# ThomasZiegler/RS-aware-differential-SfM

Hardware: AMD Instinct MI355X
Metric: Mpixels/sec RS depth+pose solve, 1280x720 pair (higher is better)
Workload: dtype f64

## Files before the change

include/rsdsfm.h:

```cpp
#ifndef RSDSFM_H
#define RSDSFM_H

#include <stddef.h>
#include <stdint.h>

#ifdef __cplusplus
extern "C" {
#endif

#define RSDSFM_OK 0
#define RSDSFM_ERR_INVALID (-1)
#define RSDSFM_ERR_HIP (-2)
#define RSDSFM_ERR_NO_DEVICE (-3)
#define RSDSFM_ERR_NUMERIC (-4)
#define RSDSFM_ERR_PENDING (-5)
#define RSDSFM_ERR_PEER (-6)

#define RSDSFM_DEPTH_CLOSED_FORM 0
#define RSDSFM_DEPTH_CERES_LM 1

#define RSDSFM_K_COMPAT 0
#define RSDSFM_K_FIXED 1

#define RSDSFM_FLOW_COMPAT_RANK 0
// ... 81 lines not shown
                  const double* alpha_m, const double* alpha_k_m, const int64_t* inlier_idx_or_null,
                  const double v_in[3], const double w_in[3], double k_in, int const_acceleration,
                  int flow_index_mode, double* inliers_out_3m, double v_out[3], double w_out[3], double* k_out,
                  rsdsfm_lm_summary* summary_or_null);
int rsdsfm_last_ransac_tag(rsdsfm_ctx* ctx, uint64_t* tag, int64_t* cache_hits_or_null);
int rsdsfm_refine_from_ransac(rsdsfm_ctx* ctx, uint64_t ransac_tag, const double* flow2n, int64_t n_flow, int64_t m, const double* inliers_3m,
                              const double* alpha_m, const double* alpha_k_m, const int64_t* inlier_idx_or_null, const double v_in[3],
                              const double w_in[3], double k_in, int const_acceleration, int flow_index_mode, double* inliers_out_3m,
                              double v_out[3], double w_out[3], double* k_out, rsdsfm_lm_summary* summary_or_null);
#define RSDSFM_REFINE_TRACE_COLS 8
#define RSDSFM_TRACE_REJECTED 0.0
#define RSDSFM_TRACE_ACCEPTED 1.0
#define RSDSFM_TRACE_INVALID 2.0
#define RSDSFM_TRACE_PARAMETER_TOL 3.0
#define RSDSFM_TRACE_FUNCTION_TOL 4.0
#define RSDSFM_TRACE_ACCEPTED_GRADIENT_TOL 5.0
int rsdsfm_set_refine_trace(rsdsfm_ctx* ctx, int32_t rows);
int rsdsfm_get_refine_trace(rsdsfm_ctx* ctx, double* trace_rows_x_8, int32_t rows);
int rsdsfm_flatten(rsdsfm_ctx* ctx, const double* flow_img_rows_cols_2, int32_t rows, int32_t cols, double fx,
                   double fy, double cx, double cy, double gamma, double flow_threshold, double* q2n,
                   double* u2n, double* alpha_n, double* alpha_k_n, int64_t* n_out);
int rsdsfm_depth_map(rsdsfm_ctx* ctx, double* inliers_3m_inout, int64_t m, double v_inout[3], double fx,
                     double fy, double cx, double cy, int32_t rows, int32_t cols,
                     double* depth_map_colmajor, int32_t* xs_or_null, int32_t* ys_or_null, int* flipped);
int rsdsfm_pose_table(rsdsfm_ctx* ctx, const double v[3], const double w[3], double k, double gamma,
                      int32_t rows, double* R_rows9, double* t_rows3);

int rsdsfm_estimate_inverse_depths_dev(rsdsfm_ctx* ctx, const double* d_q2n, const double* d_u2n, int64_t n,
                                       const double v[3], const double w[3], double k, const double* d_alpha_n,
                                       const double* d_alpha_k_n, int depth_mode, double* d_inv_depth_n);
int rsdsfm_flatten_dev(rsdsfm_ctx* ctx, const double* d_flow_img, int32_t rows, int32_t cols, double fx, double fy,
                       double cx, double cy, double gamma, double flow_threshold, double* d_q2n, double* d_u2n,
                       double* d_alpha_n, double* d_alpha_k_n, int64_t* n_out);
int rsdsfm_depth_map_dev(rsdsfm_ctx* ctx, double* d_inliers_3m_inout, int64_t m, double v_inout[3], double fx, double fy,
                         double cx, double cy, int32_t rows, int32_t cols, double* d_depth_map_colmajor,
                         int32_t* d_xs_or_null, int32_t* d_ys_or_null, int* flipped);
int rsdsfm_pose_table_dev(rsdsfm_ctx* ctx, const double v[3], const double w[3], double k, double gamma, int32_t rows,
                          double* d_R_rows9, double* d_t_rows3);
typedef struct rsdsfm_frame_params {
    int32_t ransac_trials;
    int32_t use_acceleration_mode;
    int32_t use_refinement;
    int32_t depth_mode;
    int32_t k_sign_mode;
    int32_t flow_index_mode;
    int32_t use_global_shutter_mode;
    int32_t struct_bytes;
    double ransac_tol;
    double flow_threshold;
    uint64_t seed;
} rsdsfm_frame_params;

void rsdsfm_frame_params_init(rsdsfm_frame_params* params);

typedef struct rsdsfm_frame_result {
    int64_t n_points, num_inliers;
    int32_t best_trial, flipped;
    double ransac_w[3], ransac_v[3], ransac_k;
    double w[3], v[3], k;
    rsdsfm_lm_summary refine_summary;
    const double* d_inliers;
    const int64_t* d_inlier_idx;
    const int32_t* d_scanline;
} rsdsfm_frame_result;

int rsdsfm_solve_frame_dev(rsdsfm_ctx* ctx, const double* d_flow_img, int32_t rows, int32_t cols, double fx, double fy,
                           double cx, double cy, double gamma, const rsdsfm_frame_params* params,
                           double* d_depth_map_colmajor, double* d_R_rows9_or_null, double* d_t_rows3_or_null,
                           rsdsfm_frame_result* result);
typedef struct rsdsfm_frame_job {
    const double* d_flow_img;
    int32_t rows, cols;
    double fx, fy, cx, cy, gamma;
    double* d_depth_map_colmajor;
    double* d_R_rows9_or_null;
    double* d_t_rows3_or_null;
    uint64_t seed;
} rsdsfm_frame_job;
int rsdsfm_solve_frames_dev(rsdsfm_ctx* ctx, const rsdsfm_frame_job* jobs, int32_t count, const rsdsfm_frame_params* params,
                            rsdsfm_frame_result* results);
int rsdsfm_set_sequence_lanes(rsdsfm_ctx* ctx, int32_t lanes);
int rsdsfm_set_frame_side_flatten(rsdsfm_ctx* ctx, int mode);
int rsdsfm_set_frame_tail(rsdsfm_ctx* ctx, int mode);
int rsdsfm_ransac_dev(rsdsfm_ctx* ctx, const double* d_q2n, const double* d_u2n, const double* d_alpha_n,
                      const double* d_alpha_k_n, int64_t n, int use_alpha_k, int32_t iterations, double tolerance,
                      const int32_t* samples_9xT_or_null, uint64_t seed, int depth_mode, int k_sign_mode,
                      rsdsfm_ransac_out* out);
int rsdsfm_refine_dev(rsdsfm_ctx* ctx, const double* d_flow2n, int64_t n_flow, int64_t m, const double* d_inliers_3m,
                      const double* d_alpha_m, const double* d_alpha_k_m, const int64_t* d_inlier_idx_or_null,
                      const double v_in[3], const double w_in[3], double k_in, int const_acceleration,
                      int flow_index_mode, double* d_inliers_out_3m, double v_out[3], double w_out[3], double* k_out,
                      rsdsfm_lm_summary* summary_or_null);
int rsdsfm_estimate_inverse_depths_batch_dev(rsdsfm_ctx* const* ctxs, int32_t count, const double* const* d_q2n,
                                             const double* const* d_u2n, const int64_t* n, const double* v_count_x3,
                                             const double* w_count_x3, const double* k_count, const double* const* d_alpha_n,
                                             const double* const* d_alpha_k_n, double* const* d_inv_depth_n);
int rsdsfm_depth_lm_batch_launch_dev(rsdsfm_ctx* const* ctxs, int32_t count, const double* const* d_q2n, const double* const* d_u2n,
                                     const int64_t* n, const double* v_count_x3, const double* w_count_x3, const double* k_count,
                                     const double* const* d_alpha_n, const double* const* d_alpha_k_n, double* const* d_inv_depth_n);
int rsdsfm_depth_lm_launch_dev(rsdsfm_ctx* ctx, const double* d_q2n, const double* d_u2n, int64_t n,
                               const double v[3], const double w[3], double k, const double* d_alpha_n,
                               const double* d_alpha_k_n, double* d_inv_depth_n, int launch_id);
int rsdsfm_depth_lm_sums_row_size(void);
int rsdsfm_depth_lm_reduce_dev(rsdsfm_ctx* ctx, int64_t n_shard, double* d_row_out);
int rsdsfm_depth_lm_decide_rows_dev(rsdsfm_ctx* ctx, const double* d_rows, int32_t nrows, int64_t n_total, int launch_id);
int rsdsfm_depth_lm_state(rsdsfm_ctx* ctx, int32_t* status, int32_t* next_launch, rsdsfm_lm_summary* summary_or_null);
int rsdsfm_depth_finish_dev(rsdsfm_ctx* ctx, const double* d_q2n, const double* d_u2n, int64_t n,
                            const double v[3], const double w[3], double k, const double* d_alpha_n,
                            const double* d_alpha_k_n, double* d_inv_depth_n, rsdsfm_lm_summary* summary_or_null,
                            int32_t* extra_launches);

int rsdsfm_flatten_slab_dev(rsdsfm_ctx* ctx, const double* d_img_slab, int32_t rows, int32_t slab_cols, int32_t col0,
                            double fx, double fy, double cx, double cy, double gamma, double thr, double* d_q2n,
                            double* d_u2n, double* d_alpha_n, double* d_alpha_k_n, int64_t* n_out);
int rsdsfm_sample_indices(int64_t n, int32_t iterations, uint64_t seed, int32_t* samples);
int rsdsfm_minimal9_dev(rsdsfm_ctx* ctx, const double* d_q9, const double* d_u9, const double* d_alpha9,
                        const double* d_alpha_k9, int32_t count, int use_alpha_k, int k_sign_mode, double* d_hyp);
int rsdsfm_minimal9_probe_dev(rsdsfm_ctx* ctx, const double* d_q9, const double* d_u9, const double* d_alpha9, const double* d_alpha_k9,
                              int32_t count, int use_alpha_k, int k_sign_mode, int use_cores, double* d_hyp, double* d_probe4);
size_t rsdsfm_tile_lm_state_bytes(void);
size_t rsdsfm_tile_best_bytes(void);
int32_t rsdsfm_tile_ransac_row_size(void);
int32_t rsdsfm_tile_ransac_batch(void);
int rsdsfm_tile_ransac_lm_rows_dev(rsdsfm_ctx* ctx, const double* d_q2n, const double* d_u2n, const double* d_alpha_n,
                                   const double* d_alpha_k_n, int64_t n_shard, const double* d_hyp, int32_t count,
                                   const void* d_states, int32_t round, double tolerance, double* d_rows);
int rsdsfm_tile_ransac_decide_dev(rsdsfm_ctx* ctx, const double* d_rows_all, int32_t nranks, int32_t count, void* d_states,
                                  int64_t n_total, int32_t round, int32_t* d_flags, int32_t* d_scored, double* d_trial_count,
                                  double* d_trial_err);
int rsdsfm_tile_ransac_score_rows_dev(rsdsfm_ctx* ctx, const double* d_q2n, const double* d_u2n, const double* d_alpha_n,
                                      const double* d_alpha_k_n, int64_t n_shard, const double* d_hyp, int32_t count,
                                      const void* d_states, int depth_mode, double tolerance, const int32_t* d_scored_or_null,
                                      double* d_rows);
int rsdsfm_tile_ransac_score_merge_dev(rsdsfm_ctx* ctx, const double* d_rows_all, int32_t nranks, int32_t count,
                                       const int32_t* d_scored_or_null, double* d_trial_count, double* d_trial_err);
int rsdsfm_tile_ransac_pick_dev(rsdsfm_ctx* ctx, const double* d_trial_count, const double* d_trial_err, int32_t iterations,
                                const double* d_hyp, void* d_best);
int rsdsfm_tile_ransac_final_dev(rsdsfm_ctx* ctx, const double* d_q2n, const double* d_u2n, const double* d_alpha_n,
                                 const double* d_alpha_k_n, int64_t n_shard, void* d_best, const void* d_states, int depth_mode,
                                 double tolerance, double* d_inv_depth_n, uint8_t* d_mask_n, int64_t* d_inlier_idx,
                                 double* d_inliers3m, double* d_out_alpha, double* d_out_alpha_k, rsdsfm_ransac_out* out);
int64_t rsdsfm_tile_ransac_global_inliers(rsdsfm_ctx* ctx, const void* d_best);
int rsdsfm_tile_refine_begin_dev(rsdsfm_ctx* ctx, const double* d_flow2n, int64_t n_flow, int64_t m_shard, const double* d_inl3m,
                                 const double* d_alpha_m, const double* d_alpha_k_m, const int64_t* d_inlier_idx,
                                 const double v_in[3], const double w_in[3], double k_in, int const_acceleration,
                                 int flow_index_mode);
int32_t rsdsfm_tile_refine_row_size(int const_acceleration, int32_t stage);
int rsdsfm_tile_refine_rows_dev(rsdsfm_ctx* ctx, int32_t stage, double* d_row);
int rsdsfm_tile_refine_apply_dev(rsdsfm_ctx* ctx, int32_t stage, const double* d_rows_all, int32_t nranks, int64_t m_total);
int rsdsfm_tile_refine_poll(rsdsfm_ctx* ctx, double v_out[3], double w_out[3], double* k_out, rsdsfm_lm_summary* summary);
int rsdsfm_tile_refine_finish_dev(rsdsfm_ctx* ctx, double* d_inl_out3m);
int rsdsfm_tile_zsum_dev(rsdsfm_ctx* ctx, const double* d_inl3m, int64_t m_shard, double* d_zsum1);
int rsdsfm_tile_depth_map_dev(rsdsfm_ctx* ctx, double* d_inl3m, int64_t m_shard, const double* d_zsums_all, int32_t nranks,
                              int64_t m_total, double v_inout[3], double fx, double fy, double cx, double cy, int32_t rows,
                              int32_t col0, int32_t slab_cols, double* d_depth_slab, int32_t* d_xs_or_null,
                              int32_t* d_ys_or_null, int* flipped);

#define RSDSFM_DIST_ID_BYTES 128
int rsdsfm_dist_unique_id(void* id_128_bytes);
int rsdsfm_dist_init(rsdsfm_ctx* ctx, int32_t nranks, int32_t rank, const void* id_128_bytes);
int rsdsfm_dist_adopt(rsdsfm_ctx* ctx, void* nccl_comm, int32_t nranks, int32_t rank);
typedef int (*rsdsfm_all_gather_fn)(void* user, const void* d_send, void* d_recv, size_t bytes_per_rank, void* hip_stream);
typedef int (*rsdsfm_all_reduce_sum_f64_fn)(void* user, double* d_buf, size_t count, void* hip_stream);
int rsdsfm_dist_set_transport(rsdsfm_ctx* ctx, int32_t nranks, int32_t rank, rsdsfm_all_gather_fn all_gather_fn,
                              rsdsfm_all_reduce_sum_f64_fn all_reduce_fn, void* user);
int rsdsfm_dist_finalize(rsdsfm_ctx* ctx);
// ... 75 lines not shown
```

rs-aware-differential-sfm_amd/__init__.py:

```python
import ctypes as C
import os
import sys

import numpy as np

from . import dist, pipeline, synth

_HERE = os.path.dirname(os.path.abspath(__file__))
LIB_PATH = os.environ.get("RSDSFM_LIB") or os.path.join(_HERE, "librsdsfm_hip.so")
LIB_PATH_FUSED = os.path.join(_HERE, "librsdsfm_hip_fused.so")
HEADER_PATH = os.path.join(os.path.dirname(_HERE), "include", "rsdsfm.h")

OK = 0
ERR_PENDING = -5
DEPTH_CLOSED_FORM, DEPTH_CERES_LM = 0, 1
K_COMPAT, K_FIXED = 0, 1
FLOW_COMPAT_RANK, FLOW_GATHERED = 0, 1
REFINE_TRACE_COLS = 8
TRACE_REJECTED, TRACE_ACCEPTED, TRACE_INVALID, TRACE_PARAMETER_TOL, TRACE_FUNCTION_TOL, TRACE_ACCEPTED_GRADIENT_TOL = 0.0, 1.0, 2.0, 3.0, 4.0, 5.0
TERMINATION = {0: "gradient", 1: "parameter", 2: "function", 3: "max_iter", 4: "failure", 5: "min_radius"}

_libs = {}


# ... 411 lines not shown

    def solve_frame_dev(self, d_flow_img, rows, cols, K, gamma, d_depth_map, d_R=None, d_t=None, trials=50, tol=0.05, seed=1,
                        use_acceleration_mode=False, use_refinement=True, depth_mode=DEPTH_CERES_LM, k_sign_mode=K_COMPAT, flow_threshold=1e-10,
                        flow_index_mode=FLOW_COMPAT_RANK, use_global_shutter_mode=False):
        prm = FrameParams(int(trials), int(use_acceleration_mode), int(use_refinement), int(depth_mode), int(k_sign_mode),
                          int(flow_index_mode), int(use_global_shutter_mode), 0, float(tol), float(flow_threshold), int(seed))
        res = FrameResult()
        d = C.c_double
        self._check(self.lib.rsdsfm_solve_frame_dev(self._ctx, _dp(d_flow_img), C.c_int32(rows), C.c_int32(cols), d(K[0]), d(K[1]), d(K[2]), d(K[3]),
                                                    d(gamma), C.byref(prm), _dp(d_depth_map), _dp(d_R) if d_R else None, _dp(d_t) if d_t else None,
                                                    C.byref(res)), "rsdsfm_solve_frame_dev")
        return dict(n=int(res.n_points), num_inliers=int(res.num_inliers), best_trial=int(res.best_trial), flipped=bool(res.flipped),
                    ransac_w=np.array(res.ransac_w[:]), ransac_v=np.array(res.ransac_v[:]), ransac_k=float(res.ransac_k),
                    w=np.array(res.w[:]), v=np.array(res.v[:]), k=float(res.k), refine_summary=res.refine_summary.as_dict(),
                    d_inliers=res.d_inliers, d_inlier_idx=res.d_inlier_idx, d_scanline=res.d_scanline)

    def dist_init(self, nranks, rank, unique_id):
        self._check(self.lib.rsdsfm_dist_init(self._ctx, C.c_int32(nranks), C.c_int32(rank), C.c_char_p(bytes(unique_id))), "rsdsfm_dist_init")

    def dist_set_transport(self, nranks, rank, all_gather, all_reduce):
        self._ag = ALL_GATHER_FN(lambda user, s_, r_, b_, st: int(all_gather(s_, r_, b_, st)))
        self._ar = ALL_REDUCE_FN(lambda user, p_, n_, st: int(all_reduce(p_, n_, st)))
        self._check(self.lib.rsdsfm_dist_set_transport(self._ctx, C.c_int32(nranks), C.c_int32(rank), self._ag, self._ar, None), "rsdsfm_dist_set_transport")

    def dist_finalize(self):
        self._check(self.lib.rsdsfm_dist_finalize(self._ctx), "rsdsfm_dist_finalize")

    def solve_frame_tiled_dev(self, d_img_slab, rows, cols, K, gamma, d_depth_map, d_R=None, d_t=None, trials=50, tol=0.05, seed=1,
                              use_acceleration_mode=False, use_refinement=True, depth_mode=DEPTH_CERES_LM, k_sign_mode=K_COMPAT,
                              flow_threshold=1e-10, use_global_shutter_mode=False, flow_index_mode=FLOW_COMPAT_RANK):
        prm = FrameParams(int(trials), int(use_acceleration_mode), int(use_refinement), int(depth_mode), int(k_sign_mode),
                          int(flow_index_mode), int(use_global_shutter_mode), 0, float(tol), float(flow_threshold), int(seed))
        res, info = FrameResult(), TiledInfo()
        d = C.c_double
        self._check(self.lib.rsdsfm_solve_frame_tiled_dev(self._ctx, _dp(d_img_slab) if d_img_slab else None, C.c_int32(rows), C.c_int32(cols), d(K[0]), d(K[1]),
                                                          d(K[2]), d(K[3]), d(gamma), C.byref(prm), _dp(d_depth_map), _dp(d_R) if d_R else None,
                                                          _dp(d_t) if d_t else None, C.byref(res), C.byref(info)), "rsdsfm_solve_frame_tiled_dev")
        return dict(n=int(res.n_points), num_inliers=int(res.num_inliers), best_trial=int(res.best_trial), flipped=bool(res.flipped),
                    ransac_w=np.array(res.ransac_w[:]), ransac_v=np.array(res.ransac_v[:]), ransac_k=float(res.ransac_k),
                    w=np.array(res.w[:]), v=np.array(res.v[:]), k=float(res.k), refine_summary=res.refine_summary.as_dict(),
                    d_inliers=res.d_inliers, d_inlier_idx=res.d_inlier_idx, d_scanline=res.d_scanline, flow_index_mode=int(flow_index_mode),
                    info={k2: int(getattr(info, k2)) for k2, _ in TiledInfo._fields_ if k2 != "_pad"})

    def estimate_inverse_depths_tiled_dev(self, d_q_shard, d_u_shard, n_total, v, w, k, d_alpha_shard, d_alpha_k_shard, d_inv_depth,
                                          mode=DEPTH_CERES_LM):
        sm, info = LmSummary(), TiledInfo()
        opt = lambda p_: _dp(p_) if p_ else None
        self._check(self.lib.rsdsfm_estimate_inverse_depths_tiled_dev(self._ctx, opt(d_q_shard), opt(d_u_shard), C.c_int64(n_total), _v3(v), _v3(w),
                                                                      C.c_double(k), opt(d_alpha_shard), opt(d_alpha_k_shard), C.c_int(int(mode)),
                                                                      opt(d_inv_depth), C.byref(sm), C.byref(info)),
                    "rsdsfm_estimate_inverse_depths_tiled_dev")
        return (sm.as_dict() if int(mode) == DEPTH_CERES_LM else None,
                {k2: int(getattr(info, k2)) for k2, _ in TiledInfo._fields_ if k2 != "_pad"})

    def prepared_frame_solve(self, d_flow_img, rows, cols, K, gamma, d_depth_map, d_R=None, d_t=None, trials=50, tol=0.05,
                             use_acceleration_mode=False, use_refinement=True, depth_mode=DEPTH_CERES_LM, k_sign_mode=K_COMPAT,
                             flow_threshold=1e-10, flow_index_mode=FLOW_COMPAT_RANK, use_global_shutter_mode=False):
        prm = FrameParams(int(trials), int(use_acceleration_mode), int(use_refinement), int(depth_mode), int(k_sign_mode),
                          int(flow_index_mode), int(use_global_shutter_mode), 0, float(tol), float(flow_threshold), 0)
        res = FrameResult()
        d = C.c_double
        fn = self.lib.rsdsfm_solve_frame_dev
        args = (self._ctx, _dp(d_flow_img), C.c_int32(rows), C.c_int32(cols), d(K[0]), d(K[1]), d(K[2]), d(K[3]), d(gamma), C.byref(prm),
                _dp(d_depth_map), _dp(d_R) if d_R else None, _dp(d_t) if d_t else None, C.byref(res))
        check = self._check

        def call(seed):
            prm.seed = seed
            rc = fn(*args)
            if rc != OK:
                check(rc, "rsdsfm_solve_frame_dev")
            return res

        return call

    def set_sequence_lanes(self, lanes):
        self._check(self.lib.rsdsfm_set_sequence_lanes(self._ctx, C.c_int32(int(lanes))), "rsdsfm_set_sequence_lanes")

    def set_frame_side_flatten(self, on):
        self._check(self.lib.rsdsfm_set_frame_side_flatten(self._ctx, int(on)), "rsdsfm_set_frame_side_flatten")

    def set_frame_tail(self, mode):
        self._check(self.lib.rsdsfm_set_frame_tail(self._ctx, int(mode)), "rsdsfm_set_frame_tail")

    def prepared_frames_solve(self, jobs, trials=50, tol=0.05, use_acceleration_mode=False, use_refinement=True, depth_mode=DEPTH_CERES_LM,
                              k_sign_mode=K_COMPAT, flow_threshold=1e-10, flow_index_mode=FLOW_COMPAT_RANK, use_global_shutter_mode=False):
        n = len(jobs)
        arr = (FrameJob * n)()
        for a, j in zip(arr, jobs):
            K = j["K"]
            a.d_flow_img, a.rows, a.cols = int(j["d_flow_img"]), int(j["rows"]), int(j["cols"])
            a.fx, a.fy, a.cx, a.cy, a.gamma = float(K[0]), float(K[1]), float(K[2]), float(K[3]), float(j["gamma"])
            a.d_depth_map, a.d_R, a.d_t = int(j["d_depth_map"]), int(j.get("d_R") or 0) or None, int(j.get("d_t") or 0) or None
        prm = FrameParams(int(trials), int(use_acceleration_mode), int(use_refinement), int(depth_mode), int(k_sign_mode),
                          int(flow_index_mode), int(use_global_shutter_mode), 0, float(tol), float(flow_threshold), 0)
        res = (FrameResult * n)()
        fn, ctx, check = self.lib.rsdsfm_solve_frames_dev, self._ctx, self._check

        def call(seeds):
            for a, sd in zip(arr, seeds):
                a.seed = int(sd)
            rc = fn(ctx, arr, C.c_int32(n), C.byref(prm), res)
            if rc != OK:
                check(rc, "rsdsfm_solve_frames_dev")
            return res

        return call

    def solve_frames_dev(self, jobs, seeds, **kw):
        res = self.prepared_frames_solve(jobs, **kw)(seeds)
        return [dict(n=int(r.n_points), num_inliers=int(r.num_inliers), best_trial=int(r.best_trial), flipped=bool(r.flipped),
                     ransac_w=np.array(r.ransac_w[:]), ransac_v=np.array(r.ransac_v[:]), ransac_k=float(r.ransac_k),
                     w=np.array(r.w[:]), v=np.array(r.v[:]), k=float(r.k), refine_summary=r.refine_summary.as_dict(),
                     d_inliers=r.d_inliers, d_inlier_idx=r.d_inlier_idx, d_scanline=r.d_scanline) for r in res]

    def depth_lm_reduce_dev(self, n_shard, d_row):
        self._check(self.lib.rsdsfm_depth_lm_reduce_dev(self._ctx, C.c_int64(n_shard), _dp(d_row)), "rsdsfm_depth_lm_reduce_dev")

    def depth_lm_decide_rows_dev(self, d_rows, nrows, n_total, launch_id):
        self._check(self.lib.rsdsfm_depth_lm_decide_rows_dev(self._ctx, _dp(d_rows), C.c_int32(nrows), C.c_int64(n_total), int(launch_id)), "rsdsfm_depth_lm_decide_rows_dev")

    def depth_lm_state(self):
        status, nxt, sm = C.c_int32(), C.c_int32(), LmSummary()
        self._check(self.lib.rsdsfm_depth_lm_state(self._ctx, C.byref(status), C.byref(nxt), C.byref(sm)), "rsdsfm_depth_lm_state")
        return status.value, nxt.value, sm.as_dict()

    def depth_finish_dev(self, d_q, d_u, n, v, w, k, d_alpha, d_alpha_k, d_rho):
        sm = LmSummary()
        extra = C.c_int32()
        self._check(self.lib.rsdsfm_depth_finish_dev(self._ctx, _dp(d_q), _dp(d_u), C.c_int64(n), _v3(v), _v3(w), C.c_double(k), _dp(d_alpha), _dp(d_alpha_k), _dp(d_rho), C.byref(sm), C.byref(extra)), "rsdsfm_depth_finish_dev")
        return sm.as_dict(), extra.value


def _np0(ptr):
    return _dp(ptr) if ptr else None


def tile_sizes():
    lib = load_library()
    lib.rsdsfm_tile_lm_state_bytes.restype = C.c_size_t
    lib.rsdsfm_tile_best_bytes.restype = C.c_size_t
    return (int(lib.rsdsfm_tile_lm_state_bytes()), int(lib.rsdsfm_tile_best_bytes()), int(lib.rsdsfm_tile_ransac_row_size()),
            int(lib.rsdsfm_tile_ransac_batch()))


def sample_indices(n, iterations, seed):
    lib = load_library()
    out = np.zeros((max(int(iterations), 0), 9), dtype=np.int32)
    rc = lib.rsdsfm_sample_indices(C.c_int64(n), C.c_int32(iterations), C.c_uint64(seed), _p(out))
    if rc != OK:
        raise RsdsfmError("rsdsfm_sample_indices failed (%d): needs 9 <= n < 2^31" % rc)
    return out


class _TileMixin:
    def flatten_slab_dev(self, d_img_slab, rows, slab_cols, col0, K, gamma, d_q, d_u, d_alpha, d_alpha_k, thr=1e-10):
        cnt = C.c_int64()
        d = C.c_double
        self._check(self.lib.rsdsfm_flatten_slab_dev(self._ctx, _np0(d_img_slab), C.c_int32(rows), C.c_int32(slab_cols), C.c_int32(col0), d(K[0]), d(K[1]), d(K[2]), d(K[3]), d(gamma), d(thr), _np0(d_q), _np0(d_u), _np0(d_alpha), _np0(d_alpha_k), C.byref(cnt)), "rsdsfm_flatten_slab_dev")
        return cnt.value

    def minimal9_probe_dev(self, d_q9, d_u9, d_a9, d_ak9, count, use_alpha_k, k_sign_mode, use_cores, d_hyp, d_probe4):
        self._check(self.lib.rsdsfm_minimal9_probe_dev(self._ctx, _dp(d_q9), _dp(d_u9), _dp(d_a9), _dp(d_ak9), C.c_int32(count), int(use_alpha_k), int(k_sign_mode),
                                                       int(use_cores), _dp(d_hyp), _dp(d_probe4)), "rsdsfm_minimal9_probe_dev")

    def minimal9_dev(self, d_q9, d_u9, d_a9, d_ak9, count, use_alpha_k, k_sign_mode, d_hyp):
# ... 1441 lines not shown
```

rs-aware-differential-sfm_amd/csrc/frame_host.hip:

```cpp
#include <stdlib.h>
#include <string.h>

#include <atomic>

#include <algorithm>
#include <new>

#include "rsdsfm_internal.hpp"
#include "sequence_host.hpp"

namespace rsdsfm {

static std::atomic<int> g_frames_in_flight[64];
int frames_in_flight(const Ctx* c) { return g_frames_in_flight[c->device & 63].load(std::memory_order_relaxed); }

int alpha_ones_launch(Ctx* c, double* d_alpha, int64_t n);
int flatten_device(Ctx* c, const double* d_img, int32_t rows, int32_t cols, int32_t col0, double fx, double fy, double cx, double cy, double gamma,
                   double thr, double* d_q, double* d_u, double* d_alpha, double* d_alpha_k, int64_t* n_out);

struct FrameRun {
    rsdsfm_frame_job job;
    rsdsfm_frame_params prm;
    size_t N = 0;
    int64_t n = 0;
    double *d_q = nullptr, *d_u = nullptr, *d_a = nullptr, *d_ak = nullptr, *d_in_a = nullptr, *d_in_ak = nullptr, *d_inl = nullptr, *d_inl_ref = nullptr;
    int64_t* d_idx = nullptr;
    uint8_t* d_mask = nullptr;
    int32_t* d_ys = nullptr;
    double *d_zpartials = nullptr, *d_zheader = nullptr;
    char* d_refine_ws = nullptr;
    rsdsfm_ransac_out ro;
    RansacRun ransac;
    RefineRun refine;
    Minimal9Direct direct;
    DenseFlatten dense;
    bool refinement_enqueued = false, ahead = false, side_flatten = false, dense_in_launch = false, open = false;
    bool counted = false;
    int rc_begin = RSDSFM_OK;
    int64_t m_known = -1;
    RefineTail tail;
    FinishClaim claim;
    RansacSpecTail spec_tail;
    std::function<int()> join;
};

namespace {

inline double* header_host(Ctx* c) { return reinterpret_cast<double*>(static_cast<char*>(c->h_pinned) + c->pinned_bytes - 64); }
inline RefineState* state_host(Ctx* c) { return reinterpret_cast<RefineState*>(static_cast<char*>(c->h_pinned) + c->pinned_bytes - kPinnedTail); }
inline int64_t* count_host(Ctx* c) { return reinterpret_cast<int64_t*>(static_cast<char*>(c->h_pinned) + c->pinned_bytes - kPinnedTail / 2); }
static_assert(sizeof(RefineState) + sizeof(int) <= kPinnedTail / 2, "reserved tail: state read-back | point count ... depth-map header");

struct StreamSwap {
    Ctx* c;
    hipStream_t main;
    StreamSwap(Ctx* ctx, hipStream_t other) : c(ctx), main(ctx->stream) { c->stream = other; }
    ~StreamSwap() { c->stream = main; }
};

int ensure_side_stream(Ctx* c) {
    if (c->aux_stream) return RSDSFM_OK;
    RSDSFM_HIP_CHECK(c, hipStreamCreateWithFlags(&c->aux_stream, hipStreamNonBlocking));
    RSDSFM_HIP_CHECK(c, hipEventCreateWithFlags(&c->ev_fork, hipEventDisableTiming));
    RSDSFM_HIP_CHECK(c, hipEventCreateWithFlags(&c->ev_join, hipEventDisableTiming));
    return RSDSFM_OK;
}

static void frame_uncount(const Ctx* c, FrameRun* F) {
    if (F && F->counted) {
        F->counted = false;
        g_frames_in_flight[c->device & 63].fetch_sub(1, std::memory_order_relaxed);
    }
}
struct FrameInFlightEnd {
    const Ctx* c;
    FrameRun* F;
    ~FrameInFlightEnd() { frame_uncount(c, F); }
};

int frame_begin(Ctx* c, FrameRun* F) {
    const rsdsfm_frame_job& J = F->job;
    const rsdsfm_frame_params* prm = &F->prm;
    frame_uncount(c, F);
    F->open = false;
    F->rc_begin = RSDSFM_OK;
    if (J.rows <= 0 || J.cols <= 0 || !J.d_flow_img || !J.d_depth_map_colmajor) return fail(c, RSDSFM_ERR_INVALID, "bad arguments");
    if (prm->flow_index_mode != RSDSFM_FLOW_COMPAT_RANK && prm->flow_index_mode != RSDSFM_FLOW_GATHERED) return fail(c, RSDSFM_ERR_INVALID, "unknown flow_index_mode");
    if (prm->struct_bytes != 0 && prm->struct_bytes != (int32_t)sizeof(rsdsfm_frame_params))
        return fail(c, RSDSFM_ERR_INVALID, "rsdsfm_frame_params: struct_bytes is neither 0 nor sizeof(rsdsfm_frame_params) -- caller built against another header (use rsdsfm_frame_params_init)");
    const int32_t rows = J.rows, cols = J.cols;
    const double fx = J.fx, fy = J.fy, cx = J.cx, cy = J.cy, gamma = J.gamma;
    const size_t N = (size_t)rows * (size_t)cols;
    F->N = N;
    const size_t ncells = (size_t)flatten_cells(rows, cols);
    const size_t need = 2 * Arena::need(16 * N) + 4 * Arena::need(8 * N) + 2 * Arena::need(24 * N) + Arena::need(8 * N) + Arena::need(N) +
                        Arena::need(4 * N) + Arena::need(8 * 1024) + Arena::need(64) + Arena::need(refine_workspace_bytes(c, (int64_t)N, true)) +
                        2 * Arena::need(sizeof(int64_t) * (ncells + 2048)) + Arena::need(64) + 4096;
    if (need > c->frame_bytes) {
        RSDSFM_HIP_CHECK(c, hipStreamSynchronize(c->stream));
        if (c->d_frame) RSDSFM_HIP_CHECK(c, hipFree(c->d_frame));
        c->d_frame = nullptr;
        c->frame_bytes = 0;
        RSDSFM_HIP_CHECK(c, hipMalloc(&c->d_frame, need));
        c->frame_bytes = need;
    }
    Arena fa(c->d_frame);
    F->d_q = fa.take<double>(2 * N);
    F->d_u = fa.take<double>(2 * N);
    F->d_a = fa.take<double>(N);
    F->d_ak = fa.take<double>(N);
    F->d_in_a = fa.take<double>(N);
    F->d_in_ak = fa.take<double>(N);
    F->d_inl = fa.take<double>(3 * N);
    F->d_inl_ref = fa.take<double>(3 * N);
    F->d_idx = fa.take<int64_t>(N);
    F->d_mask = fa.take<uint8_t>(N);
    F->d_ys = fa.take<int32_t>(N);
    F->d_zpartials = fa.take<double>(1024);
    F->d_zheader = fa.take<double>(8);
    F->d_refine_ws = fa.take<char>(refine_workspace_bytes(c, (int64_t)N, true));
    int64_t* d_flat_counts = fa.take<int64_t>(ncells);
    int64_t* d_flat_offsets = fa.take<int64_t>(ncells + 2048);

    int rc = ensure_pinned(c, ransac_pinned_bytes(prm->ransac_trials));
    if (rc != RSDSFM_OK) return rc;
    int64_t n = (int64_t)N;
    F->side_flatten = false;
    if (c->frame_dense_hint) {
        *count_host(c) = -1;
        int side = prm->ransac_trials > 0 ? c->frame_side_flatten : 0;
        if (side == 3 && prm->ransac_trials > c->num_cus * 2) side = 0;
        F->dense_in_launch = false;
        if (side) {
            F->side_flatten = true;
            F->direct = Minimal9Direct();
            F->direct.img = J.d_flow_img, F->direct.rows = rows, F->direct.cols = cols, F->direct.alpha_ones = prm->use_global_shutter_mode ? 1 : 0;
            F->direct.fx = fx, F->direct.fy = fy, F->direct.cx = cx, F->direct.cy = cy, F->direct.gamma = gamma;
        }
        if (side == 3) {
            if (!c->d_flat_counters) {
                RSDSFM_HIP_CHECK(c, hipMalloc(reinterpret_cast<void**>(&c->d_flat_counters), 2 * sizeof(unsigned long long)));
                RSDSFM_HIP_CHECK(c, hipMemsetAsync(c->d_flat_counters, 0, 2 * sizeof(unsigned long long), c->stream));
            }
            F->dense = DenseFlatten();
            F->dense.thr = prm->flow_threshold;
            F->dense.d_q = F->d_q, F->dense.d_u = F->d_u, F->dense.d_alpha = F->d_a, F->dense.d_alpha_k = F->d_ak;
            F->dense.d_counters = c->d_flat_counters;
            F->dense.total_out = count_host(c);
            F->dense_in_launch = true;
        } else if (side == 2) {
            F->join = [c, F, d_flat_counts, d_flat_offsets]() -> int {
                const rsdsfm_frame_job& J2 = F->job;
                int rc2 = flatten_launch(c, J2.d_flow_img, J2.rows, J2.cols, 0, J2.fx, J2.fy, J2.cx, J2.cy, J2.gamma, F->prm.flow_threshold, F->d_q, F->d_u, F->d_a,
                                         F->d_ak, d_flat_counts, d_flat_offsets, count_host(c), nullptr);
                if (rc2 == RSDSFM_OK && F->prm.use_global_shutter_mode) rc2 = alpha_ones_launch(c, F->d_a, (int64_t)F->N);
                return rc2;
            };
        } else if (side == 1) {
            rc = ensure_side_stream(c);
            if (rc != RSDSFM_OK) return rc;
            RSDSFM_HIP_CHECK(c, hipEventRecord(c->ev_fork, c->stream));
            RSDSFM_HIP_CHECK(c, hipStreamWaitEvent(c->aux_stream, c->ev_fork, 0));
            {
                StreamSwap on_side(c, c->aux_stream);
                rc = flatten_launch(c, J.d_flow_img, rows, cols, 0, fx, fy, cx, cy, gamma, prm->flow_threshold, F->d_q, F->d_u, F->d_a, F->d_ak,
                                    d_flat_counts, d_flat_offsets, count_host(c), nullptr);
                if (rc == RSDSFM_OK && prm->use_global_shutter_mode) rc = alpha_ones_launch(c, F->d_a, n);
            }
            if (rc != RSDSFM_OK) return rc;
            RSDSFM_HIP_CHECK(c, hipEventRecord(c->ev_join, c->aux_stream));
            F->join = [c]() -> int {
                RSDSFM_HIP_CHECK(c, hipStreamWaitEvent(c->stream, c->ev_join, 0));
                return RSDSFM_OK;
            };
        } else {
            rc = flatten_enqueue(c, J.d_flow_img, rows, cols, fx, fy, cx, cy, gamma, prm->flow_threshold, F->d_q, F->d_u, F->d_a, F->d_ak, count_host(c));
            if (rc != RSDSFM_OK) return rc;
        }
    } else {
        rc = flatten_device(c, J.d_flow_img, rows, cols, 0, fx, fy, cx, cy, gamma, prm->flow_threshold, F->d_q, F->d_u, F->d_a, F->d_ak, &n);
        if (rc != RSDSFM_OK) return rc;
        *count_host(c) = n;
    }
    if (prm->use_global_shutter_mode && !F->side_flatten) {
        rc = alpha_ones_launch(c, F->d_a, n);
        if (rc != RSDSFM_OK) return rc;
    }
    F->n = n;
    memset(&F->ro, 0, sizeof(F->ro));
    F->ro.inlier_idx = F->d_idx;
    F->ro.inliers = F->d_inl;
    F->ro.alpha = F->d_in_a;
    F->ro.alpha_k = F->d_in_ak;
    F->ro.mask = F->d_mask;
    F->m_known = -1;
    F->tail = [c, F](const RefineBuffers& B) -> int {
        const rsdsfm_frame_job& J2 = F->job;
        const RefineState* st = B.state;
        const int64_t m_arg = F->m_known >= 0 ? F->m_known : F->n;
        const int64_t* m_dev = F->m_known >= 0 ? nullptr : &st->m;
        PoseTableOut pt;
        if (J2.d_R_rows9_or_null && J2.d_t_rows3_or_null)
            pt.R = J2.d_R_rows9_or_null, pt.t = J2.d_t_rows3_or_null, pt.rows = J2.rows, pt.gamma = J2.gamma, pt.wk_dev = st->p + 3;
        if (B.claim.on)
            return depth_map_decided_launch(c, F->d_inl_ref, m_arg, F->d_zpartials, refine_finish_grid(c, B), B, J2.d_depth_map_colmajor, F->d_zheader,
                                            header_host(c), st->p, m_dev, &pt);
        return depth_map_slab_launch(c, F->d_inl_ref, m_arg, F->d_zpartials, refine_finish_grid(c, B), m_arg, nullptr, J2.fx, J2.fy, J2.cx, J2.cy, J2.rows,
                                     0, J2.cols, J2.d_depth_map_colmajor, nullptr, F->d_ys, F->d_zheader, header_host(c), st->p, m_dev, &pt);
    };
    F->claim = FinishClaim();
    if (c->frame_tail == 0) {
        F->claim.on = true;
        F->claim.fx = J.fx, F->claim.fy = J.fy, F->claim.cx = J.cx, F->claim.cy = J.cy;
        F->claim.rows = rows, F->claim.cols = cols;
        F->claim.ys = F->d_ys;
    }
    F->spec_tail = [c, F](const RansacBest* d_best) -> int {
        return refine_begin(c, F->d_u, F->n, F->n, F->d_inl, F->d_in_a, F->d_in_ak, F->d_idx, nullptr, nullptr, 0.0, F->prm.use_acceleration_mode,
                            F->prm.flow_index_mode, F->d_inl_ref, &F->tail, d_best, F->d_refine_ws, &F->refine, state_host(c), F->d_zpartials, false,
                            &F->claim);
    };
    F->refinement_enqueued = false;
    F->ahead = prm->use_refinement && c->ransac_spec_miss < 2;
    F->open = true;
    g_frames_in_flight[c->device & 63].fetch_add(1, std::memory_order_relaxed);
    F->counted = true;
    F->rc_begin = ransac_begin(c, F->d_q, F->d_u, F->d_a, F->d_ak, n, prm->use_acceleration_mode, prm->ransac_trials, prm->ransac_tol, nullptr, J.seed,
                               prm->depth_mode, prm->k_sign_mode, &F->ro, prm->use_refinement ? &F->spec_tail : nullptr, &F->refinement_enqueued, &F->ransac,
                               F->side_flatten ? &F->direct : nullptr, F->side_flatten && !F->dense_in_launch ? &F->join : nullptr,
                               F->dense_in_launch ? &F->dense : nullptr, F->ahead, true,
                               F->claim.on && prm->use_refinement ? refine_flag_words(F->d_refine_ws) : nullptr);
    return RSDSFM_OK;
}

int frame_finish(Ctx* c, FrameRun* F, rsdsfm_frame_result* res) {
    if (!F->open) return fail(c, RSDSFM_ERR_INVALID, "no frame solve in flight");
    F->open = false;
    FrameInFlightEnd in_flight_end_{c, F};
    const rsdsfm_frame_job& J = F->job;
    const rsdsfm_frame_params* prm = &F->prm;
    memset(res, 0, sizeof(*res));
    int rc = F->rc_begin;
    if (rc == RSDSFM_OK) rc = ransac_finish(c, &F->ransac);
    if (rc != RSDSFM_OK) RSDSFM_HIP_CHECK(c, hipStreamSynchronize(c->stream));
    if (F->side_flatten && c->aux_stream) RSDSFM_HIP_CHECK(c, hipStreamSynchronize(c->aux_stream));
    int64_t n = F->n;
    if (*count_host(c) < 0) {
        c->frame_dense_hint = 1;
        return rc != RSDSFM_OK ? rc : fail(c, RSDSFM_ERR_NUMERIC, "frame solve: the point count did not arrive");
    }
    bool counted = true;
    if (*count_host(c) != n) {
        if (F->dense_in_launch) {
            int64_t n_real = 0;
            rc = flatten_device(c, J.d_flow_img, J.rows, J.cols, 0, J.fx, J.fy, J.cx, J.cy, J.gamma, prm->flow_threshold, F->d_q, F->d_u, F->d_a, F->d_ak, &n_real);
            if (rc == RSDSFM_OK && prm->use_global_shutter_mode) rc = alpha_ones_launch(c, F->d_a, n_real);
            if (rc != RSDSFM_OK) return rc;
            *count_host(c) = n_real;
        }
        n = *count_host(c);
        F->n = n;
        F->refinement_enqueued = false;
        counted = false;
        rc = ransac_begin(c, F->d_q, F->d_u, F->d_a, F->d_ak, n, prm->use_acceleration_mode, prm->ransac_trials, prm->ransac_tol, nullptr, J.seed,
                          prm->depth_mode, prm->k_sign_mode, &F->ro, prm->use_refinement ? &F->spec_tail : nullptr, &F->refinement_enqueued, &F->ransac, nullptr, nullptr,
                          nullptr, F->ahead, true,
                               F->claim.on && prm->use_refinement ? refine_flag_words(F->d_refine_ws) : nullptr);
        if (rc == RSDSFM_OK) rc = ransac_finish(c, &F->ransac);
        counted = rc == RSDSFM_OK;
    }
    c->frame_dense_hint = n == (int64_t)F->N ? 1 : 0;
    if (rc != RSDSFM_OK) return rc;
    if (counted) ransac_commit_hints(c, F->ransac);
    const rsdsfm_ransac_out& ro = F->ro;
    res->n_points = n;
    res->num_inliers = ro.num_inliers;
    res->best_trial = ro.best_trial;
    memcpy(res->ransac_w, ro.w, sizeof(ro.w));
    memcpy(res->ransac_v, ro.v, sizeof(ro.v));
    res->ransac_k = ro.k;
    double v[3], w[3], k = ro.k;
    for (int i = 0; i < 3; ++i) v[i] = ro.v[i], w[i] = ro.w[i];
    double* d_final = F->d_inl;
    int flipped = 0;
    F->m_known = ro.num_inliers;
    if (prm->use_refinement) {
        bool exact = false;
        if (F->refinement_enqueued) {
            rc = refine_poll(c, &F->refine, v, w, &k, &res->refine_summary);
            exact = rc == kRcRefineRestartExact;
        }
        if (!F->refinement_enqueued || exact)
            rc = refine_device(c, F->d_u, n, ro.num_inliers, F->d_inl, F->d_in_a, F->d_in_ak, F->d_idx, v, w, k, prm->use_acceleration_mode,
                               prm->flow_index_mode, F->d_inl_ref, v, w, &k, &res->refine_summary, &F->tail, F->d_zpartials, exact, &F->claim);
        if (rc != RSDSFM_OK) return rc;
        d_final = F->d_inl_ref;
        const double* h_header = header_host(c);
        flipped = h_header[0] != 0.0;
        v[0] = h_header[1], v[1] = h_header[2], v[2] = h_header[3];
    } else {
        rc = depth_map_device(c, d_final, ro.num_inliers, v, J.fx, J.fy, J.cx, J.cy, J.rows, J.cols, J.d_depth_map_colmajor, nullptr, F->d_ys, &flipped, w,
                              k, J.gamma, J.d_R_rows9_or_null, J.d_t_rows3_or_null);
        if (rc != RSDSFM_OK) return rc;
    }
    res->flipped = flipped;
    memcpy(res->v, v, sizeof(v));
    memcpy(res->w, w, sizeof(w));
    res->k = k;
    res->d_inliers = d_final;
    res->d_inlier_idx = F->d_idx;
    res->d_scanline = F->d_ys;
    return RSDSFM_OK;
}

FrameRun* frame_run_of(Ctx* c) {
    if (!c->frame_run) c->frame_run = new (std::nothrow) FrameRun();
    return static_cast<FrameRun*>(c->frame_run);
}

}

void frame_release(Ctx* c) {
    frame_uncount(c, static_cast<FrameRun*>(c->frame_run));
    delete static_cast<FrameRun*>(c->frame_run);
    c->frame_run = nullptr;
    for (rsdsfm_ctx* lane : c->lanes) rsdsfm_destroy(lane);
    c->lanes.clear();
    if (c->ev_fork) (void)hipEventDestroy(c->ev_fork);
    if (c->ev_join) (void)hipEventDestroy(c->ev_join);
    if (c->ev_seq) (void)hipEventDestroy(c->ev_seq);
    if (c->aux_stream) (void)hipStreamDestroy(c->aux_stream);
    if (c->d_flat_counters) (void)hipFree(c->d_flat_counters);
    c->d_flat_counters = nullptr;
    c->ev_fork = c->ev_join = c->ev_seq = nullptr;
    c->aux_stream = nullptr;
}

}

using namespace rsdsfm;

extern "C" {

void rsdsfm_frame_params_init(rsdsfm_frame_params* p) {
    if (!p) return;
    memset(p, 0, sizeof(*p));
    p->ransac_trials = 5;
    p->use_acceleration_mode = 0;
    p->use_refinement = 1;
    p->depth_mode = RSDSFM_DEPTH_CERES_LM;
    p->k_sign_mode = RSDSFM_K_COMPAT;
    p->flow_index_mode = RSDSFM_FLOW_COMPAT_RANK;
    p->use_global_shutter_mode = 0;
    p->struct_bytes = (int32_t)sizeof(rsdsfm_frame_params);
    p->ransac_tol = 0.05;
    p->flow_threshold = 1e-10;
    p->seed = 1;
}

int rsdsfm_solve_frame_dev(rsdsfm_ctx* ctx, const double* d_flow_img, int32_t rows, int32_t cols, double fx, double fy, double cx,
                           double cy, double gamma, const rsdsfm_frame_params* prm, double* d_depth_map, double* d_R_rows9,
                           double* d_t_rows3, rsdsfm_frame_result* res) {
    if (!ctx) return RSDSFM_ERR_INVALID;
    Ctx* c = &ctx->c;
    DeviceGuard device_guard_(c);
    if (!prm || !res) return fail(c, RSDSFM_ERR_INVALID, "bad arguments");
    FrameRun* F = frame_run_of(c);
    if (!F) return fail(c, RSDSFM_ERR_INVALID, "out of host memory");
    F->prm = *prm;
    F->job = rsdsfm_frame_job{d_flow_img, rows, cols, fx, fy, cx, cy, gamma, d_depth_map, d_R_rows9, d_t_rows3, prm->seed};
    int rc = frame_begin(c, F);
    if (rc != RSDSFM_OK) return rc;
    return frame_finish(c, F, res);
}

int rsdsfm_set_sequence_lanes(rsdsfm_ctx* ctx, int32_t lanes) {
    if (!ctx) return RSDSFM_ERR_INVALID;
    Ctx* c = &ctx->c;
    DeviceGuard device_guard_(c);
    if (lanes < 0 || lanes > 16) return fail(c, RSDSFM_ERR_INVALID, "lanes must be 0 (default) .. 16");
    c->seq_lanes = lanes;
    return RSDSFM_OK;
}

int rsdsfm_set_frame_tail(rsdsfm_ctx* ctx, int mode) {
    if (!ctx) return RSDSFM_ERR_INVALID;
    if (mode < 0 || mode > 1) return fail(&ctx->c, RSDSFM_ERR_INVALID, "mode must be 0 (short launch tail) or 1 (stage-by-stage launches)");
    ctx->c.frame_tail = mode;
    return RSDSFM_OK;
}

int rsdsfm_set_frame_side_flatten(rsdsfm_ctx* ctx, int mode) {
    if (!ctx) return RSDSFM_ERR_INVALID;
    if (mode < 0 || mode > 3) return fail(&ctx->c, RSDSFM_ERR_INVALID, "mode must be 0 (flatten first), 1 (flatten on a second stream), 2 (flatten behind the minimal solver) or 3 (flatten inside the solver's launch)");
    ctx->c.frame_side_flatten = mode;
    return RSDSFM_OK;
}

}

namespace rsdsfm {

int sequence_lane_count(const Ctx* c, int count) { return std::max(1, std::min<int>(count, c->seq_lanes > 0 ? c->seq_lanes : kSequenceLanesDefault)); }

int solve_frames_run(Ctx* c, const rsdsfm_frame_job* jobs, int32_t count, const rsdsfm_frame_params* prm, rsdsfm_frame_result* results, const PairHook* hook) {
    const int L = sequence_lane_count(c, count);
    while ((int)c->lanes.size() < L - 1) {
        rsdsfm_ctx* lane = nullptr;
        int rc = rsdsfm_create(&lane, c->device, nullptr);
        if (rc != RSDSFM_OK) return fail(c, rc, "could not create a sequence lane");
        c->lanes.push_back(lane);
    }
    auto lane_ctx = [&](int l) -> Ctx* { return l == 0 ? c : &c->lanes[(size_t)l - 1]->c; };
    if (L > 1) {
        if (!c->ev_seq) RSDSFM_HIP_CHECK(c, hipEventCreateWithFlags(&c->ev_seq, hipEventDisableTiming));
        RSDSFM_HIP_CHECK(c, hipEventRecord(c->ev_seq, c->stream));
    }
    for (int l = 1; l < L; ++l) {
        Ctx* lc = lane_ctx(l);
        RSDSFM_HIP_CHECK(c, hipStreamWaitEvent(lc->stream, c->ev_seq, 0));
        lc->ransac_k0 = c->ransac_k0;
        lc->ransac_math_mode = c->ransac_math_mode;
        lc->lm_arithmetic = c->lm_arithmetic;
        lc->refine_arithmetic = c->refine_arithmetic;
        lc->lma_count_only_force = c->lma_count_only_force;
        lc->frame_side_flatten = c->frame_side_flatten;
        lc->frame_tail = c->frame_tail;
        lc->refine_stage_mode = c->refine_stage_mode;
    }
    for (int l = 0; l < L; ++l) lane_ctx(l)->refine_stage_separate = L > 1;
    int first_error = RSDSFM_OK;
    int in_flight[16];
    for (int l = 0; l < 16; ++l) in_flight[l] = -1;
    auto finish_lane = [&](int l) {
        const int i = in_flight[l];
        if (i < 0) return;
        in_flight[l] = -1;
        Ctx* lc = lane_ctx(l);
        int rc = frame_finish(lc, static_cast<FrameRun*>(lc->frame_run), &results[i]);
        if (rc != RSDSFM_OK && first_error == RSDSFM_OK) {
            first_error = rc;
            if (lc != c) c->err = "pair " + std::to_string(i) + ": " + lc->err;
        }
        if (rc == RSDSFM_OK && hook && first_error == RSDSFM_OK) {
            rc = (*hook)(lc, i, static_cast<FrameRun*>(lc->frame_run)->job, results[i]);
            if (rc != RSDSFM_OK) {
                first_error = rc;
                c->err = "pair " + std::to_string(i) + ": " + std::string(lc->err);
            }
        }
    };
    for (int i = 0; i < count && first_error == RSDSFM_OK; ++i) {
        const int l = i % L;
        finish_lane(l);
        if (first_error != RSDSFM_OK) break;
        Ctx* lc = lane_ctx(l);
        FrameRun* F = frame_run_of(lc);
        if (!F) {
            first_error = fail(c, RSDSFM_ERR_INVALID, "out of host memory");
            break;
        }
        F->prm = *prm;
        F->job = jobs[i];
        int rc = frame_begin(lc, F);
        if (rc != RSDSFM_OK) {
            first_error = rc;
            if (lc != c) c->err = "pair " + std::to_string(i) + ": " + lc->err;
            break;
        }
        in_flight[l] = i;
    }
    for (;;) {
        int best = -1;
        for (int l = 0; l < L; ++l)
            if (in_flight[l] >= 0 && (best < 0 || in_flight[l] < in_flight[best])) best = l;
        if (best < 0) break;
        finish_lane(best);
    }
    for (int l = 0; l < L; ++l) lane_ctx(l)->refine_stage_separate = false;
    return first_error;
}

}

extern "C" {

int rsdsfm_solve_frames_dev(rsdsfm_ctx* ctx, const rsdsfm_frame_job* jobs, int32_t count, const rsdsfm_frame_params* prm, rsdsfm_frame_result* results) {
    if (!ctx) return RSDSFM_ERR_INVALID;
    Ctx* c = &ctx->c;
    DeviceGuard device_guard_(c);
    if (count < 0 || !prm || (count > 0 && (!jobs || !results))) return fail(c, RSDSFM_ERR_INVALID, "bad arguments");
    if (count == 0) return RSDSFM_OK;
    return solve_frames_run(c, jobs, count, prm, results, nullptr);
}

int rsdsfm_set_refine_stage(rsdsfm_ctx* ctx, int mode) {
    if (!ctx) return RSDSFM_ERR_INVALID;
    Ctx* c = &ctx->c;
    if (mode < 0 || mode > 2) return fail(c, RSDSFM_ERR_INVALID, "refine stage: 0 (automatic), 1 (in the next pass's prologue) or 2 (a launch of its own)");
    c->refine_stage_mode = mode;
    return RSDSFM_OK;
}

}
```

rs-aware-differential-sfm_amd/csrc/ransac_host.hip:

```cpp
#include <stdio.h>
#include <stdlib.h>
#include <string.h>

#include <algorithm>
#include <vector>

#include "rsdsfm_internal.hpp"

namespace rsdsfm {

namespace {


inline uint64_t splitmix64(uint64_t& state) {
    uint64_t z = (state += 0x9E3779B97F4A7C15ULL);
    z = (z ^ (z >> 30)) * 0xBF58476D1CE4E5B9ULL;
    z = (z ^ (z >> 27)) * 0x94D049BB133111EBULL;
    return z ^ (z >> 31);
}

void sample_indices(int64_t n, int T, uint64_t seed, std::vector<int32_t>& out) {
    struct Slot {
        int64_t key;
        int32_t val;
// ... 75 lines not shown
    rsdsfm_ransac_out* out = R.out;
    const int T = R.T, Tn = R.Tn, batch = R.batch, depth_mode = R.depth_mode;
    const int64_t n = R.n;
    const double tol = R.tol;
    int rc = RSDSFM_OK;
    for (;;) {
        switch (R.pc) {
            case kPcStart: {
                const bool zero_in_minimal9 = T > 0 && R.zero_bytes % 8 == 0 && (reinterpret_cast<uintptr_t>(R.zero_begin) & 7) == 0;
                if (!zero_in_minimal9) RSDSFM_HIP_CHECK(c, hipMemsetAsync(R.zero_begin, 0, R.zero_bytes, c->stream));
                if (T > 0) {
                    memcpy(R.h_samples_pinned, R.samples.data(), sizeof(int32_t) * (size_t)T * 9);
                    Minimal9Direct dir = R.direct ? *R.direct : Minimal9Direct();
                    R.core_epoch = 0;
                    if (R.core_math && depth_mode == RSDSFM_DEPTH_CERES_LM && T <= c->num_cus * 2 && c->d_core_flag) {
                        c->core_epoch = c->core_epoch >= 0x3fffffff ? 1 : c->core_epoch + 1;
                        dir.core_flag = c->d_core_flag;
                        dir.core_epoch = R.core_epoch = c->core_epoch;
                    }
                    if (R.direct && R.dense && T <= c->num_cus * 2)
                        rc = minimal9_flatten_launch(c, R.h_samples_pinned, T, R.use_alpha_k, R.k_sign_mode, R.d_hyp, zero_in_minimal9 ? R.zero_begin : nullptr,
                                                     zero_in_minimal9 ? R.zero_bytes : 0, dir, R.dense->thr, R.dense->d_q, R.dense->d_u, R.dense->d_alpha,
                                                     R.dense->d_alpha_k, R.dense->d_counters, R.dense->total_out);
                    else
                        rc = minimal9_launch(c, R.d_q, R.d_u, R.d_a, R.d_ak, R.h_samples_pinned, T, R.use_alpha_k, R.k_sign_mode, R.d_hyp,
                                             zero_in_minimal9 ? R.zero_begin : nullptr, zero_in_minimal9 ? R.zero_bytes : 0, &dir);
                    if (rc != RSDSFM_OK) return rc;
                    if (R.after_minimal9) {
                        rc = (*R.after_minimal9)();
                        if (rc != RSDSFM_OK) return rc;
                    }
                }
                R.b0 = 0;
                R.pc = kPcBatchBegin;
                break;
            }
            case kPcBatchBegin: {
                if (R.b0 >= T) {
                    R.pc = kPcFinal;
                    break;
                }
                R.B = std::min(batch, T - R.b0);
                R.need_score = true;
                if (depth_mode == RSDSFM_DEPTH_CERES_LM) {
                    if (R.b0 > 0)
                        RSDSFM_HIP_CHECK(c, hipMemsetAsync(R.d_flags, 0, (size_t)(reinterpret_cast<char*>(R.d_irr_count + R.batch) - reinterpret_cast<char*>(R.d_flags)), c->stream));
                    R.round = 0;
                    R.pc = kPcRoundEnqueue;
                } else {
                    R.pc = kPcScore;
                }
                break;
            }
            case kPcRoundEnqueue: {
                const int b0 = R.b0, B = R.B, round = R.round;
                bool flags_via_pick = false;
                if (round > 4 * kMaxIter) return fail(c, RSDSFM_ERR_NUMERIC, "LM state machines did not terminate");
                if (R.analytic && round == 0) {
                    rc = ransac_lma_launch(c, R.d_q, R.d_u, R.d_a, R.d_ak, n, R.d_hyp + (size_t)b0 * 8, B, R.d_states + b0, R.d_partials, R.d_flags,
                                           R.d_scored + b0, R.d_tcount + b0, R.d_terr + b0, tol, R.lma_cand, 2, R.d_irr_count, R.d_irr_list, R.d_unscored,
                                           nullptr, R.core_epoch ? c->d_core_flag : nullptr, R.core_epoch, R.count_only);
                } else {
                    rc = ransac_lm_round_launch(c, R.d_q, R.d_u, R.d_a, R.d_ak, n, R.d_hyp + (size_t)b0 * 8, B, R.d_states + b0, R.d_partials, R.d_flags,
                                                R.d_scored + b0, R.d_tcount + b0, R.d_terr + b0, round, tol, R.k0, R.fused_base, R.core_math,
                                                R.core_epoch ? c->d_core_flag : nullptr, R.core_epoch, R.d_unscored);
                }
                if (rc != RSDSFM_OK) return rc;
                if (round == 0 && B == T) {
                    const PickLazy lazy = R.count_only ? PickLazy{R.d_scored, R.d_unscored, R.d_flags + 1} : PickLazy();
                    if (c->ransac_score_idle < kScoreIdleLimit) {
                        if (R.count_only) {
                            rc = ransac_pick_launch(c, R.d_tcount, R.d_terr, T, R.d_hyp, R.d_best, nullptr, R.d_flags, nullptr, 0, nullptr, 0, 0, nullptr, 0.0, lazy);
                            if (rc != RSDSFM_OK) return rc;
                        }
                        rc = ransac_score_launch(c, R.d_q, R.d_u, R.d_a, R.d_ak, n, R.d_hyp, T, R.d_states, depth_mode, tol, R.d_scored, R.d_partials,
                                                 R.d_tcount, R.d_terr, R.d_unscored, R.d_flags + 1);
                        if (rc != RSDSFM_OK) return rc;
                        R.spec_scored = true;
                    }
                    rc = ransac_pick_launch(c, R.d_tcount, R.d_terr, T, R.d_hyp, R.d_best, R.h_best, R.d_flags, R.h_running, R.spec_scored ? 1 : 0,
                                            nullptr, 0, 0, nullptr, R.tie_margin, lazy);
                    if (rc != RSDSFM_OK) return rc;
                    flags_via_pick = true;
                    rc = ransac_final_launch(c, R.d_q, R.d_u, R.d_a, R.d_ak, n, R.d_best, R.d_states, depth_mode, tol, R.d_rho, R.d_mask, R.d_bcounts,
                                             R.d_boffs, out->inlier_idx, out->inliers, out->alpha, out->alpha_k, R.h_best, R.refine_flag_words);
                    if (rc != RSDSFM_OK) return rc;
                    R.final_done = true;
                    R.spec_final = true;
                    if (R.spec_tail && R.tail_ahead) {
                        rc = (*R.spec_tail)(R.d_best);
                        if (rc != RSDSFM_OK) return rc;
                        R.tail_enqueued = true;
                    }
                }
                if (!flags_via_pick) RSDSFM_HIP_CHECK(c, hipMemcpyAsync(R.h_running, R.d_flags, sizeof(int) * 8, hipMemcpyDeviceToHost, c->stream));
                R.pc = kPcRoundWait;
                if (yield_at_wait) return RSDSFM_OK;
                break;
            }
            case kPcRoundWait: {
                yield_at_wait = false;
                if (int rcs = sync_stream(c, "ransac_finish line 244")) return rcs;
                const int* h_running = R.h_running;
                if (R.round == 0 && R.analytic && (h_running[3] & 16) != 0) R.lma_guard |= h_running[3] >> 8;
                if (R.round == 0 && R.analytic && (h_running[3] & 6) != 0 && !((h_running[3] & 1) && R.core_math)) {
                    rc = lma_start_over(c, R, (h_running[3] >> 8) | ((h_running[3] & 4) ? (1 << 7) : 0));
                    if (rc != RSDSFM_OK) return rc;
                    break;
                }
                if (R.round == 0 && R.core_math && (h_running[3] & 1) != 0) {
                    R.core_math = false;
                    R.restarted = true;
                    R.not_one_step = 0;
                    R.final_done = R.spec_scored = R.tail_enqueued = R.spec_final = false;
                    R.dense = nullptr;
                    R.after_minimal9 = nullptr;
                    R.pc = kPcStart;
                    break;
                }
                if (R.round == 0) {
                    R.not_one_step += h_running[2];
                    if (R.b0 == 0) {
                        int best = 0;
                        for (int a2 = 1; a2 <= 3; ++a2)
                            if (h_running[4 + a2] > (best ? h_running[4 + best] : 0)) best = a2;
                        if (best) R.fused_base_next = best;
                        int second = 0;
                        for (int a2 = 1; a2 <= 3; ++a2)
                            if (a2 != best && h_running[4 + a2] > (second ? h_running[4 + second] : 0)) second = a2;
                        if (best) {
                            R.lma_cand_next[0] = best;
                            R.lma_cand_next[1] = second ? second : (best > 1 ? best - 1 : 2);
                        }
                    }
                }
                if (h_running[0] == 0) {
                    R.pc = kPcAfterRounds;
                } else {
                    R.final_done = false;
                    R.round += 1;
                    R.pc = kPcRoundEnqueue;
                }
                break;
            }
            case kPcAfterRounds: {
                R.need_score = R.h_running[1] > 0;
                if (R.B == T) R.score_hint_next = R.need_score ? 1 : 0;
                if (R.need_score && R.final_done && R.spec_scored && !R.h_best->lazy_pending) R.need_score = false;
                if (R.need_score) R.final_done = false;
                R.pc = kPcScore;
                break;
            }
            case kPcScore: {
                if (R.need_score) {
                    rc = ransac_score_launch(c, R.d_q, R.d_u, R.d_a, R.d_ak, n, R.d_hyp + (size_t)R.b0 * 8, R.B, R.d_states + R.b0, depth_mode, tol,
                                             depth_mode == RSDSFM_DEPTH_CERES_LM ? R.d_scored + R.b0 : nullptr, R.d_partials, R.d_tcount + R.b0,
                                             R.d_terr + R.b0, depth_mode == RSDSFM_DEPTH_CERES_LM ? R.d_unscored : nullptr, R.d_flags + 1);
                    if (rc != RSDSFM_OK) return rc;
                }
                R.b0 += batch;
                R.pc = kPcBatchBegin;
                break;
            }
            case kPcFinal: {
                if (!R.final_done) {
                    R.tail_enqueued = false;
                    R.spec_final = false;
                    rc = ransac_pick_launch(c, R.d_tcount, R.d_terr, T, R.d_hyp, R.d_best, R.h_best, nullptr, nullptr, 0, nullptr, 0, 0, nullptr, R.tie_margin,
                                            R.count_only ? PickLazy{R.d_scored, R.d_unscored, R.d_flags + 1} : PickLazy());
                    if (rc != RSDSFM_OK) return rc;
                    rc = ransac_final_launch(c, R.d_q, R.d_u, R.d_a, R.d_ak, n, R.d_best, R.d_states, depth_mode, tol, R.d_rho, R.d_mask, R.d_bcounts,
                                             R.d_boffs, out->inlier_idx, out->inliers, out->alpha, out->alpha_k, R.h_best, R.refine_flag_words);
                    if (rc != RSDSFM_OK) return rc;
                }
                if (R.spec_tail && !R.tail_enqueued) {
                    rc = (*R.spec_tail)(R.d_best);
                    if (rc != RSDSFM_OK) return rc;
                    R.tail_enqueued = true;
                }
                if (T > 0 && out->trial_count) RSDSFM_HIP_CHECK(c, hipMemcpyAsync(R.h_tcount, R.d_tcount, sizeof(double) * T, hipMemcpyDeviceToHost, c->stream));
                if (T > 0 && out->trial_err) RSDSFM_HIP_CHECK(c, hipMemcpyAsync(R.h_terr, R.d_terr, sizeof(double) * T, hipMemcpyDeviceToHost, c->stream));
                if (T > 0 && out->trial_vel) RSDSFM_HIP_CHECK(c, hipMemcpyAsync(R.h_hyp, R.d_hyp, sizeof(double) * 8 * T, hipMemcpyDeviceToHost, c->stream));
                if (T > 0 && out->trial_steps && depth_mode == RSDSFM_DEPTH_CERES_LM)
                    RSDSFM_HIP_CHECK(c, hipMemcpyAsync(R.h_states, R.d_states, sizeof(LmState) * T, hipMemcpyDeviceToHost, c->stream));
                R.pc = kPcFinalWait;
                if (yield_at_wait) return RSDSFM_OK;
                break;
            }
            case kPcFinalWait: {
                if (int rcs = sync_stream(c, "ransac_finish line 345")) return rcs;
                const RansacBest* h_best = R.h_best;
#ifdef RSDSFM_DEBUG_HOOKS
                if (getenv("RSDSFM_RANSAC_DEBUG")) fprintf(stderr, "[ransac] final wait: lazy_pending %d undecided %d flags %d %d %d %d hist %d %d %d %d spec_scored %d spec_final %d tail %d idle %d\n", h_best->lazy_pending, h_best->undecided, R.h_running[0], R.h_running[1], R.h_running[2], R.h_running[3], R.h_running[4], R.h_running[5], R.h_running[6], R.h_running[7], (int)R.spec_scored, (int)R.spec_final, (int)R.tail_enqueued, c->ransac_score_idle);
#endif
                if (R.count_only && h_best->lazy_pending) {
                    if (++R.lazy_rounds > T + 2) return fail(c, RSDSFM_ERR_NUMERIC, "lazy error sums did not settle");
                    R.final_done = R.tail_enqueued = R.spec_final = false;
                    R.need_score = true;
                    R.score_hint_next = 1;
                    R.b0 = 0;
                    R.B = T;
                    R.pc = kPcScore;
                    break;
                }
                if (R.analytic && h_best->lma_tie) {
                    rc = lma_start_over(c, R, 1 << 7);
                    if (rc != RSDSFM_OK) return rc;
                    break;
                }
                R.lma_tie_seen = h_best->lma_tie != 0;
                R.shared_best = h_best->shared_best;
                if (h_best->num_inliers != h_best->num_inliers_scan) {
                    if (R.analytic) {
                        rc = lma_start_over(c, R, 1 << 10);
                        if (rc != RSDSFM_OK) return rc;
                        break;
                    }
                    return fail(c, RSDSFM_ERR_NUMERIC, "inlier count mismatch between scoring and compaction");
                }
                out->num_inliers = h_best->num_inliers;
                out->best_trial = h_best->best_trial;
                memcpy(out->w, &h_best->hyp[0], 3 * sizeof(double));
                memcpy(out->v, &h_best->hyp[3], 3 * sizeof(double));
                out->k = h_best->hyp[6];
                out->inlier_error = h_best->inlier_error;
                for (int t = 0; t < T; ++t) {
                    if (out->trial_count) out->trial_count[t] = (int64_t)R.h_tcount[t];
                    if (out->trial_err) out->trial_err[t] = R.h_terr[t];
                    if (out->trial_vel) memcpy(out->trial_vel + (size_t)7 * t, R.h_hyp + (size_t)8 * t, 7 * sizeof(double));
                    if (out->trial_steps) out->trial_steps[t] = depth_mode == RSDSFM_DEPTH_CERES_LM ? R.h_states[t].num_successful : 1;
                }
                if (R.spec_tail_held) *R.spec_tail_held = R.tail_enqueued;
                R.hints_ready = true;
                R.pc = kPcDone;
                (void)Tn;
                return RSDSFM_OK;
            }
            default:
                return RSDSFM_OK;
        }
    }
}

}

void ransac_commit_hints(Ctx* c, const RansacRun& R) {
    if (!R.hints_ready || R.depth_mode != RSDSFM_DEPTH_CERES_LM || R.T <= 0) return;
    if (R.fused_base_next) c->ransac_fused_base = R.fused_base_next;
    if (R.score_hint_next >= 0) c->ransac_score_idle = R.score_hint_next ? 0 : std::min(c->ransac_score_idle + 1, kScoreIdleLimit);
    c->ransac_not_one_step = R.not_one_step;
    c->ransac_spec_miss = R.spec_final ? 0 : std::min(c->ransac_spec_miss + 1, 2);
    if (R.count_only) c->lma_count_only_runs += 1, c->lma_lazy_runs += (R.lazy_rounds > 0 || R.shared_best > 1) ? 1 : 0;
    if (R.lazy_rounds > 0 || R.shared_best > 1) c->lma_unique_run = 0;
    else if (R.shared_best == 1) c->lma_unique_run = std::min(c->lma_unique_run + 1, 2);
    if (R.lma_guard) c->lma_last_guard = R.lma_guard, c->lma_handed_over += 1;
    if (R.lma_restarted) {
        c->lma_hold = 16;
        c->lma_restarts += 1;
        c->lma_last_guard = R.lma_guard;
    } else if (c->lma_hold > 0 && !R.analytic) {
        c->lma_hold = R.lma_tie_seen ? 16 : c->lma_hold - 1;
    }
    if (R.restarted) {
        c->ransac_standard_math = 16;
        c->ransac_restarts += 1;
    } else if (c->ransac_standard_math > 0) {
        c->ransac_standard_math -= 1;
    }
}

int ransac_begin(Ctx* c, const double* d_q, const double* d_u, const double* d_a, const double* d_ak, int64_t n, int use_alpha_k, int T,
                 double tol, const int32_t* h_samples, uint64_t seed, int depth_mode, int k_sign_mode, rsdsfm_ransac_out* out,
                 const RansacSpecTail* spec_tail, bool* spec_tail_held, RansacRun* run, const Minimal9Direct* direct,
                 const std::function<int()>* after_minimal9, const DenseFlatten* dense, bool tail_ahead, bool count_only, int* refine_flag_words) {
    RansacRun& R = *run;
    R = RansacRun();
    R.tail_ahead = tail_ahead;
    R.core_math = c->ransac_math_mode == 0 && c->ransac_standard_math == 0;
    R.analytic = depth_mode == RSDSFM_DEPTH_CERES_LM && T > 0 && c->lm_arithmetic == 0 && c->lma_hold == 0;
    R.tie_margin = depth_mode != RSDSFM_DEPTH_CERES_LM || c->lm_arithmetic != 0 ? 0.0 : (R.analytic ? kLmaTie : -kLmaTie);
    R.lma_cand[0] = c->lma_cand[0], R.lma_cand[1] = c->lma_cand[1];
    R.count_only = count_only && R.analytic && T <= kRansacBatch && (c->lma_unique_run >= 2 || c->lma_count_only_force);
    if (R.count_only) R.tie_margin = 0.0;
    R.refine_flag_words = refine_flag_words;
    if (spec_tail_held) *spec_tail_held = false;
    if (!out) return fail(c, RSDSFM_ERR_INVALID, "null out");
    if (n < 9) return fail(c, RSDSFM_ERR_INVALID, "ransac needs at least 9 points (the reference would compute rand() % 0)");
    if (T < 0) return fail(c, RSDSFM_ERR_INVALID, "negative iterations");
    if (depth_mode != RSDSFM_DEPTH_CLOSED_FORM && depth_mode != RSDSFM_DEPTH_CERES_LM) return fail(c, RSDSFM_ERR_INVALID, "unknown depth_mode");
    if (n > (int64_t)INT32_MAX) return fail(c, RSDSFM_ERR_INVALID, "n exceeds the int32 sample index range");
    if (T > 0) {
        if (h_samples) {
            R.samples.assign(h_samples, h_samples + (size_t)T * 9);
            for (int32_t s : R.samples)
                if (s < 0 || s >= n) return fail(c, RSDSFM_ERR_INVALID, "sample index out of range");
        } else {
            sample_indices(n, T, seed, R.samples);
        }
    }
    const int Tn = std::max(T, 1);
    const int batch = std::min(Tn, kRansacBatch);
    const size_t partials_doubles = std::max<size_t>((size_t)ransac_lm_partials_doubles(c, n, batch), (size_t)ransac_lma_partials_doubles(c, n, batch));
    size_t need = Arena::need(sizeof(double) * Tn * 8) + Arena::need(sizeof(int) * batch) + Arena::need(sizeof(int) * ransac_lma_list_ints(batch)) +
                  Arena::need(sizeof(LmState) * Tn) + Arena::need(sizeof(double) * partials_doubles) +
                  Arena::need(sizeof(int) * 8) + 2 * Arena::need(sizeof(int) * Tn) + 2 * Arena::need(sizeof(double) * Tn) + Arena::need(sizeof(RansacBest)) +
                  2 * Arena::need(sizeof(int64_t) * 2048) + Arena::need(sizeof(double) * (size_t)n) + Arena::need((size_t)n) + 4096;
    int rc = ensure_ws(c, need);
    if (rc != RSDSFM_OK) return rc;
    Arena ws(c->d_ws);
    R.d_hyp = ws.take<double>((size_t)Tn * 8);
    R.zero_begin = ws.base + ws.off;
    R.d_states = ws.take<LmState>(Tn);
    R.d_scored = ws.take<int>(Tn);
    R.d_flags = ws.take<int>(8);
    R.d_irr_count = ws.take<int>(batch);
    R.zero_bytes = (size_t)((ws.base + ws.off) - R.zero_begin);
    R.d_irr_list = ws.take<int>(ransac_lma_list_ints(batch));
    R.d_unscored = ws.take<int>(batch);
    R.d_partials = ws.take<double>(partials_doubles);
    R.d_tcount = ws.take<double>(Tn);
    R.d_terr = ws.take<double>(Tn);
    R.d_best = ws.take<RansacBest>(1);
    R.d_bcounts = ws.take<int64_t>(2048);
    R.d_boffs = ws.take<int64_t>(2048);
    R.d_rho = out->inv_depth ? out->inv_depth : ws.take<double>((size_t)n);
    R.d_mask = out->mask ? out->mask : ws.take<uint8_t>((size_t)n);

    rc = ensure_pinned(c, ransac_pinned_bytes(T));
    if (rc != RSDSFM_OK) return rc;
    if (!c->d_core_flag) {
        RSDSFM_HIP_CHECK(c, hipMalloc(reinterpret_cast<void**>(&c->d_core_flag), 64));
        RSDSFM_HIP_CHECK(c, hipMemsetAsync(c->d_core_flag, 0, 64, c->stream));
    }
    char* hp = static_cast<char*>(c->h_pinned);
    R.h_best = reinterpret_cast<RansacBest*>(hp);
    R.h_running = reinterpret_cast<int*>(hp + sizeof(RansacBest));
    R.h_tcount = reinterpret_cast<double*>(hp + sizeof(RansacBest) + 32);
    R.h_terr = R.h_tcount + Tn;
    R.h_hyp = R.h_terr + Tn;
    R.h_states = reinterpret_cast<LmState*>(R.h_hyp + (size_t)8 * Tn);
    R.h_samples_pinned = reinterpret_cast<int32_t*>(R.h_states + Tn);

    R.d_q = d_q, R.d_u = d_u, R.d_a = d_a, R.d_ak = d_ak;
    R.n = n, R.T = T, R.Tn = Tn, R.batch = batch, R.tol = tol, R.depth_mode = depth_mode, R.use_alpha_k = use_alpha_k, R.k_sign_mode = k_sign_mode;
    R.out = out, R.spec_tail = spec_tail, R.spec_tail_held = spec_tail_held;
    R.direct = direct, R.after_minimal9 = after_minimal9, R.dense = dense;
    R.k0 = c->ransac_k0 != 0 ? c->ransac_k0 : (c->ransac_not_one_step == 0 ? 2 : (int)KMAX);
    R.fused_base = R.k0 == 2 ? 1 : std::min(std::max(c->ransac_fused_base, 1), (int)KMAX);
    R.pc = kPcStart;
    return ransac_advance(c, R, true);
}

int ransac_finish(Ctx* c, RansacRun* run) { return ransac_advance(c, *run, false); }

int ransac_device(Ctx* c, const double* d_q, const double* d_u, const double* d_a, const double* d_ak, int64_t n,
                  int use_alpha_k, int T, double tol, const int32_t* h_samples, uint64_t seed, int depth_mode,
                  int k_sign_mode, rsdsfm_ransac_out* out, const RansacSpecTail* spec_tail, bool* spec_tail_held) {
    RansacRun run;
    int rc = ransac_begin(c, d_q, d_u, d_a, d_ak, n, use_alpha_k, T, tol, h_samples, seed, depth_mode, k_sign_mode, out, spec_tail, spec_tail_held,
// ... 126 lines not shown
```

rs-aware-differential-sfm_amd/csrc/ransac_kernels.hip:

```cpp
#include <algorithm>

#include "device_math.hpp"
#include "lm_common.hpp"
#include "rsdsfm_internal.hpp"

namespace rsdsfm {

namespace {

constexpr int kRB = 256;
constexpr int kRP = RSDSFM_FUSED ? 5 : 6;
constexpr int kFused = 1;
constexpr int kTiledFusedBase = 2;
constexpr int NSR = NS + 2 * kFused;
constexpr int kNSum = NSR - (KMAX + 1);
constexpr int kTStride = 65;

template <int K0>
struct R0Shape {
    static constexpr int NSk = 3 + 5 * K0;
    static constexpr int F = kFused;
    static constexpr int nsum = NSk - (K0 + 1) + 2 * F;
};
static_assert(R0Shape<KMAX>::nsum == kNSum, "full shape uses every sum slot");
// ... 599 lines not shown
    }
}

__global__ __launch_bounds__(64) void ransac_pick_kernel(const double* __restrict__ trial_count, const double* __restrict__ trial_err, int T,
                                                        const double* __restrict__ hyp, RansacBest* best, RansacBest* best_host,
                                                        const int* __restrict__ flags, int* __restrict__ flags_host, int scored_ahead,
                                                        const double* __restrict__ cnt_rt = nullptr, int cnt_stride = 0, int nranks = 0,
                                                        int64_t* __restrict__ m_all = nullptr, double tie_margin = 0.0, PickLazy lazy = PickLazy()) {
    if (blockIdx.x != 0) return;
    const int lane = threadIdx.x;
    int undecided = (flags && (flags[0] != 0 || (flags[1] > 0 && !scored_ahead) || flags[3] != 0)) ? 1 : 0;
    double best_count, best_err;
    int bi;
    pick_best_trial(trial_count, trial_err, T, lane, bi, best_count, best_err);
    int tie = 0;
    if (tie_margin != 0.0 && bi >= 0 && best_count > 0.0 && !(flags && (flags[0] != 0 || (flags[1] > 0 && !scored_ahead)))) {
        const double tm = fabs(tie_margin);
        for (int t0 = 0; t0 < T; t0 += 64) {
            const int t = t0 + lane;
            const bool hit = t < T && t != bi && trial_count[t] == best_count && fabs(trial_err[t] - best_err) <= tm * best_count;
            if (__builtin_amdgcn_ballot_w64(hit) != 0) tie = 1;
        }
    }
    if (tie_margin > 0.0) undecided |= tie;
    int pending = 0, list_n = 0, ns = 0;
    if (bi >= 0 && best_count > 0.0 && !(flags && (flags[0] != 0 || (flags[1] > 0 && !scored_ahead) || flags[3] != 0))) {
        int nco = 0;
        for (int t0 = 0; t0 < T; t0 += 64) {
            const int t = t0 + lane;
            const bool hit = t < T && trial_count[t] == best_count;
            ns += __builtin_popcountll(__builtin_amdgcn_ballot_w64(hit));
            nco += __builtin_popcountll(__builtin_amdgcn_ballot_w64(hit && lazy.scored && lazy.scored[t] == 2));
        }
        if (ns > 1 && nco > 0) {
            int base = 0;
            for (int t0 = 0; t0 < T; t0 += 64) {
                const int t = t0 + lane;
                const bool co = t < T && trial_count[t] == best_count && lazy.scored[t] == 2;
                const unsigned long long mk = __builtin_amdgcn_ballot_w64(co);
                if (co) {
                    lazy.list[base + __builtin_popcountll(mk & ((1ull << lane) - 1ull))] = t;
                    lazy.scored[t] = 0;
                }
                base += __builtin_popcountll(mk);
            }
            if (lane == 0) *lazy.list_count = nco;
            pending = 1;
            list_n = nco;
            undecided = 1;
        }
    }
    if (flags_host && lane < 8) flags_host[lane] = (lane == 1 && pending) ? list_n : (flags[lane] | ((lane == 3 && tie && tie_margin > 0.0) ? 4 : 0));
    if (m_all)
        for (int r = lane; r < nranks; r += 64) m_all[r] = bi >= 0 ? (int64_t)cnt_rt[(int64_t)r * cnt_stride + bi] : 0;
    const double h = (lane < 8 && bi >= 0) ? hyp[(int64_t)bi * 8 + lane] : 0.0;
    if (lane < 8) best->hyp[lane] = h;
    if (lane < 8 && best_host) best_host->hyp[lane] = h;
    if (lane == 0) {
        best->best_trial = bi;
        best->undecided = undecided;
        best->lma_tie = tie;
        best->lazy_pending = pending;
        best->shared_best = ns;
        best->num_inliers = bi >= 0 ? (int64_t)best_count : 0;
        best->inlier_error = best_err;
        if (best_host) {
            best_host->best_trial = bi;
            best_host->undecided = undecided;
            best_host->lma_tie = tie;
            best_host->lazy_pending = pending;
            best_host->shared_best = ns;
            best_host->num_inliers = bi >= 0 ? (int64_t)best_count : 0;
            best_host->inlier_error = best_err;
        }
    }
}

__global__ __launch_bounds__(kRB) void ransac_final_kernel(const double2* __restrict__ q, const double2* __restrict__ u,
                                                          const double* __restrict__ alpha,
                                                          const double* __restrict__ alpha_k, int64_t n, int64_t chunk,
                                                          const RansacBest* __restrict__ best,
                                                          const LmState* __restrict__ states, int depth_mode, double tol,
                                                          double* __restrict__ rho_out, uint8_t* __restrict__ mask_out,
                                                          int64_t* __restrict__ block_counts) {
    __shared__ LmPlanLds plan;
    __shared__ int s_cnt[kRB / 64];
    const int tid = threadIdx.x, lane = tid & 63, wv = tid >> 6;
    if (best->undecided) return;
    const int bt = best->best_trial;
    Pose pose;
    pose.w[0] = best->hyp[0], pose.w[1] = best->hyp[1], pose.w[2] = best->hyp[2];
    pose.v[0] = best->hyp[3], pose.v[1] = best->hyp[4], pose.v[2] = best->hyp[5];
    pose.k = best->hyp[6];
    if (depth_mode == RSDSFM_DEPTH_CERES_LM && bt >= 0) {
        if (tid == 0) {
            plan.n_hist = states[bt].n_hist;
            plan.K = 0;
            plan.write_which = 0;
        }
        if (tid < kMaxIter) plan.inv_hist[tid] = 1.0 / states[bt].hist[tid];
    }
    __syncthreads();
    const double two_over = 2.0 / (2.0 + pose.k);
    const int64_t i0 = (int64_t)blockIdx.x * chunk;
    const int64_t i1 = (i0 + chunk < n) ? i0 + chunk : n;
    int count = 0;
    for (int64_t i = i0 + tid; i < i1; i += kRB) {
        double2 qq = q[i], uu = u[i];
        const double al = alpha[i], ak = alpha_k[i];
        bool in = false;
        double rho = 0.0;
        if (bt >= 0) {
            rho = hyp_rho(qq.x, qq.y, uu.x, uu.y, al, ak, pose, two_over, depth_mode, plan);
            in = point_error(qq.x, qq.y, uu.x, uu.y, al, ak, pose, two_over, rho) < tol;
        }
        rho_out[i] = rho;
        mask_out[i] = in ? 1 : 0;
        count += in ? 1 : 0;
    }
    for (int off = 32; off >= 1; off >>= 1) count += __shfl_xor(count, off, 64);
    if (lane == 0) s_cnt[wv] = count;
    __syncthreads();
    if (tid == 0) {
        int c = 0;
        for (int w2 = 0; w2 < kRB / 64; ++w2) c += s_cnt[w2];
        block_counts[blockIdx.x] = c;
    }
}

__global__ __launch_bounds__(256) void ransac_scan_kernel(const int64_t* __restrict__ block_counts, int nblocks,
                                                         int64_t* __restrict__ block_offsets, RansacBest* best, RansacBest* best_host) {
    __shared__ int64_t s_part[256];
    const int tid = threadIdx.x;
    const int per = (nblocks + 255) / 256;
    int64_t sum = 0;
    for (int j = 0; j < per; ++j) {
        const int b = tid * per + j;
        if (b < nblocks) sum += block_counts[b];
    }
    s_part[tid] = sum;
    __syncthreads();
    if (tid == 0) {
        int64_t run = 0;
        for (int i = 0; i < 256; ++i) {
            int64_t v = s_part[i];
            s_part[i] = run;
            run += v;
        }
        best->num_inliers_scan = run;
        if (best_host) best_host->num_inliers_scan = run;
    }
    __syncthreads();
    int64_t run = s_part[tid];
    for (int j = 0; j < per; ++j) {
        const int b = tid * per + j;
        if (b < nblocks) {
            block_offsets[b] = run;
            run += block_counts[b];
        }
    }
}

__global__ __launch_bounds__(kRB) void ransac_scatter_kernel(const double2* __restrict__ q, const double* __restrict__ alpha,
                                                            const double* __restrict__ alpha_k, int64_t n, int64_t chunk,
                                                            const double* __restrict__ rho, const uint8_t* __restrict__ mask,
                                                            const int64_t* __restrict__ block_counts, RansacBest* best,
                                                            RansacBest* best_host, int64_t* __restrict__ inlier_idx, double* __restrict__ inliers,
                                                            double* __restrict__ out_alpha, double* __restrict__ out_alpha_k,
                                                            int* __restrict__ zero_words = nullptr) {
    __shared__ int s_wave[kRB / 64];
    __shared__ int64_t s_base;
    if (zero_words && blockIdx.x == 0 && threadIdx.x < (int)(kRefineStateBlockTail / sizeof(int))) zero_words[threadIdx.x] = 0;
    __shared__ int64_t s_pre[kRB / 64], s_all[kRB / 64];
    const int tid = threadIdx.x, lane = tid & 63, wv = tid >> 6;
    const int undecided = best->undecided;
    const int64_t i0 = (int64_t)blockIdx.x * chunk;
    const int64_t i1 = (i0 + chunk < n) ? i0 + chunk : n;
    {
        int64_t pre = 0, all = 0;
        for (int b = tid; b < (int)gridDim.x; b += kRB) {
            const int64_t cnt = block_counts[b];
            all += cnt;
            if (b < (int)blockIdx.x) pre += cnt;
        }
#pragma unroll
        for (int off = 32; off > 0; off >>= 1) {
            pre += __shfl_down(pre, off);
            all += __shfl_down(all, off);
        }
        if (lane == 0) s_pre[wv] = pre, s_all[wv] = all;
        __syncthreads();
        if (tid == 0) {
            int64_t p2 = 0, a2 = 0;
            for (int w2 = 0; w2 < kRB / 64; ++w2) p2 += s_pre[w2], a2 += s_all[w2];
            s_base = p2;
            if (blockIdx.x == 0 && !undecided) {
                best->num_inliers_scan = a2;
                if (best_host) best_host->num_inliers_scan = a2;
            }
        }
    }
// ... 113 lines not shown
    return RSDSFM_OK;
}

int ransac_score_launch(Ctx* c, const double* q, const double* u, const double* a, const double* ak, int64_t n,
                        const double* hyp, int T, const LmState* states, int depth_mode, double tol, const int* scored,
                        double* partials, double* trial_count, double* trial_err, const int* unscored_list, const int* unscored_count) {
    const int grid = ransac_pixel_grid(c, n);
    const int groups = ransac_lm_groups(c, grid, T);
    hipLaunchKernelGGL(ransac_score_kernel, dim3(((grid + 7) / 8) * 8 * groups), dim3(kRB), sizeof(double) * T * 2, c->stream,
                       reinterpret_cast<const double2*>(q), reinterpret_cast<const double2*>(u), a, ak, n, hyp, T, states,
                       depth_mode, tol, scored, partials, grid, groups, unscored_list, unscored_list ? unscored_count : nullptr);
    RSDSFM_HIP_CHECK(c, hipGetLastError());
    hipLaunchKernelGGL(ransac_reduce_scores_kernel, dim3(T), dim3(256), 0, c->stream, partials, grid, T, scored, trial_count,
                       trial_err);
    RSDSFM_HIP_CHECK(c, hipGetLastError());
    return RSDSFM_OK;
}

int ransac_lm_rows_launch(Ctx* c, const double* q, const double* u, const double* a, const double* ak, int64_t n,
                          const double* hyp, int T, const LmState* states, double* partials, int round, double tol, double* rows,
                          int* core_flags, const int* m9_flag, int m9_epoch) {
    const int grid = ransac_pixel_grid(c, n);
    const dim3 g2(grid, ransac_lm_groups(c, grid, T));
    const bool core = core_flags != nullptr && round == 0;
    int rc = lm_launch(c, g2, KMAX, q, u, a, ak, n, hyp, T, states, partials, round, tol, core ? core_flags : nullptr, kTiledFusedBase, core,
                       core ? m9_flag : nullptr, m9_epoch);
    if (rc != RSDSFM_OK) return rc;
    hipLaunchKernelGGL(ransac_lm_rows_kernel, dim3(T), dim3(256), 0, c->stream, partials, grid, T, states, round, rows,
                       static_cast<const int*>(core ? core_flags : nullptr));
    RSDSFM_HIP_CHECK(c, hipGetLastError());
    return RSDSFM_OK;
}

int ransac_rows_payload_doubles(int T, bool core_trailer) { return T * NSR + (core_trailer ? 2 : 0); }

int ransac_decide_rows_launch(Ctx* c, const double* rows_all, int nranks, int T, LmState* states, int64_t n_total, int round,
                              int* flags, int* scored, double* trial_count, double* trial_err, bool core_trailer, double* cnt_rt, int cnt_stride) {
    if (cnt_rt && nranks > 256) return fail(c, RSDSFM_ERR_INVALID, "more than 256 ranks");
    RSDSFM_HIP_CHECK(c, hipMemsetAsync(flags, 0, sizeof(int), c->stream));
    hipLaunchKernelGGL(ransac_decide_kernel, dim3(T), dim3(256), 0, c->stream, rows_all, nranks, T, 0, states, n_total, round, (int)KMAX, flags,
                       static_cast<int*>(nullptr), scored, trial_count, trial_err, kTiledFusedBase, static_cast<int*>(nullptr),
                       static_cast<int*>(nullptr), core_trailer ? T * NSR / 2 + 1 : 0, cnt_rt, cnt_stride);
    RSDSFM_HIP_CHECK(c, hipGetLastError());
    return RSDSFM_OK;
}

int ransac_score_rows_launch(Ctx* c, const double* q, const double* u, const double* a, const double* ak, int64_t n,
                             const double* hyp, int T, const LmState* states, int depth_mode, double tol, const int* scored,
                             double* partials, double* rows) {
    const int grid = ransac_pixel_grid(c, n);
    const int groups = ransac_lm_groups(c, grid, T);
    hipLaunchKernelGGL(ransac_score_kernel, dim3(((grid + 7) / 8) * 8 * groups), dim3(kRB), sizeof(double) * T * 2, c->stream,
                       reinterpret_cast<const double2*>(q), reinterpret_cast<const double2*>(u), a, ak, n, hyp, T, states,
                       depth_mode, tol, scored, partials, grid, groups, static_cast<const int*>(nullptr), static_cast<const int*>(nullptr));
    RSDSFM_HIP_CHECK(c, hipGetLastError());
    hipLaunchKernelGGL(ransac_score_rows_kernel, dim3(T), dim3(256), 0, c->stream, partials, grid, T, scored, rows);
    RSDSFM_HIP_CHECK(c, hipGetLastError());
    return RSDSFM_OK;
}

int ransac_score_merge_launch(Ctx* c, const double* rows_all, int nranks, int T, const int* scored, double* trial_count,
                              double* trial_err, double* cnt_rt, int cnt_stride) {
    if (cnt_rt && nranks > 256) return fail(c, RSDSFM_ERR_INVALID, "more than 256 ranks");
    hipLaunchKernelGGL(ransac_reduce_scores_kernel, dim3(T), dim3(256), 0, c->stream, rows_all, nranks, T, scored, trial_count,
                       trial_err, cnt_rt, cnt_stride);
    RSDSFM_HIP_CHECK(c, hipGetLastError());
    return RSDSFM_OK;
}

int ransac_rows_doubles() { return NSR; }

int ransac_pick_launch(Ctx* c, const double* trial_count, const double* trial_err, int T, const double* hyp, RansacBest* best,
                       RansacBest* best_host, const int* d_flags, int* h_flags, int scored_ahead, const double* cnt_rt, int cnt_stride,
                       int nranks, int64_t* m_all, double tie_margin, PickLazy lazy) {
    hipLaunchKernelGGL(ransac_pick_kernel, dim3(1), dim3(64), 0, c->stream, trial_count, trial_err, T, hyp, best, best_host, d_flags, h_flags, scored_ahead,
                       cnt_rt, cnt_stride, nranks, m_all, tie_margin, lazy);
    RSDSFM_HIP_CHECK(c, hipGetLastError());
    return RSDSFM_OK;
}

int ransac_final_launch(Ctx* c, const double* q, const double* u, const double* a, const double* ak, int64_t n,
                        RansacBest* best, const LmState* states, int depth_mode, double tol, double* rho, uint8_t* mask,
                        int64_t* block_counts, int64_t* block_offsets, int64_t* inlier_idx, double* inliers,
                        double* out_alpha, double* out_alpha_k, RansacBest* best_host, int* zero_words) {
    int64_t blocks = (n + kRB - 1) / kRB;
    if (blocks < 1) blocks = 1;
    const int64_t cap = 2048;
    int64_t chunk = kRB;
    if (blocks > cap) {
        chunk = ((blocks + cap - 1) / cap) * kRB;
        blocks = (n + chunk - 1) / chunk;
    }
    hipLaunchKernelGGL(ransac_final_kernel, dim3((int)blocks), dim3(kRB), 0, c->stream, reinterpret_cast<const double2*>(q),
                       reinterpret_cast<const double2*>(u), a, ak, n, chunk, best, states, depth_mode, tol, rho, mask,
                       block_counts);
    RSDSFM_HIP_CHECK(c, hipGetLastError());
    if (inlier_idx || inliers || out_alpha || out_alpha_k) {
        hipLaunchKernelGGL(ransac_scatter_kernel, dim3((int)blocks), dim3(kRB), 0, c->stream, reinterpret_cast<const double2*>(q),
                           a, ak, n, chunk, rho, mask, block_counts, best, best_host, inlier_idx, inliers, out_alpha, out_alpha_k, zero_words);
    } else {
        if (zero_words) RSDSFM_HIP_CHECK(c, hipMemsetAsync(zero_words, 0, kRefineStateBlockTail, c->stream));
        hipLaunchKernelGGL(ransac_scan_kernel, dim3(1), dim3(256), 0, c->stream, block_counts, (int)blocks, block_offsets, best, best_host);
    }
    RSDSFM_HIP_CHECK(c, hipGetLastError());
    return RSDSFM_OK;
}

}
```

rs-aware-differential-sfm_amd/csrc/refine_host.hip:

```cpp
#include <string.h>

#include <algorithm>

#include "rsdsfm_internal.hpp"

namespace rsdsfm {

int refine_begin(Ctx* c, const double* d_flow, int64_t n_flow, int64_t m, const double* d_inl, const double* d_alpha,
                 const double* d_alpha_k, const int64_t* d_inlier_idx, const double v_in[3], const double w_in[3], double k_in,
                 int const_acceleration, int flow_index_mode, double* d_inl_out, const RefineTail* tail, const RansacBest* d_best,
                 void* ws_base, RefineRun* run, RefineState* hs_prefetch, double* d_zpartials, bool exact, const FinishClaim* claim) {
    if (m < 0 || n_flow < 0 || (!d_best && (!v_in || !w_in))) return fail(c, RSDSFM_ERR_INVALID, "bad arguments");
    if (flow_index_mode != RSDSFM_FLOW_COMPAT_RANK && flow_index_mode != RSDSFM_FLOW_GATHERED) return fail(c, RSDSFM_ERR_INVALID, "unknown flow_index_mode");
    if (flow_index_mode == RSDSFM_FLOW_GATHERED && m > 0 && !d_inlier_idx) return fail(c, RSDSFM_ERR_INVALID, "gathered mode needs inlier_idx");
    if (m > 0 && (!d_flow || !d_inl || !d_alpha || !d_alpha_k || !d_inl_out)) return fail(c, RSDSFM_ERR_INVALID, "null device pointer");
    const int np = const_acceleration ? 7 : 6;
    const size_t M = (size_t)std::max<int64_t>(m, 1);
    const size_t npart = (size_t)(d_best ? refine_partials_doubles_cap(c) : refine_partials_doubles(c, m));
    int rc = RSDSFM_OK;
    if (!ws_base) {
        rc = ensure_ws(c, refine_workspace_bytes(c, m, d_best != nullptr));
        if (rc != RSDSFM_OK) return rc;
        ws_base = c->d_ws;
    }
    rc = ensure_pinned(c, sizeof(RefineState) + 64);
    if (rc != RSDSFM_OK) return rc;
    Arena ws(ws_base);
    RefineBuffers& B = run->B;
    B = RefineBuffers();
    B.flow = d_flow;
    B.n_flow = n_flow;
    B.m = m;
    B.m_on_device = d_best != nullptr;
    B.inl = d_inl;
    B.alpha = d_alpha;
    B.alpha_k = d_alpha_k;
    B.inlier_idx = d_inlier_idx;
    B.flow_index_mode = flow_index_mode;
    static_assert(sizeof(RefineState) % sizeof(int) == 0, "flag follows the state");
    char* state_block = ws.take<char>(sizeof(RefineState) + 64);
    B.state = reinterpret_cast<RefineState*>(state_block);
    B.uu = ws.take<double>(4 * M);
    B.beta = ws.take<double>(M);
    B.rho_a = ws.take<double>(M);
    B.rho_b = ws.take<double>(M);
    B.srho = ws.take<double>(M);
    B.partials = ws.take<double>(npart);
    B.bad_index = reinterpret_cast<int*>(state_block + sizeof(RefineState));
    B.zpartials = d_zpartials;
    if (claim && claim->on && d_zpartials) B.claim = *claim;
    run->np = np;
    run->rf = !exact && c->lm_arithmetic == 0 && c->refine_arithmetic == 0;
    if (run->rf) c->refine_rf_runs += 1;
    run->d_inl_out = d_inl_out;
    run->tail = tail;
    run->launched = 0;
    run->hint_prev = c->refine_iters_hint;
    run->hs = hs_prefetch ? hs_prefetch : static_cast<RefineState*>(c->h_pinned);
    run->prefetch = hs_prefetch != nullptr;
    run->prefetched = false;
    B.state_host = hs_prefetch;
    if (d_best && claim && claim->on && run->rf && !c->refine_stage_separate) {
        B.best_dev = d_best;
    } else if (d_best) {
        rc = refine_state_from_best_launch(c, d_best, B, np);
        if (rc != RSDSFM_OK) return rc;
    } else {
        RefineState* hs = static_cast<RefineState*>(c->h_pinned);
        int* h_bad = reinterpret_cast<int*>(static_cast<char*>(c->h_pinned) + sizeof(RefineState));
        memset(hs, 0, sizeof(RefineState));
        hs->np = np;
        for (int i = 0; i < 3; ++i) {
            hs->p[i] = v_in[i];
            hs->p[3 + i] = w_in[i];
        }
        hs->p[6] = k_in;
        hs->termination = -1;
        hs->radius = kInitialRadius;
        hs->need_schur = 1;
        memset(h_bad, 0, kRefineStateBlockTail);
        RSDSFM_HIP_CHECK(c, hipMemcpyAsync(B.state, hs, sizeof(RefineState) + kRefineStateBlockTail, hipMemcpyHostToDevice, c->stream));
    }
    rc = refine_trace_reset(c);
    if (rc != RSDSFM_OK) return rc;
    if (!run->rf) {
        rc = refine_init_launch(c, B, np);
        if (rc != RSDSFM_OK) return rc;
    }
    const int hp = run->hint_prev;
    run->chunk = (hp >= 0 && hp <= 3) ? hp + 1 : (hp > 8 ? std::min(hp + 1, 28) : 7);
    return refine_enqueue_chunk(c, run);
}

int refine_enqueue_chunk(Ctx* c, RefineRun* run) {
    static const bool watch = getenv("RSDSFM_SYNC_WATCHDOG_S") != nullptr;
    if (watch) {
        const RefineBuffers B = run->B;
        const int launched = run->launched, chunk = run->chunk, rf = run->rf ? 1 : 0;
        set_sync_dumper([B, launched, chunk, rf](Ctx* cc) {
            fprintf(stderr, "[rsdsfm] last refinement chunk enqueued: slots [%d, %d), radius-factorised %d\n", launched, launched + chunk, rf);
            refine_rf_debug_dump(cc, B);
        });
    }
    if (run->rf) {
        for (int i = 0; i <= run->chunk; ++i) {
            const int g = run->launched + i;
            int rc = refine_rf_pass_launch(c, run->B, run->np, g, run->launched, nullptr, 0, -1, nullptr, i == run->chunk);
            if (rc != RSDSFM_OK) return rc;
        }
        run->launched += 1;
    } else {
        for (int i = 0; i < run->chunk; ++i) {
            int rc = refine_iter_launch(c, run->B, run->np, i, run->chunk);
            if (rc != RSDSFM_OK) return rc;
        }
    }
    run->launched += run->chunk;
    int rc = RSDSFM_OK;
    if (run->B.claim.on) {
        FinishClaim& C = run->B.claim;
        const int64_t npix = (int64_t)C.rows * C.cols;
        if (run->B.m >= ((int64_t)1 << 31)) return fail(c, RSDSFM_ERR_INVALID, "depth map: more than 2^31 inliers");
        rc = claim_map_acquire(c, 2, (size_t)std::max<int64_t>(std::max<int64_t>(npix, run->B.m), 1), &C.owner, &C.tag, &C.mask);
        if (rc != RSDSFM_OK) return rc;
    }
    rc = refine_finish_launch(c, run->B, run->d_inl_out);
    if (rc != RSDSFM_OK) return rc;
    run->tail_done = false;
    if (run->tail && !(run->hint_prev > run->launched + 1)) {
        rc = (*run->tail)(run->B);
        run->tail_done = true;
    }
    if (rc != RSDSFM_OK) return rc;
    if (run->prefetch) run->prefetched = true;
    return rc;
}

int refine_poll(Ctx* c, RefineRun* run, double v_out[3], double w_out[3], double* k_out, rsdsfm_lm_summary* summary) {
    if (!v_out || !w_out || !k_out) return fail(c, RSDSFM_ERR_INVALID, "bad arguments");
    RefineState* hs = run->hs;
    int* h_bad = reinterpret_cast<int*>(reinterpret_cast<char*>(hs) + sizeof(RefineState));
    for (bool first = true;; first = false) {
        if (!(first && run->prefetch && run->prefetched)) {
            if (!run->prefetch) RSDSFM_HIP_CHECK(c, hipMemcpyAsync(hs, run->B.state, sizeof(RefineState) + sizeof(int), hipMemcpyDeviceToHost, c->stream));
            if (int rcs = sync_stream(c, "refine_poll line 168")) return rcs;
        }
// ... 164 lines not shown
```

rs-aware-differential-sfm_amd/csrc/refine_kernels.hip:

```cpp
#include "refine_common.hpp"

namespace rsdsfm {


template <int NP>
__global__ __launch_bounds__(kFB) void refine_init_kernel(const double2* __restrict__ flow, int64_t n_flow, int64_t m,
                                                         const double* __restrict__ inl, const double* __restrict__ alpha,
                                                         const double* __restrict__ alpha_k,
                                                         const int64_t* __restrict__ inlier_idx, int flow_index_mode,
                                                         const RefineState* __restrict__ st, double4* __restrict__ xyuv,
                                                         double* __restrict__ beta_out, double* __restrict__ rho0,
                                                         double* __restrict__ srho, double* __restrict__ partials,
                                                         int* __restrict__ bad_index, int want_zsum) {
    using CT = Counts<NP>;
    __shared__ double s_red[kFB / 64][CT::NINIT];
    const PassShape ps = pass_shape(st, m);
    if (!ps.live) return;
    m = ps.m;
    double p[7];
#pragma unroll
    for (int c = 0; c < 7; ++c) p[c] = st->p[c];
    double acc[CT::NINIT];
#pragma unroll
    for (int s = 0; s < CT::NINIT; ++s) acc[s] = 0.0;
// ... 356 lines not shown
        return 0;
    }
    const double rel = cost_change / model_change;
    if (tr) tr[4] = rel;
    if (rel > kMinRelDecrease) {
        double gmax = s[CT::BACK_MAX], xsq = s[CT::BACK_MAX + 1];
        for (int c = 0; c < 7; ++c) st->p[c] = st->pc[c];
        for (int c = 0; c < NP; ++c) {
            xsq += st->p[c] * st->p[c];
            if (fabs(s[4 + c]) > gmax) gmax = fabs(s[4 + c]);
        }
        st->cur ^= 1;
        st->zsum = s[CT::BACK_MAX + 2];
        st->cost = 0.5 * s[3];
        st->gmax = gmax;
        st->x_norm = sqrt(xsq);
        st->radius = radius_accept(st->radius, rel);
        st->decrease_factor = 2.0;
        st->num_successful += 1;
        if (gmax <= kGradientTol) st->termination = RSDSFM_TERM_GRADIENT;
        if (tr) tr[7] = gmax <= kGradientTol ? RSDSFM_TRACE_ACCEPTED_GRADIENT_TOL : RSDSFM_TRACE_ACCEPTED;
    } else {
        if (tr) tr[7] = RSDSFM_TRACE_REJECTED;
        st->num_unsuccessful += 1;
        st->radius = st->radius / st->decrease_factor;
        st->decrease_factor *= 2.0;
    }
    return st->termination < 0 && st->num_successful > successful_before ? 1 : 0;
}

template <int NP>
__global__ __launch_bounds__(kFB) void refine_decide_kernel(const double* __restrict__ partials, int nblocks,
                                                           RefineState* st, double* __restrict__ trace, int trace_rows) {
    using CT = Counts<NP>;
    __shared__ double s_red[kFB / 64][CT::NBACK];
    __shared__ double s[CT::NBACK];
    if (st->termination >= 0) return;
    const int solve_ok = st->solve_ok;
    if (solve_ok) reduce_partials<CT::NBACK>(partials, nblocks >= 0 ? nblocks : st->grid, CT::BACK_MAX, s_red, s);
    if (threadIdx.x != 0) return;
    (void)decide_serial<NP>(st, s, solve_ok, trace, trace_rows);
}

__global__ __launch_bounds__(kFB) void refine_finish_kernel(int64_t m, const double* __restrict__ inl,
                                                           const double* __restrict__ rho_a, const double* __restrict__ rho_b,
                                                           const RefineState* __restrict__ st, double* __restrict__ inl_out,
                                                           double* __restrict__ zpartials, RefineState* __restrict__ state_host,
                                                           const int* __restrict__ bad_index) {
    __shared__ double s_red[kFB / 64];
    if (state_host && blockIdx.x == 0) {
        static_assert(sizeof(RefineState) % 8 == 0, "copied as 8-byte words");
        for (int i = threadIdx.x; i < (int)(sizeof(RefineState) / 8); i += kFB)
            reinterpret_cast<double*>(state_host)[i] = reinterpret_cast<const double*>(st)[i];
        if (threadIdx.x == 0) *reinterpret_cast<int*>(reinterpret_cast<char*>(state_host) + sizeof(RefineState)) = *bad_index;
    }
    const double* __restrict__ rho = st->cur ? rho_b : rho_a;
    if (m < 0) m = st->m;
    const int64_t stride = (int64_t)gridDim.x * kFB;
    double acc = 0.0;
    for (int64_t i = (int64_t)blockIdx.x * kFB + threadIdx.x; i < m; i += stride) {
        inl_out[3 * i] = inl[3 * i];
        inl_out[3 * i + 1] = inl[3 * i + 1];
        const double z = 1.0 / rho[i];
        inl_out[3 * i + 2] = z;
        acc += z;
    }
    if (zpartials) {
        const double r = wave_sum(acc);
        if ((threadIdx.x & 63) == 0) s_red[threadIdx.x >> 6] = r;
        __syncthreads();
        if (threadIdx.x == 0) {
            double t = s_red[0];
            for (int w2 = 1; w2 < kFB / 64; ++w2) t += s_red[w2];
            zpartials[blockIdx.x] = t;
        }
    }
}

__global__ __launch_bounds__(kFB) void refine_finish_claim_kernel(int64_t m, const double* __restrict__ inl, const double* __restrict__ rho_a,
                                                                 const double* __restrict__ rho_b, const RefineState* __restrict__ st,
                                                                 double* __restrict__ inl_out, double* __restrict__ zpartials,
                                                                 RefineState* __restrict__ state_host, const int* __restrict__ bad_index,
                                                                 double fx, double fy, double cx, double cy, int rows, int ncols,
                                                                 unsigned* __restrict__ owner, unsigned tag, int32_t* __restrict__ ys) {
    __shared__ double s_red[kFB / 64];
    if (state_host && blockIdx.x == 0) {
        for (int i = threadIdx.x; i < (int)(sizeof(RefineState) / 8); i += kFB)
            reinterpret_cast<double*>(state_host)[i] = reinterpret_cast<const double*>(st)[i];
        if (threadIdx.x == 0) *reinterpret_cast<int*>(reinterpret_cast<char*>(state_host) + sizeof(RefineState)) = *bad_index;
    }
    const double* __restrict__ rho = st->cur ? rho_b : rho_a;
    if (m < 0) m = st->m;
    const int64_t stride = (int64_t)gridDim.x * kFB;
    double acc = 0.0;
    for (int64_t i = (int64_t)blockIdx.x * kFB + threadIdx.x; i < m; i += stride) {
        const double xn = inl[3 * i], yn = inl[3 * i + 1];
        inl_out[3 * i] = xn;
        inl_out[3 * i + 1] = yn;
        const double z = 1.0 / rho[i];
        inl_out[3 * i + 2] = z;
        acc += z;
        const int x = (int)(fx * xn + cx + 0.5);
        const int y = (int)(fy * yn + cy + 0.5);
        ys[i] = y;
        if (x >= 0 && x < ncols && y >= 0 && y < rows) atomicMax(&owner[(int64_t)x * rows + y], tag | (unsigned)i);
    }
    const double r = wave_sum(acc);
    if ((threadIdx.x & 63) == 0) s_red[threadIdx.x >> 6] = r;
    __syncthreads();
    if (threadIdx.x == 0) {
        double t = s_red[0];
        for (int w2 = 1; w2 < kFB / 64; ++w2) t += s_red[w2];
        zpartials[blockIdx.x] = t;
    }
}

__global__ void refine_state_from_best_kernel(const RansacBest* __restrict__ best, RefineState* __restrict__ st, int np, int cap,
                                              int* __restrict__ bad_index) {
    if (threadIdx.x != 0 || blockIdx.x != 0) return;
    RefineState z;
    memset(&z, 0, sizeof(z));
    z.np = np;
    for (int i = 0; i < 3; ++i) {
        z.p[i] = best->hyp[3 + i];
        z.p[3 + i] = best->hyp[i];
    }
    z.p[6] = best->hyp[6];
    z.termination = -1;
    z.radius = kInitialRadius;
    z.need_schur = 1;
    const int64_t m = best->undecided ? 0 : best->num_inliers_scan;
    z.m = m;
    int64_t b = (m + kFB - 1) / kFB;
    if (b < 1) b = 1;
    if (b > cap) {
        const int64_t iters = (b + cap - 1) / cap;
        b = (b + iters - 1) / iters;
    }
    z.grid = (int)b;
    *st = z;
    bad_index[0] = 0;
    bad_index[4] = bad_index[5] = bad_index[6] = 0;
}

static inline int refine_grid_cap(const Ctx* c) { return c->num_cus * kWorkgroupsPerCu; }
static inline int refine_grid(const Ctx* c, int64_t m) {
    int64_t b = (m + kFB - 1) / kFB;
    const int64_t cap = (int64_t)c->num_cus * kWorkgroupsPerCu;
    if (b < 1) b = 1;
    if (b > cap) {
        const int64_t iters = (b + cap - 1) / cap;
        b = (b + iters - 1) / iters;
    }
    return (int)b;
}

static inline int refine_partials_half(const Ctx* c) { return refine_grid_cap(c) * SlotRow<7>::NW; }
constexpr int kStateDoubles = (int)((sizeof(RefineState) + 63) / 64 * 8);
int refine_partials_doubles_cap(const Ctx* c) { return 2 * refine_partials_half(c) + 2 * kStateDoubles + 8 + refine_rf_extra_doubles(); }
int refine_partials_half_doubles(const Ctx* c) { return refine_partials_half(c); }
int refine_state_doubles() { return kStateDoubles; }
int refine_partials_doubles(const Ctx* c, int64_t m) { (void)m; return refine_partials_doubles_cap(c); }
static inline double* rows_buffer(const Ctx* c, const RefineBuffers& B, int which) { return B.partials + (size_t)(which & 1) * refine_partials_half(c); }
static inline RefineState* chunk_state(const Ctx* c, const RefineBuffers& B, int which) {
    return reinterpret_cast<RefineState*>(B.partials + 2 * (size_t)refine_partials_half(c) + (size_t)(which & 1) * kStateDoubles);
}
static inline const RefineState* slot_state_in(const Ctx* c, const RefineBuffers& B, int j) { return j == 0 ? B.state : chunk_state(c, B, j - 1); }

int refine_state_from_best_launch(Ctx* c, const RansacBest* d_best, const RefineBuffers& B, int np) {
    hipLaunchKernelGGL(refine_state_from_best_kernel, dim3(1), dim3(64), 0, c->stream, d_best, B.state, np, refine_grid_cap(c), B.bad_index);
    RSDSFM_HIP_CHECK(c, hipGetLastError());
    return RSDSFM_OK;
}

template <int NP>
static int refine_init_t(Ctx* c, const RefineBuffers& B) {
    const int grid = B.m_on_device ? refine_grid_cap(c) : refine_grid(c, B.m);
    const int64_t m_arg = B.m_on_device ? -1 : B.m;
    hipLaunchKernelGGL(refine_init_kernel<NP>, dim3(grid), dim3(kFB), 0, c->stream, reinterpret_cast<const double2*>(B.flow), B.n_flow,
// ... 255 lines not shown
        st->need_schur = 0;
    }
}

template <int NP>
__global__ __launch_bounds__(kFB) void refine_slot_apply_kernel(const double* __restrict__ rows_all, int nranks, const RefineState* __restrict__ st_in,
                                                               RefineState* __restrict__ st_out, double* __restrict__ trace, int trace_rows) {
    __shared__ RefineState s_state;
    state_to_lds(&s_state, st_in);
    RefineState* st = &s_state;
    if (st->termination < 0 && st->pending_apply) slot_apply_body<NP>(st, rows_all, nranks >= 0 ? nranks : st->grid, trace, trace_rows);
    __syncthreads();
    if (threadIdx.x == 0) st->pending_apply = 0;
    __syncthreads();
    state_from_lds(st_out, st);
}

template <int NP>
static int refine_iter_t(Ctx* c, const RefineBuffers& B, int j, int chunk) {
    const int grid = B.m_on_device ? refine_grid_cap(c) : refine_grid(c, B.m);
    const int64_t m_arg = B.m_on_device ? -1 : B.m;
    const int nb_arg = B.m_on_device ? -1 : grid;
    hipLaunchKernelGGL(refine_slot_pass_kernel<NP>, dim3(grid), dim3(kFB), 0, c->stream, m_arg, reinterpret_cast<const double4*>(B.uu), B.beta,
                       B.alpha, B.alpha_k, B.rho_a, B.rho_b, B.srho, slot_state_in(c, B, j), chunk_state(c, B, j), rows_buffer(c, B, j - 1), nb_arg,
                       rows_buffer(c, B, j), B.want_zsum ? 1 : 0, c->d_refine_trace, c->refine_trace_rows);
    RSDSFM_HIP_CHECK(c, hipGetLastError());
    const bool separate = c->refine_stage_mode == 2 || (c->refine_stage_mode == 0 && (c->refine_stage_separate || frames_in_flight(c) > 1));
    if (j == chunk - 1 || separate) {
        hipLaunchKernelGGL(refine_slot_apply_kernel<NP>, dim3(1), dim3(kFB), 0, c->stream, rows_buffer(c, B, j), nb_arg, chunk_state(c, B, j),
                           j == chunk - 1 ? B.state : chunk_state(c, B, j), c->d_refine_trace, c->refine_trace_rows);
        RSDSFM_HIP_CHECK(c, hipGetLastError());
    }
    return RSDSFM_OK;
}

template <int NP>
static int refine_slot_rows_t(Ctx* c, const RefineBuffers& B, double* row, int j, const double* rows_all_prev, int nranks) {
    const int grid = B.m_on_device ? refine_grid_cap(c) : refine_grid(c, B.m);
    hipLaunchKernelGGL(refine_slot_pass_kernel<NP>, dim3(grid), dim3(kFB), 0, c->stream, B.m_on_device ? (int64_t)-1 : B.m, reinterpret_cast<const double4*>(B.uu), B.beta, B.alpha,
                       B.alpha_k, B.rho_a, B.rho_b, B.srho, slot_state_in(c, B, j), chunk_state(c, B, j), rows_all_prev, nranks, rows_buffer(c, B, 0),
                       B.want_zsum ? 1 : 0, c->d_refine_trace, c->refine_trace_rows);
    RSDSFM_HIP_CHECK(c, hipGetLastError());
    hipLaunchKernelGGL(refine_slot_row_kernel<NP>, dim3(1), dim3(kFB), 0, c->stream, rows_buffer(c, B, 0), B.m_on_device ? -1 : grid, row,
                       static_cast<const RefineState*>(B.state));
    RSDSFM_HIP_CHECK(c, hipGetLastError());
    return RSDSFM_OK;
}
int refine_slot_row_doubles(int np) { return np == 7 ? SlotRow<7>::NW : SlotRow<6>::NW; }
int refine_slot_partials_doubles(const Ctx* c, int64_t m) { return refine_partials_doubles(c, m); }
int refine_slot_rows_launch(Ctx* c, const RefineBuffers& B, int np, double* row, int j, const double* rows_all_prev, int nranks) {
    return np == 7 ? refine_slot_rows_t<7>(c, B, row, j, rows_all_prev, nranks) : refine_slot_rows_t<6>(c, B, row, j, rows_all_prev, nranks);
}
int refine_slot_apply_launch(Ctx* c, const RefineBuffers& B, int np, const double* rows_all, int nranks, int chunk) {
    if (np == 7)
        hipLaunchKernelGGL(refine_slot_apply_kernel<7>, dim3(1), dim3(kFB), 0, c->stream, rows_all, nranks, chunk_state(c, B, chunk - 1), B.state,
                           c->d_refine_trace, c->refine_trace_rows);
    else
        hipLaunchKernelGGL(refine_slot_apply_kernel<6>, dim3(1), dim3(kFB), 0, c->stream, rows_all, nranks, chunk_state(c, B, chunk - 1), B.state,
                           c->d_refine_trace, c->refine_trace_rows);
    RSDSFM_HIP_CHECK(c, hipGetLastError());
    return RSDSFM_OK;
}

int refine_stage_row_doubles(int np, int stage) {
    if (np == 7) return stage == 0 ? Counts<7>::NINIT : stage == 1 ? Counts<7>::NSCHUR : Counts<7>::NBACK;
    return stage == 0 ? Counts<6>::NINIT : stage == 1 ? Counts<6>::NSCHUR : Counts<6>::NBACK;
}
int refine_stage_rows_launch(Ctx* c, const RefineBuffers& B, int np, int stage, double* row) {
    return np == 7 ? refine_stage_rows_t<7>(c, B, stage, row) : refine_stage_rows_t<6>(c, B, stage, row);
}
int refine_stage_apply_launch(Ctx* c, const RefineBuffers& B, int np, int stage, const double* rows_all, int nranks, int64_t m_total, const int64_t* m_total_dev) {
    return np == 7 ? refine_stage_apply_t<7>(c, B, stage, rows_all, nranks, m_total, m_total_dev)
                   : refine_stage_apply_t<6>(c, B, stage, rows_all, nranks, m_total, m_total_dev);
}

int refine_init_launch(Ctx* c, const RefineBuffers& B, int np) { return np == 7 ? refine_init_t<7>(c, B) : refine_init_t<6>(c, B); }
int refine_iter_launch(Ctx* c, const RefineBuffers& B, int np, int j, int chunk) { return np == 7 ? refine_iter_t<7>(c, B, j, chunk) : refine_iter_t<6>(c, B, j, chunk); }

int refine_finish_grid(const Ctx* c, const RefineBuffers& B) { return B.m_on_device ? refine_grid_cap(c) : refine_grid(c, B.m); }

int refine_finish_launch(Ctx* c, const RefineBuffers& B, double* inl_out) {
    if (!B.m_on_device && B.m == 0 && !B.zpartials && !B.state_host) return RSDSFM_OK;
    if (B.claim.on) {
        hipLaunchKernelGGL(refine_finish_claim_kernel, dim3(refine_finish_grid(c, B)), dim3(kFB), 0, c->stream, B.m_on_device ? (int64_t)-1 : B.m, B.inl,
                           B.rho_a, B.rho_b, B.state, inl_out, B.zpartials, B.state_host, B.bad_index, B.claim.fx, B.claim.fy, B.claim.cx, B.claim.cy,
                           B.claim.rows, B.claim.cols, B.claim.owner, B.claim.tag, B.claim.ys);
        RSDSFM_HIP_CHECK(c, hipGetLastError());
        return RSDSFM_OK;
    }
    hipLaunchKernelGGL(refine_finish_kernel, dim3(refine_finish_grid(c, B)), dim3(kFB), 0, c->stream,
                       B.m_on_device ? (int64_t)-1 : B.m, B.inl, B.rho_a, B.rho_b, B.state, inl_out, B.zpartials, B.state_host, B.bad_index);
    RSDSFM_HIP_CHECK(c, hipGetLastError());
    return RSDSFM_OK;
}

}
```

rs-aware-differential-sfm_amd/csrc/refine_rf_kernels.hip:

```cpp
#include "refine_common.hpp"

#ifndef RF_LOADS_ONLY
#define RF_LOADS_ONLY 0
#endif
#ifndef RF_NP7_PREFETCH
#define RF_NP7_PREFETCH 0
#endif

namespace rsdsfm {

namespace {

constexpr int kRfListCap = 64;
constexpr int kRfEntry = 8;

template <int NP>
struct RfRow {
    static constexpr int TRI = NP * (NP + 1) / 2;
    static constexpr int OFF_JTJ = 0, OFF_B = TRI, OFF_JTB = 2 * TRI, OFF_C = 2 * TRI + NP;
    static constexpr int NSCHUR = 2 * TRI + 2 * NP;
    static constexpr int MODEL = NSCHUR, STEPSQ = NSCHUR + 1, COST2 = NSCHUR + 2, XSQ = NSCHUR + 3, ZSUM = NSCHUR + 4, GMAX = NSCHUR + 5;
    static constexpr int NW = NSCHUR + 6;
    static constexpr int NF = TRI + NP;
    static_assert(NW % 2 == 0, "rows are read as double2");
// ... 512 lines not shown
            if (tid < RR::NF) {
                double f = L.fe[0][tid];
                for (int e = 1; e < n; ++e) f += L.fe[e][tid];
                L.F[tid] = f;
            }
            __syncthreads();
        }
        if (tid == 0) {
            const int rc = rf_solve<NP>(st, L.cur, L.F, n > 0, radius);
            int again = 0;
            if (rc < 0) {
                rf_restart(st, kRfGuardPivot);
            } else if (rc == 0) {
                double* tr = (trace && st->iteration >= 1 && st->iteration <= trace_rows) ? trace + (int64_t)(st->iteration - 1) * kRefineTraceCols : nullptr;
                if (tr) {
                    tr[0] = (double)st->iteration, tr[1] = st->cost, tr[3] = 0.0, tr[5] = st->radius, tr[7] = RSDSFM_TRACE_INVALID;
                    tr[2] = tr[4] = tr[6] = __builtin_nan("");
                }
                st->num_unsuccessful += 1;
                st->invalid_run += 1;
                if (st->invalid_run >= kMaxInvalid)
                    st->termination = RSDSFM_TERM_FAILURE;
                else
                    st->radius *= 0.5, again = 1;
            } else if (resolve) {
                st->rf_resolves += 1;
            }
            st->solve_ok = rc == 1 ? 1 : 0;
            L.loop = again;
        }
        __syncthreads();
        RF_BEAT(21);
        const int again = L.loop;
        __syncthreads();
        if (!again) break;
        resolve = true;
    }
    RF_BEAT(30);
    if (ext_out) {
        if (tid < RR::NSCHUR) ext_out->sums[tid] = L.cur[tid];
        const int n = L.nlist;
        for (int q = tid; q < n * kRfEntry; q += kFB) ext_out->list[q] = L.list[q];
        if (tid == 0) ext_out->nlist = (double)n;
    }
    RF_BEAT(31);
#undef RF_BEAT
}

struct RfPassArgs {
    int64_t m;
    const double4* xyuv_in;
    double4* xyuv_out;
    double* beta;
    const double* alpha;
    const double* alpha_k;
    double* rho_a;
    double* rho_b;
    const RefineState* st_in;
    RefineState* st_out;
    const double* rows_prev;
    int nrows_prev, row_stride;
    RfLists lists_prev;
    int* list_count;
    double* list_entries;
    int* list_count_zero;
    const RfExt* ext_in;
    RfExt* ext_out;
    double* partials;
    double* trace;
    int trace_rows;
    int64_t m_total;
    const int64_t* m_total_dev;
    const double2* flow;
    int64_t n_flow;
    const double* inl;
    const int64_t* inlier_idx;
    int flow_index_mode;
    int* bad_index;
    unsigned long long* beat;
    int slot;
    const RansacBest* best;
    int grid_cap;
    unsigned long long* stamps;
};

struct RfLoad {
    double4 c4;
    double rho, ab, ak;
};
template <int NP>
__device__ __forceinline__ RfLoad rf_load(const RfPassArgs& A, const double* __restrict__ rho, int64_t i, bool live) {
    RfLoad l;
    l.c4 = make_double4(0.0, 0.0, 0.0, 0.0), l.rho = 0.0, l.ab = 0.0, l.ak = 0.0;
    if (live) {
        l.c4 = A.xyuv_in[i];
        l.rho = rho[i];
        if (NP == 6) {
            l.ab = A.beta[i];
        } else {
            l.ab = A.alpha[i], l.ak = A.alpha_k[i];
        }
    }
    return l;
}

}

template <int NP, bool FIRST, bool ZSUM>
__global__ __launch_bounds__(kFB) void refine_rf_pass_kernel(const RfPassArgs A) {
    using RR = RfRow<NP>;
    __shared__ RfStageLds<NP> s_stage;
    __shared__ double s_red[kFB / 64][RR::NW];
    __shared__ RefineState s_state;
    const bool stamp = A.stamps && blockIdx.x == 0 && threadIdx.x == 0;
    if (A.beat && threadIdx.x == 0) {
        if (A.beat[7]) atomicAdd(&A.beat[2], 1ull);
        if (blockIdx.x == 0) A.beat[0] = ((unsigned long long)A.slot << 8) | 1;
        if (blockIdx.x < 512) A.beat[8 + blockIdx.x] = ((unsigned long long)A.slot << 8) | 1;
    }
    __shared__ unsigned long long tk[8];
    if (stamp) {
#pragma unroll
        for (int i = 0; i < 8; ++i) tk[i] = 0;
    }
    if (stamp) tk[0] = wall_clock64();
    if (FIRST && A.best) {
        if (threadIdx.x < sizeof(RefineState) / 8) reinterpret_cast<unsigned long long*>(&s_state)[threadIdx.x] = 0ull;
        __syncthreads();
        if (threadIdx.x == 0) {
            RefineState& z = s_state;
            z.np = NP;
            for (int i = 0; i < 3; ++i) {
                z.p[i] = A.best->hyp[3 + i];
                z.p[3 + i] = A.best->hyp[i];
            }
            z.p[6] = A.best->hyp[6];
            z.termination = -1;
            z.radius = kInitialRadius;
            z.need_schur = 1;
            const int64_t mb = A.best->undecided ? 0 : A.best->num_inliers_scan;
            z.m = mb;
            int64_t b = (mb + kFB - 1) / kFB;
            if (b < 1) b = 1;
            if (b > A.grid_cap) {
                const int64_t iters = (b + A.grid_cap - 1) / A.grid_cap;
                b = (b + iters - 1) / iters;
            }
            z.grid = (int)b;
        }
        __syncthreads();
    } else {
        state_to_lds(&s_state, A.st_in);
    }
    RefineState* st = &s_state;
    if (stamp) tk[1] = wall_clock64();
    if (FIRST) {
        if (threadIdx.x < 7) st->p0[threadIdx.x] = st->p[threadIdx.x];
        if (threadIdx.x == 0) st->rf = 1, st->rf_guard = 0, st->rf_resolves = 0, st->pending_apply = 0;
        __syncthreads();
    } else if (st->termination < 0 && st->pending_apply) {
        int64_t mt = A.m_total_dev ? *A.m_total_dev : (A.m_total >= 0 ? A.m_total : (A.m >= 0 ? A.m : st->m));
        rf_apply_body<NP>(st, s_stage, A.rows_prev, A.nrows_prev >= 0 ? A.nrows_prev : st->grid, A.row_stride, A.lists_prev, A.ext_in,
                          blockIdx.x == 0 ? A.ext_out : nullptr, mt, blockIdx.x == 0 ? A.trace : nullptr, A.trace_rows, stamp ? tk + 4 : nullptr);
        __syncthreads();
    }
    if (threadIdx.x == 0) st->pending_apply = st->termination < 0 ? 1 : 0;
    __syncthreads();
    if (stamp) tk[2] = wall_clock64();
    if (A.beat && threadIdx.x == 0) {
        if (blockIdx.x == 0) A.beat[0] = ((unsigned long long)A.slot << 8) | 2;
        if (blockIdx.x < 512) A.beat[8 + blockIdx.x] = ((unsigned long long)A.slot << 8) | ((st->termination >= 0 || (A.m < 0 && (int)blockIdx.x >= st->grid)) ? 9 : 2);
        if (A.beat[7] && (st->termination >= 0 || (A.m < 0 && (int)blockIdx.x >= st->grid))) atomicAdd(&A.beat[3], 1ull);
    }
    if (blockIdx.x == 0) {
        state_from_lds(A.st_out, st);
        if (threadIdx.x == 0) *A.list_count_zero = 0;
    }
    if (st->termination >= 0) return;
    const PassShape ps = pass_shape(st, A.m);
    if (!ps.live) return;
    const int64_t m = ps.m;
    double acc[RR::NW];
#pragma unroll
    for (int s = 0; s < RR::NW; ++s) acc[s] = 0.0;
    constexpr bool kLdsC = NP == 7 && !FIRST;
    __shared__ double s_cacc[kLdsC ? 3 * NP : 1][kLdsC ? kFB : 1];
    double* const lds_c = kLdsC ? &s_cacc[0][threadIdx.x] : nullptr;
    if (kLdsC) {
#pragma unroll
        for (int a = 0; a < 3 * NP; ++a) lds_c[a * kFB] = 0.0;
    }
    const int64_t stride = (int64_t)ps.grid * kFB;
    const int64_t i0 = (int64_t)blockIdx.x * kFB + threadIdx.x;
    RfPoint P0q = rf_point(st->p0);
    const RfPoint P0 = rf_point_uniform(P0q);
    if (FIRST) {
        RfPoint Pq = rf_point(st->p);
        const RfPoint P = rf_point_uniform(Pq);
        for (int64_t i = i0; i < m; i += stride) {
            int64_t fi = (A.flow_index_mode == RSDSFM_FLOW_GATHERED) ? A.inlier_idx[i] : i;
            if (fi < 0 || fi >= A.n_flow) {
                *A.bad_index = 1;
                fi = 0;
            }
            const double2 f = A.flow[fi];
            const double x = A.inl[3 * i], y = A.inl[3 * i + 1];
            const double rho = 1.0 / A.inl[3 * i + 2];
            const double al = A.alpha[i], ak = A.alpha_k[i];
            A.xyuv_out[i] = make_double4(x, y, f.x, f.y);
            const double ab = NP == 6 ? P.c1 * __builtin_fma(P.k, ak, al) : al;
            if (NP == 6) A.beta[i] = ab;
            A.rho_a[i] = rho;
            const RfGeom g = rf_geom(x, y);
            double be, dbe;
            rf_beta<NP>(ab, ak, P, be, dbe);
            RfEval<NP> o;
            rf_resid<NP>(g, f.x, f.y, be, P, rho, o);
            rf_jac<NP>(g, be, dbe, rho, o);
            acc[RR::COST2] = __builtin_fma(o.r0, o.r0, __builtin_fma(o.r1, o.r1, acc[RR::COST2]));
            acc[RR::GMAX] = fmax(acc[RR::GMAX], fabs(__builtin_fma(o.J0, o.r0, o.J1 * o.r1)));
            acc[RR::XSQ] = __builtin_fma(rho, rho, acc[RR::XSQ]);
            if (ZSUM) acc[RR::ZSUM] += 1.0 / rho;
            const bool flagged = rf_flagged(o.h, o.h);
            const double ihm = flagged ? 0.0 : rcp_core(flagged ? 1.0 : o.h);
            rf_schur_accumulate<NP>(o, ihm, acc);
            if (flagged) rf_list_append(A.list_count, A.list_entries, x, y, f.x, f.y, ab, ak, rho, i);
        }
    } else {
        RfPoint Pq = rf_point(st->p), Pcq = rf_point(st->pc);
        const RfPoint P = rf_point_uniform(Pq), Pc = rf_point_uniform(Pcq);
        double dp[7];
#pragma unroll
        for (int c = 0; c < 7; ++c) dp[c] = uniform_d(st->dp[c]);
        const double inv_radius = uniform_d(1.0 / st->radius);
        const double psi = uniform_d(1.0 / (1.0 + 1.0 / st->radius));
        const double* __restrict__ rho = st->cur ? A.rho_b : A.rho_a;
        double* __restrict__ cand = st->cur ? A.rho_a : A.rho_b;
        auto body = [&](const RfLoad& l0, int64_t i) {
            const double x = l0.c4.x, y = l0.c4.y, ux = l0.c4.z, uy = l0.c4.w, rh = l0.rho;
            const RfGeom g = rf_geom(x, y);
            double be, dbe, bec, dbec, be0, dbe0;
            rf_beta<NP>(l0.ab, l0.ak, P, be, dbe);
            rf_beta<NP>(l0.ab, l0.ak, Pc, bec, dbec);
            rf_beta<NP>(l0.ab, l0.ak, P0, be0, dbe0);
            RfEval<NP> o;
            rf_resid<NP>(g, ux, uy, be, P, rh, o);
            double da0, da1, db0, db1;
            rf_av(g, dp[0], dp[1], dp[2], da0, da1);
            rf_bw(g, dp[3], dp[4], dp[5], db0, db1);
            double t0 = be * __builtin_fma(rh, da0, db0), t1 = be * __builtin_fma(rh, da1, db1);
            if (NP == 7) {
                const double dk = dbe * dp[6];
                t0 = __builtin_fma(dk, o.in0, t0);
                t1 = __builtin_fma(dk, o.in1, t1);
            }
            double a00, a10;
            rf_av(g, P0.v0, P0.v1, P0.v2, a00, a10);
            const double h0 = (be0 * be0) * __builtin_fma(a00, a00, a10 * a10);
            const double gJ = __builtin_fma(o.J0, o.r0, o.J1 * o.r1), tJ = __builtin_fma(o.J0, t0, o.J1 * t1);
            const bool flagged = rf_flagged(o.h, h0);
            double drho = -((psi * (gJ + tJ)) * rcp_core(flagged ? 1.0 : o.h));
            if (__builtin_amdgcn_ballot_w64(flagged) != 0) {
                if (flagged) {
                    asm volatile("; listed inlier: exact e-block inverse" ::: "memory");
                    double sr, E0, E1;
                    const double ete_inv = rf_ete_inv_exact(o.J0, o.J1, h0, inv_radius, sr, E0, E1);
                    drho = -((ete_inv * (sr * (gJ + tJ))) * sr);
                }
            }
            const double m0 = __builtin_fma(o.J0, drho, t0), m1 = __builtin_fma(o.J1, drho, t1);
            acc[RR::MODEL] -= __builtin_fma(m0, __builtin_fma(0.5, m0, o.r0), m1 * __builtin_fma(0.5, m1, o.r1));
            const double cd = rh + drho;
            cand[i] = cd;
            acc[RR::STEPSQ] = __builtin_fma(drho, drho, acc[RR::STEPSQ]);
            RfEval<NP> oc;
            rf_resid<NP>(g, ux, uy, bec, Pc, cd, oc);
            rf_jac<NP>(g, bec, dbec, cd, oc);
            acc[RR::COST2] = __builtin_fma(oc.r0, oc.r0, __builtin_fma(oc.r1, oc.r1, acc[RR::COST2]));
            acc[RR::GMAX] = fmax(acc[RR::GMAX], fabs(__builtin_fma(oc.J0, oc.r0, oc.J1 * oc.r1)));
            acc[RR::XSQ] = __builtin_fma(cd, cd, acc[RR::XSQ]);
            if (ZSUM) acc[RR::ZSUM] += 1.0 / cd;
            const bool flagged_c = rf_flagged(oc.h, h0);
            const double ihm = flagged_c ? 0.0 : rcp_core(flagged_c ? 1.0 : oc.h);
            rf_schur_accumulate<NP>(oc, ihm, acc, lds_c);
            if (flagged_c) rf_list_append(A.list_count, A.list_entries, x, y, ux, uy, l0.ab, l0.ak, cd, i);
        };
        const int64_t last = m - 1;
        if (NP == 6) {
            RfLoad l0 = rf_load<NP>(A, rho, i0, i0 <= last);
            RfLoad l1 = rf_load<NP>(A, rho, i0 + stride, i0 + stride <= last);
            for (int64_t i = i0; i < m; i += stride) {
                const int64_t i2 = i + 2 * stride;
                const RfLoad l2 = rf_load<NP>(A, rho, i2, i2 <= last);
#if RF_LOADS_ONLY
                acc[0] += l0.c4.x + l0.c4.y + l0.c4.z + l0.c4.w + l0.rho + l0.ab;
                cand[i] = l0.rho;
#else
                body(l0, i);
#endif
                l0 = l1;
                l1 = l2;
            }
        } else {
#if RF_NP7_PREFETCH == 1
            RfLoad l0 = rf_load<NP>(A, rho, i0, i0 <= last);
            for (int64_t i = i0; i < m; i += stride) {
                const RfLoad l1 = rf_load<NP>(A, rho, i + stride, i + stride <= last);
                body(l0, i);
                l0 = l1;
// ... 89 lines not shown
int refine_rf_row_doubles(int np) { return (np == 7 ? RfRow<7>::NW : RfRow<6>::NW) + kRfListDoubles; }

namespace {
static_assert(kWorkgroupsPerCu == 1, "rf_grid_cap and the cap of RefineState::grid (refine_state_from_best_kernel) agree only at one workgroup per CU");
inline int rf_grid_cap(const Ctx* c) { return c->num_cus; }
inline int rf_grid(const Ctx* c, int64_t m) {
    int64_t b = (m + kFB - 1) / kFB;
    const int64_t cap = rf_grid_cap(c);
    if (b < 1) b = 1;
    if (b > cap) {
        const int64_t iters = (b + cap - 1) / cap;
        b = (b + iters - 1) / iters;
    }
    return (int)b;
}
struct RfLayout {
    double* rows[2];
    RefineState* cs[2];
    double* list[3];
    RfExt* ext[2];
};
static_assert(RfRow<7>::NW <= SlotRow<7>::NW && RfRow<6>::NW <= SlotRow<7>::NW, "the rows buffer is sized by SlotRow<7>::NW doubles per workgroup");
inline RfLayout rf_layout(const Ctx* c, const RefineBuffers& B) {
    RfLayout Lo;
    double* base = B.partials;
    const size_t half = (size_t)refine_partials_half_doubles(c);
    Lo.rows[0] = base, Lo.rows[1] = base + half;
    double* p = base + 2 * half;
    const size_t sd = (size_t)refine_state_doubles();
    Lo.cs[0] = reinterpret_cast<RefineState*>(p), Lo.cs[1] = reinterpret_cast<RefineState*>(p + sd);
    p += 2 * sd + 8;
    for (int i = 0; i < 3; ++i) Lo.list[i] = p + (size_t)i * kRfListCap * kRfEntry;
    p += 3 * kRfListCap * kRfEntry;
    Lo.ext[0] = reinterpret_cast<RfExt*>(p), Lo.ext[1] = reinterpret_cast<RfExt*>(p + kRfExtDoubles);
    return Lo;
}
inline int rf_mod3(int g) { return ((g % 3) + 3) % 3; }
inline int* rf_list_count(const RefineBuffers& B, int g) { return refine_rf_counters(B) + rf_mod3(g); }
inline double* rf_list_entries(const RfLayout& Lo, int g) { return Lo.list[rf_mod3(g)]; }
inline RfLists rf_lists_of(const RfLayout& Lo, const RefineBuffers& B, int g, const double* rows_all, int nranks, int nw) {
    RfLists l;
    if (rows_all) {
        l.counts = reinterpret_cast<const int*>(rows_all + nw), l.count_stride = 2 * (nw + kRfListDoubles);
        l.entries = rows_all + nw + 2, l.entry_stride = nw + kRfListDoubles, l.nlists = nranks;
    } else {
        l.counts = rf_list_count(B, g), l.count_stride = 0, l.entries = rf_list_entries(Lo, g), l.entry_stride = 0, l.nlists = 1;
    }
    return l;
}

struct RfBeat {
    const Ctx* c;
    unsigned long long* words;
};
RfBeat g_beats[32];
int g_nbeats = 0;
unsigned long long* rf_beat(Ctx* c) {
    static const bool on = getenv("RSDSFM_SYNC_WATCHDOG_S") != nullptr && getenv("RSDSFM_NO_BEAT") == nullptr;
    if (!on) return nullptr;
    for (int i = 0; i < g_nbeats; ++i)
        if (g_beats[i].c == c) return g_beats[i].words;
    if (g_nbeats >= 32) return nullptr;
    unsigned long long* w = nullptr;
    if (hipHostMalloc((void**)&w, 64 + 8 * 512, hipHostMallocDefault) != hipSuccess) return nullptr;
    for (int i = 0; i < 8 + 512; ++i) w[i] = 0;
    w[7] = getenv("RSDSFM_BEAT_COUNT_WORKGROUPS") ? 1 : 0;
    g_beats[g_nbeats].c = c, g_beats[g_nbeats].words = w;
    ++g_nbeats;
    return w;
}
unsigned long long* rf_stamps(Ctx* c) {
    static int on = -1;
    static unsigned long long* buf = nullptr;
    if (on < 0) {
        const char* e = getenv("RSDSFM_RF_STAMPS");
        on = (e && e[0] == '1') ? 1 : 0;
        if (on && (hipMalloc(&buf, 128) != hipSuccess || hipMemset(buf, 0, 128) != hipSuccess)) buf = nullptr;
    }
    (void)c;
    return buf;
}
template <int NP, bool ZSUM>
void rf_pass_launch_t(Ctx* c, const RfPassArgs& A, bool first, int grid) {
    if (first)
        hipLaunchKernelGGL((refine_rf_pass_kernel<NP, true, ZSUM>), dim3(grid), dim3(kFB), 0, c->stream, A);
    else
        hipLaunchKernelGGL((refine_rf_pass_kernel<NP, false, ZSUM>), dim3(grid), dim3(kFB), 0, c->stream, A);
}
}

int refine_rf_pass_launch(Ctx* c, const RefineBuffers& B, int np, int g, int g_first, const double* rows_all_prev, int nranks, int64_t m_total,
                          const int64_t* m_total_dev, bool publish) {
    const RfLayout Lo = rf_layout(c, B);
    const int grid = B.m_on_device ? rf_grid_cap(c) : rf_grid(c, B.m);
    const int nw = np == 7 ? RfRow<7>::NW : RfRow<6>::NW;
    RfPassArgs A = {};
    A.m = B.m_on_device ? -1 : B.m;
    A.xyuv_in = reinterpret_cast<const double4*>(B.uu);
    A.xyuv_out = reinterpret_cast<double4*>(B.uu);
    A.beta = B.beta;
    A.alpha = B.alpha;
    A.alpha_k = B.alpha_k;
    A.rho_a = B.rho_a;
    A.rho_b = B.rho_b;
    A.st_in = g == g_first ? B.state : Lo.cs[(g - 1) & 1];
    A.st_out = publish ? B.state : Lo.cs[g & 1];
    if (rows_all_prev)
        A.rows_prev = rows_all_prev, A.nrows_prev = nranks, A.row_stride = nw + kRfListDoubles;
    else
        A.rows_prev = Lo.rows[(g - 1) & 1], A.nrows_prev = B.m_on_device ? -1 : grid, A.row_stride = nw;
    A.lists_prev = rf_lists_of(Lo, B, g - 1, rows_all_prev, nranks, nw);
    A.list_count = rf_list_count(B, g);
    A.list_entries = rf_list_entries(Lo, g);
    A.list_count_zero = rf_list_count(B, g + 1);
    A.ext_in = Lo.ext[(g - 1) & 1];
    A.ext_out = Lo.ext[g & 1];
    A.partials = Lo.rows[g & 1];
    A.trace = c->d_refine_trace;
    A.trace_rows = c->refine_trace_rows;
    A.m_total = m_total;
    A.m_total_dev = m_total_dev;
    A.flow = reinterpret_cast<const double2*>(B.flow);
    A.n_flow = B.n_flow;
    A.inl = B.inl;
    A.inlier_idx = B.inlier_idx;
    A.flow_index_mode = B.flow_index_mode;
    A.bad_index = B.bad_index;
    A.best = g == 0 ? B.best_dev : nullptr;
    A.grid_cap = rf_grid_cap(c);
    A.stamps = rf_stamps(c);
    A.beat = rf_beat(c);
    A.slot = g;
    const bool first = g == 0;
    if (np == 7) {
        if (B.want_zsum) rf_pass_launch_t<7, true>(c, A, first, grid); else rf_pass_launch_t<7, false>(c, A, first, grid);
    } else {
        if (B.want_zsum) rf_pass_launch_t<6, true>(c, A, first, grid); else rf_pass_launch_t<6, false>(c, A, first, grid);
    }
    RSDSFM_HIP_CHECK(c, hipGetLastError());
    return RSDSFM_OK;
}

int refine_rf_apply_launch(Ctx* c, const RefineBuffers& B, int np, int g, bool to_published, const double* rows_all, int nranks, int64_t m_total,
                           const int64_t* m_total_dev) {
    const RfLayout Lo = rf_layout(c, B);
    const int grid = B.m_on_device ? rf_grid_cap(c) : rf_grid(c, B.m);
    const int nw = np == 7 ? RfRow<7>::NW : RfRow<6>::NW;
    const double* rows = rows_all ? rows_all : Lo.rows[g & 1];
    const int nrows = rows_all ? nranks : (B.m_on_device ? -1 : grid);
    const int stride = rows_all ? nw + kRfListDoubles : nw;
    const RfLists lists = rf_lists_of(Lo, B, g, rows_all, nranks, nw);
    RefineState* st_io = Lo.cs[g & 1];
    if (np == 7)
        hipLaunchKernelGGL(refine_rf_apply_kernel<7>, dim3(1), dim3(kFB), 0, c->stream, rows, nrows, stride, lists, st_io, to_published ? B.state : st_io,
                           Lo.ext[g & 1], Lo.ext[(g + 1) & 1], m_total, m_total_dev, c->d_refine_trace, c->refine_trace_rows, rf_beat(c), g);
    else
        hipLaunchKernelGGL(refine_rf_apply_kernel<6>, dim3(1), dim3(kFB), 0, c->stream, rows, nrows, stride, lists, st_io, to_published ? B.state : st_io,
                           Lo.ext[g & 1], Lo.ext[(g + 1) & 1], m_total, m_total_dev, c->d_refine_trace, c->refine_trace_rows, rf_beat(c), g);
    RSDSFM_HIP_CHECK(c, hipGetLastError());
    return RSDSFM_OK;
}

int refine_rf_row_launch(Ctx* c, const RefineBuffers& B, int np, int g, double* row) {
    const RfLayout Lo = rf_layout(c, B);
    const int grid = B.m_on_device ? rf_grid_cap(c) : rf_grid(c, B.m);
    if (np == 7)
        hipLaunchKernelGGL(refine_rf_row_kernel<7>, dim3(1), dim3(kFB), 0, c->stream, Lo.rows[g & 1], B.m_on_device ? -1 : grid, static_cast<const RefineState*>(Lo.cs[g & 1]),
                           rf_list_count(B, g), rf_list_entries(Lo, g), row);
    else
        hipLaunchKernelGGL(refine_rf_row_kernel<6>, dim3(1), dim3(kFB), 0, c->stream, Lo.rows[g & 1], B.m_on_device ? -1 : grid, static_cast<const RefineState*>(Lo.cs[g & 1]),
                           rf_list_count(B, g), rf_list_entries(Lo, g), row);
    RSDSFM_HIP_CHECK(c, hipGetLastError());
    return RSDSFM_OK;
}

void refine_rf_debug_dump(Ctx* c, const RefineBuffers& B) {
    const RfLayout Lo = rf_layout(c, B);
    hipStream_t s2 = nullptr;
    if (hipStreamCreateWithFlags(&s2, hipStreamNonBlocking) != hipSuccess) return;
    RefineState h[3];
    int cnt[8] = {0, 0, 0, 0, 0, 0, 0, 0};
    const RefineState* src[3] = {B.state, Lo.cs[0], Lo.cs[1]};
    for (int i = 0; i < 3; ++i) (void)hipMemcpyAsync(&h[i], src[i], sizeof(RefineState), hipMemcpyDeviceToHost, s2);
    (void)hipMemcpyAsync(cnt, B.bad_index, sizeof(int) * 8, hipMemcpyDeviceToHost, s2);
    if (hipStreamSynchronize(s2) != hipSuccess) {
        fprintf(stderr, "[rsdsfm] refinement dump: the copies did not complete either\n");
        return;
    }
    const char* names[3] = {"published", "chunk state 0", "chunk state 1"};
    for (int i = 0; i < 3; ++i)
        fprintf(stderr, "[rsdsfm] %s: np %d termination %d iteration %d slots %d pending_apply %d rf %d guard %d cur %d solve_ok %d m %lld grid %d radius %g cost %g successful %d unsuccessful %d invalid_run %d\n",
                names[i], h[i].np, h[i].termination, h[i].iteration, h[i].slots, h[i].pending_apply, h[i].rf, h[i].rf_guard, h[i].cur, h[i].solve_ok, (long long)h[i].m, h[i].grid, h[i].radius,
                h[i].cost, h[i].num_successful, h[i].num_unsuccessful, h[i].invalid_run);
    fprintf(stderr, "[rsdsfm] bad_index %d, list counters %d %d %d (m_on_device %d, m %lld)\n", cnt[0], cnt[4], cnt[5], cnt[6], (int)B.m_on_device, (long long)B.m);
    for (int i = 0; i < g_nbeats; ++i)
        fprintf(stderr, "[rsdsfm] context %p%s: last pass slot %llu phase %llu; pass workgroups started %llu, left %llu; last stage kernel slot %llu phase %llu\n", (const void*)g_beats[i].c, g_beats[i].c == c ? " (the waiting one)" : "",
                g_beats[i].words[0] >> 8, g_beats[i].words[0] & 255, g_beats[i].words[2], g_beats[i].words[3], g_beats[i].words[1] >> 8, g_beats[i].words[1] & 255);
    for (int i = 0; i < g_nbeats; ++i) {
        if (g_beats[i].c != c) continue;
        int hist[16] = {0};
        const unsigned long long last = g_beats[i].words[0] >> 8;
        fprintf(stderr, "[rsdsfm] workgroups of the waiting context's pass (slot %llu) not at phase 4 / 9:", last);
        for (int b = 0; b < 256; ++b) {
            const unsigned long long w = g_beats[i].words[8 + b];
            hist[w & 15] += 1;
            if ((w & 255) != 4 && (w & 255) != 9) fprintf(stderr, " [%d: slot %llu phase %llu]", b, w >> 8, w & 255);
        }
        fprintf(stderr, "\n[rsdsfm] phase histogram:");
        for (int p = 0; p < 10; ++p) fprintf(stderr, " %d:%d", p, hist[p]);
        fprintf(stderr, "\n");
    }
}

int refine_rf_read_stamps(Ctx* c, unsigned long long out[16]) {
    unsigned long long* b = rf_stamps(c);
    if (!b) return RSDSFM_ERR_INVALID;
// ... 8 lines not shown
```

rs-aware-differential-sfm_amd/csrc/rsdsfm_internal.hpp:

```cpp
#pragma once

#include <hip/hip_runtime.h>
#include <stdint.h>

#include <functional>
#include <string>
#include <vector>

#include "../../include/rsdsfm.h"

namespace rsdsfm {

constexpr int kMaxIter = 50;
constexpr int kRefineTraceCols = RSDSFM_REFINE_TRACE_COLS;
constexpr double kInitialRadius = 1e4;
constexpr double kMaxRadius = 1e16;
constexpr double kMinRadius = 1e-32;
constexpr double kMinRelDecrease = 1e-3;
constexpr double kMinLmDiag = 1e-6;
constexpr double kMaxLmDiag = 1e32;
constexpr double kFunctionTol = 1e-6;
constexpr double kGradientTol = 1e-10;
static_assert(kGradientTol < 1.0, "the indicator encoding of the gradient-maximum slots needs kGradientTol < 1");
constexpr double kParameterTol = 1e-8;
constexpr int kMaxInvalid = 5;
constexpr double kLmaTie = 1e-11;

constexpr int KMAX = 3;
constexpr int NS = 3 + 5 * KMAX;

struct Pose {
    double v[3];
    double w[3];
    double k;
};

struct LmScal {
    int32_t status;
    int32_t n_hist;
    int32_t K;
    int32_t write_which;
    int32_t iteration;
    int32_t num_successful;
    int32_t num_unsuccessful;
    int32_t invalid_run;
    int32_t termination;
    int32_t rho_holds;
    int32_t launches;
    int32_t next_launch;
    int32_t predict;
    int32_t restart;
    double radius;
    double decrease_factor;
    double cost;
    double initial_cost;
    double cand[KMAX];
};
struct LmState : LmScal {
    double hist[kMaxIter];
};

constexpr size_t kRefineStateBlockTail = 32;
struct RansacBest {
    int32_t best_trial;
    int32_t undecided;
    int64_t num_inliers;
    int64_t num_inliers_scan;
    double inlier_error;
    double hyp[8];
    int32_t lma_tie;
    int32_t shared_best;
    int32_t _pad_shared;
    int32_t lazy_pending;
};
struct PickLazy {
    int* scored = nullptr;
    int* list = nullptr;
    int* list_count = nullptr;
};

constexpr int kScoreIdleLimit = 4;
constexpr int kRansacBatch = 128;

struct Ctx {
    int device = 0;
    hipStream_t stream = nullptr;
    bool own_stream = false;
    std::string err;
    double* d_partials = nullptr;
    unsigned* d_tickets = nullptr;
    LmState* d_lm = nullptr;
    LmState* h_lm = nullptr;
    int lm_issued_k = 0;
    int true_flow_exhaustive = 0;
    int ransac_fused_base = 2;
    int ransac_score_idle = kScoreIdleLimit;
    int refine_iters_hint = -1;
    int ransac_standard_math = 0;
    int* d_core_flag = nullptr;
    int core_epoch = 0;
    int ransac_math_mode = 0;
    int64_t ransac_restarts = 0;
    int lm_arithmetic = 0;
    int lma_hold = 0;
    bool lma_count_only_force = false;
    int64_t lma_count_only_runs = 0, lma_lazy_runs = 0;
    int lma_unique_run = 0;
    int64_t lma_restarts = 0;
    int64_t lma_handed_over = 0;
    int lma_last_guard = 0;
    int* d_lma_list = nullptr;
    int depth_lma_parity = 0;
    int lma_cand[2] = {2, 1};
    int ransac_spec_miss = 0;
    int frame_dense_hint = 1;
    int lm_issued_d = 0;
    int depth_epoch = 0;
    int depth_standard_math = 0;
    int64_t depth_restarts = 0;
    int depth_core_launch = 0;
    int prof_what = 0;
    void* d_stage = nullptr;
    size_t stage_bytes = 0;
    void* d_ws = nullptr;
    size_t ws_bytes = 0;
    void* d_frame = nullptr;
    size_t frame_bytes = 0;
    void* h_pinned = nullptr;
    hipEvent_t ev_ready = nullptr;
    size_t pinned_bytes = 0;
    int num_cus = 256;
    int ransac_k0 = 0;
    int ransac_not_one_step = -1;
    bool profile = false;
    hipEvent_t ev_prof[2] = {nullptr, nullptr};
    unsigned long long* d_clk_probe = nullptr;
    bool prof_pending = false;
    double* d_refine_trace = nullptr;
    int refine_trace_rows = 0;
    int depth_variant = 0;
    void* d_tile = nullptr;
    size_t tile_bytes = 0;
    void* tile_session = nullptr;
    int tile_np = 0;
    void* flow_pair = nullptr;
    void* flow_clip = nullptr;
    int flow_batch = 0;
    void* flow_check = nullptr;
    void* link = nullptr;
    void* fuse = nullptr;
    void* rectify_dense = nullptr;
    unsigned* d_claim[3] = {nullptr, nullptr, nullptr};
    size_t claim_words[3] = {0, 0, 0};
    unsigned claim_epoch[3] = {0, 0, 0};
    void* dist = nullptr;
    void* frame_run = nullptr;
    hipStream_t aux_stream = nullptr;
    hipEvent_t ev_fork = nullptr, ev_join = nullptr, ev_seq = nullptr;
    int frame_side_flatten = 3;
    int frame_tail = 0;
    unsigned long long* d_flat_counters = nullptr;
    int seq_lanes = 0;
    int refine_stage_mode = 0;
    bool refine_stage_separate = false;
    int refine_arithmetic = 0;
    int64_t refine_rf_runs = 0, refine_rf_restarts = 0, refine_rf_resolves = 0;
    int refine_rf_last_guard = 0;
    struct RansacCache {
        uint64_t tag = 0, stage_gen = 0;
        const double *d_u = nullptr, *d_inl = nullptr, *d_alpha = nullptr, *d_alpha_k = nullptr;
        const int64_t* d_idx = nullptr;
        int64_t n = 0, m = 0;
        const void* h_u = nullptr;
        double u_probe[16] = {0};
        double inl_probe[16] = {0};
    } ransac_cache;
    uint64_t stage_gen = 0, ransac_tag_counter = 0;
    int64_t refine_cache_hits = 0;
    std::vector<rsdsfm_ctx*> lanes;
};
constexpr int kSequenceLanesDefault = 3;
void dist_release(Ctx* c);
void dist_reset_hold(Ctx* c);
void frame_release(Ctx* c);
void flow_release(Ctx* c);
void flow_check_release(Ctx* c);
void rectify_dense_release(Ctx* c);
void link_release(Ctx* c);
void fuse_release(Ctx* c);

constexpr int kDepthBlock = 256;
constexpr int kDepthMaxBlocks = 512;
constexpr int kDecideBlock = 256;
constexpr int kDepthBatchMax = 8;

#define RSDSFM_HIP_CHECK(ctx, expr)                                                            \
    do {                                                                                       \
        hipError_t _e = (expr);                                                                \
        if (_e != hipSuccess) {                                                                \
            (ctx)->err = std::string(#expr) + ": " + hipGetErrorString(_e);                    \
            return RSDSFM_ERR_HIP;                                                             \
        }                                                                                      \
    } while (0)

struct DeviceGuard {
    int prev = -1;
    bool switched = false;
    explicit DeviceGuard(const Ctx* c) {
        if (hipGetDevice(&prev) == hipSuccess && prev != c->device) switched = hipSetDevice(c->device) == hipSuccess;
    }
    ~DeviceGuard() {
        if (switched) (void)hipSetDevice(prev);
    }
    DeviceGuard(const DeviceGuard&) = delete;
    DeviceGuard& operator=(const DeviceGuard&) = delete;
};

int fail(Ctx* c, int code, const char* msg);
int ensure_stage(Ctx* c, size_t bytes);
struct XferItem {
    void* host;
    const void* dev;
    size_t bytes;
};
struct XferUp {
    void* dev;
    const void* host;
    size_t bytes;
};
int xfer_h2d(Ctx* c, void* d_dst, const void* h_src, size_t bytes);
int xfer_h2d_many(Ctx* c, const XferUp* items, int count);
int xfer_d2h(Ctx* c, void* h_dst, const void* d_src, size_t bytes);
int xfer_d2h_many(Ctx* c, const XferItem* items, int count);
bool xfer_trace_on();
void xfer_trace(const char* label);
void xfer_trace_span(const char* label, double us);
void xfer_trace_dump(const char* what);
int ensure_ws(Ctx* c, size_t bytes);
int sync_stream(Ctx* c, const char* where);
void set_sync_dumper(std::function<void(Ctx*)> f);
int ensure_pinned(Ctx* c, size_t bytes);

struct Arena {
// ... 26 lines not shown
int depth_lm_decide_rows_launch(Ctx* c, const double* d_rows, int nrows, int64_t n_total, int launch_id);
bool depth_lma_allowed(const Ctx* c, int64_t n);
int depth_lma_batch_launch(Ctx* const* cs, int count, const double* const* q, const double* const* u, const double* const* a,
                           const double* const* ak, const int64_t* n, const Pose* poses, double* const* rho);
int depth_lma_row_doubles();
int depth_lma_shard_launch(Ctx* c, const double* q, const double* u, const double* a, const double* ak, int64_t n, const Pose& pose, double* rho, double* d_row);
int depth_lma_shard_finish_launch(Ctx* c, const double* q, const double* u, const double* a, const double* ak, int64_t n, const Pose& pose, double* rho,
                                  const double* d_rows_all, int nranks, int64_t n_total);

}

namespace rsdsfm {
int alpha_launch(Ctx* c, const double* flow_px, int64_t n, double h, double gamma, double* alpha);
int alpha_k_launch(Ctx* c, const double* q_px, const double* flow_px, int64_t n, double h, double gamma, double* alpha_k);
int depth_map_device(Ctx* c, double* d_inl, int64_t m, double v_inout[3], double fx, double fy, double cx, double cy, int32_t rows, int32_t cols,
                     double* d_depth_map, int32_t* d_xs, int32_t* d_ys, int* flipped, const double* w_or_null, double k, double gamma,
                     double* d_R_rows9, double* d_t_rows3);
struct PoseTableOut {
    double* R = nullptr;
    double* t = nullptr;
    int rows = 0;
    double gamma = 0.0;
    const double* wk_dev = nullptr;
};
int pose_table_launch(Ctx* c, const Pose& pose, double gamma, int rows, double* R, double* t, const double* v_dev = nullptr,
                      const double* wk_dev = nullptr);
int64_t flatten_cells(int rows, int cols);
int flatten_launch(Ctx* c, const double* d_img, int rows, int cols, int col0, double fx, double fy, double cx, double cy,
                   double gamma, double thr, double* d_q, double* d_u, double* d_alpha, double* d_alpha_k, int64_t* d_counts,
                   int64_t* d_offsets, int64_t* d_total, hipEvent_t total_ready = nullptr);
int depth_map_launch(Ctx* c, double* d_inl, int64_t m, const double v[3], double fx, double fy, double cx, double cy, int rows,
                     int cols, double* d_depth_map, int32_t* d_xs, int32_t* d_ys, double* d_header, double* d_partials,
                     double* h_header = nullptr, const double* v_dev = nullptr, const int64_t* m_dev = nullptr,
                     const PoseTableOut* pt = nullptr);
int depth_map_slab_launch(Ctx* c, double* d_inl, int64_t m, const double* d_zsums, int nz, int64_t m_total, const double v[3],
                          double fx, double fy, double cx, double cy, int rows, int col0, int ncols, double* d_depth_map,
                          int32_t* d_xs, int32_t* d_ys, double* d_header, double* h_header = nullptr, const double* v_dev = nullptr,
                          const int64_t* m_dev = nullptr, const PoseTableOut* pt = nullptr);
int claim_map_acquire(Ctx* c, int which, size_t npix, unsigned** map, unsigned* tag, unsigned* mask);
int claim_map_reserve(Ctx* c, int which, size_t words);
int zsum_row_launch(Ctx* c, const double* d_inl, int64_t m, double* d_partials, double* d_out);
}

namespace rsdsfm {
struct Minimal9Direct {
    const double* img = nullptr;
    int rows = 0, cols = 0, alpha_ones = 0;
    double fx = 0, fy = 0, cx = 0, cy = 0, gamma = 0;
    int* core_flag = nullptr;
    int core_epoch = 0;
    double* probe = nullptr;
};
int minimal9_launch(Ctx* c, const double* q, const double* u, const double* alpha, const double* alpha_k,
                    const int32_t* samples, int T, int use_alpha_k, int k_sign_mode, double* hyp_out, void* zero_begin = nullptr,
                    size_t zero_bytes = 0, const Minimal9Direct* direct = nullptr);
struct DenseFlatten {
    double thr = 0.0;
    double *d_q = nullptr, *d_u = nullptr, *d_alpha = nullptr, *d_alpha_k = nullptr;
    unsigned long long* d_counters = nullptr;
    int64_t* total_out = nullptr;
};
int minimal9_flatten_launch(Ctx* c, const int32_t* samples, int T, int use_alpha_k, int k_sign_mode, double* hyp_out, void* zero_begin, size_t zero_bytes,
                            const Minimal9Direct& direct, double thr, double* d_q, double* d_u, double* d_alpha, double* d_alpha_k,
                            unsigned long long* d_counters, int64_t* total_out);
}

namespace rsdsfm {
int ransac_pixel_grid(const Ctx* c, int64_t n);
int ransac_lm_partials_doubles(const Ctx* c, int64_t n, int batch);
int ransac_lm_round_launch(Ctx* c, const double* q, const double* u, const double* a, const double* ak, int64_t n,
                           const double* hyp, int T, LmState* states, double* partials, int* flags, int* scored,
                           double* trial_count, double* trial_err, int round, double tol, int k0, int fused_base, bool core_math,
                           const int* m9_core_flag = nullptr, int m9_core_epoch = 0, int* unscored_list = nullptr);
int ransac_score_launch(Ctx* c, const double* q, const double* u, const double* a, const double* ak, int64_t n,
                        const double* hyp, int T, const LmState* states, int depth_mode, double tol, const int* scored,
                        double* partials, double* trial_count, double* trial_err, const int* unscored_list = nullptr, const int* unscored_count = nullptr);
int ransac_pick_launch(Ctx* c, const double* trial_count, const double* trial_err, int T, const double* hyp, RansacBest* best,
                       RansacBest* best_host = nullptr, const int* d_flags = nullptr, int* h_flags = nullptr, int scored_ahead = 0,
                       const double* cnt_rt = nullptr, int cnt_stride = 0, int nranks = 0, int64_t* m_all = nullptr, double tie_margin = 0.0,
                       PickLazy lazy = PickLazy());
int ransac_final_launch(Ctx* c, const double* q, const double* u, const double* a, const double* ak, int64_t n,
                        RansacBest* best, const LmState* states, int depth_mode, double tol, double* rho, uint8_t* mask,
                        int64_t* block_counts, int64_t* block_offsets, int64_t* inlier_idx, double* inliers,
                        double* out_alpha, double* out_alpha_k, RansacBest* best_host = nullptr, int* zero_words = nullptr);
int ransac_rows_doubles();
int ransac_lm_rows_launch(Ctx* c, const double* q, const double* u, const double* a, const double* ak, int64_t n,
                          const double* hyp, int T, const LmState* states, double* partials, int round, double tol, double* rows,
                          int* core_flags = nullptr, const int* m9_flag = nullptr, int m9_epoch = 0);
int ransac_rows_payload_doubles(int T, bool core_trailer);
int ransac_decide_rows_launch(Ctx* c, const double* rows_all, int nranks, int T, LmState* states, int64_t n_total, int round,
                              int* flags, int* scored, double* trial_count, double* trial_err, bool core_trailer = false,
                              double* cnt_rt = nullptr, int cnt_stride = 0);
int ransac_score_rows_launch(Ctx* c, const double* q, const double* u, const double* a, const double* ak, int64_t n,
                             const double* hyp, int T, const LmState* states, int depth_mode, double tol, const int* scored,
                             double* partials, double* rows);
int ransac_score_merge_launch(Ctx* c, const double* rows_all, int nranks, int T, const int* scored, double* trial_count,
                              double* trial_err, double* cnt_rt = nullptr, int cnt_stride = 0);
void sample_indices(int64_t n, int T, uint64_t seed, int32_t* out);
int64_t ransac_lma_partials_doubles(const Ctx* c, int64_t n, int batch);
size_t ransac_lma_list_ints(int batch);
int ransac_lma_launch(Ctx* c, const double* q, const double* u, const double* a, const double* ak, int64_t n, const double* hyp, int T,
                      LmState* states, double* partials, int* flags, int* scored, double* trial_count, double* trial_err, double tol,
                      const int* cand_steps, int ncand, int* irr_count, int* irr_list, int* unscored_list, int* guard_word,
                      const int* m9_core_flag = nullptr, int m9_core_epoch = 0, bool count_only = false);
int ransac_lma_rows_doubles();
int ransac_lma_rows_launch(Ctx* c, const double* q, const double* u, const double* a, const double* ak, int64_t n, const double* hyp, int T,
                           double* partials, double tol, const int* cand_steps, int ncand, int* irr_count, int* irr_list, double* rows);
int ransac_lma_decide_rows_launch(Ctx* c, const double* rows_all, int nranks, int64_t rank_stride, int T, int64_t n_total, const double* hyp,
                                  LmState* states, int* flags, int* scored, double* trial_count, double* trial_err, double tol, const int* cand_steps,
                                  int ncand, int* unscored_list, int* guard_word, double* cnt_rt, int cnt_stride, const int* m9_core_flag = nullptr,
                                  int m9_core_epoch = 0);
}

namespace rsdsfm {
struct RefineState {
    int32_t np, cur, iteration, invalid_run, num_successful, num_unsuccessful, termination, solve_ok;
    double p[7], pc[7], sp[7], yp[7];
    double radius, decrease_factor, cost, initial_cost, x_norm, gmax, stepsq_p;
    int64_t m;
    int32_t grid;
    int32_t need_schur;
    double zsum;
    int32_t slots;
    int32_t spec_miss_run;
    int32_t pending_apply;
    int32_t rf;
    double dp[7];
    double p0[7];
    int32_t rf_guard, rf_resolves;
};
constexpr int kTermRestartExact = 64;
struct FinishClaim {
    bool on = false;
    double fx = 0.0, fy = 0.0, cx = 0.0, cy = 0.0;
    int rows = 0, cols = 0;
    int32_t* ys = nullptr;
    unsigned* owner = nullptr;
    unsigned tag = 0, mask = 0;
};
struct RefineBuffers {
    const double* flow;
    int64_t n_flow, m;
    bool m_on_device = false;
    const double* inl;
    const double* alpha;
    const double* alpha_k;
    const int64_t* inlier_idx;
    int flow_index_mode;
    RefineState* state;
    double* uu;
    double* beta;
    double* rho_a;
    double* rho_b;
    double* srho;
    double* partials;
    int* bad_index;
    RefineState* state_host = nullptr;
    double* zpartials = nullptr;
    const RansacBest* best_dev = nullptr;
    FinishClaim claim;
    bool want_zsum = false;
};
size_t ransac_pinned_bytes(int T);
typedef std::function<int(const RansacBest*)> RansacSpecTail;
struct RansacRun {
    int pc = 0;
    const double *d_q = nullptr, *d_u = nullptr, *d_a = nullptr, *d_ak = nullptr;
    int64_t n = 0;
    int T = 0, Tn = 1, batch = 1, depth_mode = 0, use_alpha_k = 0, k_sign_mode = 0, k0 = 0, fused_base = 0;
    double tol = 0.0;
    rsdsfm_ransac_out* out = nullptr;
    const RansacSpecTail* spec_tail = nullptr;
    bool* spec_tail_held = nullptr;
    int core_epoch = 0;
    int* d_unscored = nullptr;
    bool core_math = true;
    bool analytic = false;
    bool lma_restarted = false;
    int* refine_flag_words = nullptr;
    bool count_only = false;
    int lazy_rounds = 0;
    int shared_best = 0;
    double tie_margin = 0.0;
    int lma_guard = 0;
    bool lma_tie_seen = false;
    int lma_cand[2] = {2, 1}, lma_cand_next[2] = {0, 0};
    int *d_irr_count = nullptr, *d_irr_list = nullptr;
    bool restarted = false;
    bool tail_ahead = true;
    const Minimal9Direct* direct = nullptr;
    const DenseFlatten* dense = nullptr;
    const std::function<int()>* after_minimal9 = nullptr;
    std::vector<int32_t> samples;
    double *d_hyp = nullptr, *d_partials = nullptr, *d_tcount = nullptr, *d_terr = nullptr, *d_rho = nullptr;
    char* zero_begin = nullptr;
    size_t zero_bytes = 0;
    LmState* d_states = nullptr;
    int *d_scored = nullptr, *d_flags = nullptr;
    RansacBest* d_best = nullptr;
    int64_t *d_bcounts = nullptr, *d_boffs = nullptr;
    uint8_t* d_mask = nullptr;
    RansacBest* h_best = nullptr;
    int* h_running = nullptr;
    double *h_tcount = nullptr, *h_terr = nullptr, *h_hyp = nullptr;
    LmState* h_states = nullptr;
    int32_t* h_samples_pinned = nullptr;
    int b0 = 0, B = 0, round = 0;
    bool need_score = true, final_done = false, spec_scored = false, tail_enqueued = false, spec_final = false;
    int not_one_step = 0, fused_base_next = 0, score_hint_next = -1;
    bool hints_ready = false;
};
int ransac_begin(Ctx* c, const double* d_q, const double* d_u, const double* d_a, const double* d_ak, int64_t n, int use_alpha_k, int T,
                 double tol, const int32_t* h_samples, uint64_t seed, int depth_mode, int k_sign_mode, rsdsfm_ransac_out* out,
                 const RansacSpecTail* spec_tail, bool* spec_tail_held, RansacRun* run, const Minimal9Direct* direct,
                 const std::function<int()>* after_minimal9, const DenseFlatten* dense = nullptr, bool tail_ahead = true, bool count_only = false,
                 int* refine_flag_words = nullptr);
int ransac_finish(Ctx* c, RansacRun* run);
void ransac_commit_hints(Ctx* c, const RansacRun& run);
int flatten_enqueue(Ctx* c, const double* d_img, int32_t rows, int32_t cols, double fx, double fy, double cx, double cy, double gamma,
                    double thr, double* d_q, double* d_u, double* d_alpha, double* d_alpha_k, int64_t* h_total);
typedef std::function<int(const RefineBuffers&)> RefineTail;
int refine_finish_grid(const Ctx* c, const RefineBuffers& B);
int depth_map_decided_launch(Ctx* c, double* d_inl, int64_t m, const double* d_zsums, int nz, const RefineBuffers& B, double* d_depth_map,
                             double* d_header, double* h_header, const double* v_dev, const int64_t* m_dev, const PoseTableOut* pt);
struct RefineRun {
    RefineBuffers B;
    int np = 6, launched = 0, chunk = 5, hint_prev = -1;
    bool rf = false;
    double* d_inl_out = nullptr;
    const RefineTail* tail = nullptr;
    RefineState* hs = nullptr;
    bool prefetch = false, prefetched = false;
    bool tail_done = false;
};
constexpr size_t kPinnedTail = 1024;
size_t refine_workspace_bytes(const Ctx* c, int64_t m, bool m_on_device);
int refine_begin(Ctx* c, const double* d_flow, int64_t n_flow, int64_t m, const double* d_inl, const double* d_alpha,
                 const double* d_alpha_k, const int64_t* d_inlier_idx, const double v_in[3], const double w_in[3], double k_in,
                 int const_acceleration, int flow_index_mode, double* d_inl_out, const RefineTail* tail, const RansacBest* d_best,
                 void* ws_base, RefineRun* run, RefineState* hs_prefetch, double* d_zpartials, bool exact = false,
                 const FinishClaim* claim = nullptr);
constexpr int kRcRefineRestartExact = 1;
int refine_device(Ctx* c, const double* d_flow, int64_t n_flow, int64_t m, const double* d_inl, const double* d_alpha,
                  const double* d_alpha_k, const int64_t* d_inlier_idx, const double v_in[3], const double w_in[3], double k_in,
                  int const_acceleration, int flow_index_mode, double* d_inl_out, double v_out[3], double w_out[3], double* k_out,
                  rsdsfm_lm_summary* summary, const RefineTail* tail, double* d_zpartials, bool exact = false, const FinishClaim* claim = nullptr);
int refine_enqueue_chunk(Ctx* c, RefineRun* run);
int frames_in_flight(const Ctx* c);
int refine_poll(Ctx* c, RefineRun* run, double v_out[3], double w_out[3], double* k_out, rsdsfm_lm_summary* summary);
int refine_partials_doubles(const Ctx* c, int64_t m);
int refine_partials_doubles_cap(const Ctx* c);
int refine_state_from_best_launch(Ctx* c, const RansacBest* d_best, const RefineBuffers& B, int np);
int* refine_flag_words(void* ws_base);
inline int refine_trace_reset(Ctx* c) {
    if (!c->d_refine_trace) return RSDSFM_OK;
    return hipMemsetAsync(c->d_refine_trace, 0xFF, (size_t)c->refine_trace_rows * kRefineTraceCols * sizeof(double), c->stream) == hipSuccess ? RSDSFM_OK : RSDSFM_ERR_HIP;
}
int refine_init_launch(Ctx* c, const RefineBuffers& B, int np);
int refine_rf_pass_launch(Ctx* c, const RefineBuffers& B, int np, int g, int g_first, const double* rows_all_prev, int nranks, int64_t m_total,
                          const int64_t* m_total_dev, bool publish = false);
int refine_rf_apply_launch(Ctx* c, const RefineBuffers& B, int np, int g, bool to_published, const double* rows_all, int nranks, int64_t m_total,
                           const int64_t* m_total_dev);
int refine_rf_row_launch(Ctx* c, const RefineBuffers& B, int np, int g, double* row);
int refine_rf_row_doubles(int np);
void refine_rf_debug_dump(Ctx* c, const RefineBuffers& B);
int refine_rf_read_stamps(Ctx* c, unsigned long long out[16]);
int refine_rf_extra_doubles();
int refine_partials_half_doubles(const Ctx* c);
int refine_state_doubles();
inline int* refine_rf_counters(const RefineBuffers& B) { return B.bad_index + 4; }
int refine_iter_launch(Ctx* c, const RefineBuffers& B, int np, int j, int chunk);
int refine_finish_launch(Ctx* c, const RefineBuffers& B, double* inl_out);
int refine_stage_row_doubles(int np, int stage);
int refine_slot_row_doubles(int np);
int refine_slot_partials_doubles(const Ctx* c, int64_t m);
int refine_slot_rows_launch(Ctx* c, const RefineBuffers& B, int np, double* row, int j, const double* rows_all_prev, int nranks);
int refine_slot_apply_launch(Ctx* c, const RefineBuffers& B, int np, const double* rows_all, int nranks, int chunk);
int refine_stage_rows_launch(Ctx* c, const RefineBuffers& B, int np, int stage, double* row);
int refine_stage_apply_launch(Ctx* c, const RefineBuffers& B, int np, int stage, const double* rows_all, int nranks, int64_t m_total,
                              const int64_t* m_total_dev = nullptr);
}

namespace rsdsfm {
int back_project_launch(Ctx* c, const unsigned char* d_img, const double* d_depth_cm, const double* d_R, const double* d_t, double fx,
                        double fy, double cx, double cy, int rows, int cols, int mode, int q5_mode, unsigned char* d_gs, float* d_c3d);
int interpolate_cracky_launch(Ctx* c, const unsigned char* d_in, int rows, int cols, int offset, unsigned char* d_out);
int rectify_frame_launch(Ctx* c, const double* d_inl, int64_t m, const unsigned char* d_img, const double* d_depth_cm, const double* d_R,
                         const double* d_t, double fx, double fy, double cx, double cy, int rows, int cols, int mode, int q5_mode, int offset,
                         unsigned char* d_preview, unsigned char* d_gs, float* d_c3d, unsigned char* d_fixed, double* d_partials);
int depth_preview_launch(Ctx* c, const double* d_inl, int64_t m, double fx, double fy, double cx, double cy, int rows, int cols,
                         unsigned char* d_out, double* d_partials);
}

struct rsdsfm_ctx {
    rsdsfm::Ctx c;
};
```

Baseline: 1755.

## Hand RANSAC inliers directly to first refinement pass, skipping scatter launch

The RANSAC final kernel now writes per-block compacted local inlier indices using ballot and prefix counts. The first refinement pass gathers inlier data straight from the pixel arrays through those indices and writes the inlier outputs itself, so the separate scatter kernel launch and its extra pass over memory are skipped. A fallback launches the scatter when refinement is not enqueued or has to restart in exact mode. The cost is an added barrier per block iteration in the final kernel and more complex first-pass loads, and the path only applies when several context conditions hold.

```diff
diff --git a/include/rsdsfm.h b/include/rsdsfm.h
--- a/include/rsdsfm.h
+++ b/include/rsdsfm.h
@@ -187,6 +187,7 @@
 int rsdsfm_set_sequence_lanes(rsdsfm_ctx* ctx, int32_t lanes);
 int rsdsfm_set_frame_side_flatten(rsdsfm_ctx* ctx, int mode);
 int rsdsfm_set_frame_tail(rsdsfm_ctx* ctx, int mode);
+int rsdsfm_set_frame_handoff(rsdsfm_ctx* ctx, int mode);
 int rsdsfm_ransac_dev(rsdsfm_ctx* ctx, const double* d_q2n, const double* d_u2n, const double* d_alpha_n,
                       const double* d_alpha_k_n, int64_t n, int use_alpha_k, int32_t iterations, double tolerance,
                       const int32_t* samples_9xT_or_null, uint64_t seed, int depth_mode, int k_sign_mode,
diff --git a/rs-aware-differential-sfm_amd/__init__.py b/rs-aware-differential-sfm_amd/__init__.py
--- a/rs-aware-differential-sfm_amd/__init__.py
+++ b/rs-aware-differential-sfm_amd/__init__.py
@@ -517,6 +517,9 @@
 
     def set_frame_tail(self, mode):
         self._check(self.lib.rsdsfm_set_frame_tail(self._ctx, int(mode)), "rsdsfm_set_frame_tail")
+
+    def set_frame_handoff(self, mode):
+        self._check(self.lib.rsdsfm_set_frame_handoff(self._ctx, int(mode)), "rsdsfm_set_frame_handoff")
 
     def prepared_frames_solve(self, jobs, trials=50, tol=0.05, use_acceleration_mode=False, use_refinement=True, depth_mode=DEPTH_CERES_LM,
                               k_sign_mode=K_COMPAT, flow_threshold=1e-10, flow_index_mode=FLOW_COMPAT_RANK, use_global_shutter_mode=False):
diff --git a/rs-aware-differential-sfm_amd/csrc/frame_host.hip b/rs-aware-differential-sfm_amd/csrc/frame_host.hip
--- a/rs-aware-differential-sfm_amd/csrc/frame_host.hip
+++ b/rs-aware-differential-sfm_amd/csrc/frame_host.hip
@@ -27,6 +27,7 @@
     int64_t* d_idx = nullptr;
     uint8_t* d_mask = nullptr;
     int32_t* d_ys = nullptr;
+    uint32_t* d_local_idx = nullptr;
     double *d_zpartials = nullptr, *d_zheader = nullptr;
     char* d_refine_ws = nullptr;
     rsdsfm_ransac_out ro;
@@ -94,7 +95,7 @@
     F->N = N;
     const size_t ncells = (size_t)flatten_cells(rows, cols);
     const size_t need = 2 * Arena::need(16 * N) + 4 * Arena::need(8 * N) + 2 * Arena::need(24 * N) + Arena::need(8 * N) + Arena::need(N) +
-                        Arena::need(4 * N) + Arena::need(8 * 1024) + Arena::need(64) + Arena::need(refine_workspace_bytes(c, (int64_t)N, true)) +
+                        2 * Arena::need(4 * N) + Arena::need(8 * 1024) + Arena::need(64) + Arena::need(refine_workspace_bytes(c, (int64_t)N, true)) +
                         2 * Arena::need(sizeof(int64_t) * (ncells + 2048)) + Arena::need(64) + 4096;
     if (need > c->frame_bytes) {
         RSDSFM_HIP_CHECK(c, hipStreamSynchronize(c->stream));
@@ -116,6 +117,7 @@
     F->d_idx = fa.take<int64_t>(N);
     F->d_mask = fa.take<uint8_t>(N);
     F->d_ys = fa.take<int32_t>(N);
+    uint32_t* d_local_idx = fa.take<uint32_t>(N);
     F->d_zpartials = fa.take<double>(1024);
     F->d_zheader = fa.take<double>(8);
     F->d_refine_ws = fa.take<char>(refine_workspace_bytes(c, (int64_t)N, true));
@@ -218,10 +220,12 @@
     F->spec_tail = [c, F](const RansacBest* d_best) -> int {
         return refine_begin(c, F->d_u, F->n, F->n, F->d_inl, F->d_in_a, F->d_in_ak, F->d_idx, nullptr, nullptr, 0.0, F->prm.use_acceleration_mode,
                             F->prm.flow_index_mode, F->d_inl_ref, &F->tail, d_best, F->d_refine_ws, &F->refine, state_host(c), F->d_zpartials, false,
-                            &F->claim);
+                            &F->claim, F->ransac.direct_final ? &F->ransac.handoff : nullptr);
     };
     F->refinement_enqueued = false;
     F->ahead = prm->use_refinement && c->ransac_spec_miss < 2;
+    F->d_local_idx = (c->frame_handoff == 0 && F->ahead && F->claim.on && c->lm_arithmetic == 0 && c->refine_arithmetic == 0 && !c->refine_stage_separate)
+                         ? d_local_idx : nullptr;
     F->open = true;
     g_frames_in_flight[c->device & 63].fetch_add(1, std::memory_order_relaxed);
     F->counted = true;
@@ -229,7 +233,7 @@
                                prm->depth_mode, prm->k_sign_mode, &F->ro, prm->use_refinement ? &F->spec_tail : nullptr, &F->refinement_enqueued, &F->ransac,
                                F->side_flatten ? &F->direct : nullptr, F->side_flatten && !F->dense_in_launch ? &F->join : nullptr,
                                F->dense_in_launch ? &F->dense : nullptr, F->ahead, true,
-                               F->claim.on && prm->use_refinement ? refine_flag_words(F->d_refine_ws) : nullptr);
+                               F->claim.on && prm->use_refinement ? refine_flag_words(F->d_refine_ws) : nullptr, F->d_local_idx);
     return RSDSFM_OK;
 }
 
@@ -265,7 +269,7 @@
         rc = ransac_begin(c, F->d_q, F->d_u, F->d_a, F->d_ak, n, prm->use_acceleration_mode, prm->ransac_trials, prm->ransac_tol, nullptr, J.seed,
                           prm->depth_mode, prm->k_sign_mode, &F->ro, prm->use_refinement ? &F->spec_tail : nullptr, &F->refinement_enqueued, &F->ransac, nullptr, nullptr,
                           nullptr, F->ahead, true,
-                               F->claim.on && prm->use_refinement ? refine_flag_words(F->d_refine_ws) : nullptr);
+                               F->claim.on && prm->use_refinement ? refine_flag_words(F->d_refine_ws) : nullptr, F->d_local_idx);
         if (rc == RSDSFM_OK) rc = ransac_finish(c, &F->ransac);
         counted = rc == RSDSFM_OK;
     }
@@ -290,6 +294,11 @@
             rc = refine_poll(c, &F->refine, v, w, &k, &res->refine_summary);
             exact = rc == kRcRefineRestartExact;
         }
+        if ((!F->refinement_enqueued || exact) && F->ransac.direct_final) {
+            rc = ransac_scatter_launch(c, F->ransac.handoff);
+            if (rc != RSDSFM_OK) return rc;
+            F->ransac.direct_final = false;
+        }
         if (!F->refinement_enqueued || exact)
             rc = refine_device(c, F->d_u, n, ro.num_inliers, F->d_inl, F->d_in_a, F->d_in_ak, F->d_idx, v, w, k, prm->use_acceleration_mode,
                                prm->flow_index_mode, F->d_inl_ref, v, w, &k, &res->refine_summary, &F->tail, F->d_zpartials, exact, &F->claim);
@@ -390,6 +399,13 @@
     return RSDSFM_OK;
 }
 
+int rsdsfm_set_frame_handoff(rsdsfm_ctx* ctx, int mode) {
+    if (!ctx) return RSDSFM_ERR_INVALID;
+    if (mode < 0 || mode > 1) return fail(&ctx->c, RSDSFM_ERR_INVALID, "mode must be 0 (the first refinement pass gathers its inliers) or 1 (the compaction launch)");
+    ctx->c.frame_handoff = mode;
+    return RSDSFM_OK;
+}
+
 int rsdsfm_set_frame_side_flatten(rsdsfm_ctx* ctx, int mode) {
     if (!ctx) return RSDSFM_ERR_INVALID;
     if (mode < 0 || mode > 3) return fail(&ctx->c, RSDSFM_ERR_INVALID, "mode must be 0 (flatten first), 1 (flatten on a second stream), 2 (flatten behind the minimal solver) or 3 (flatten inside the solver's launch)");
@@ -426,6 +442,7 @@
         lc->lma_count_only_force = c->lma_count_only_force;
         lc->frame_side_flatten = c->frame_side_flatten;
         lc->frame_tail = c->frame_tail;
+        lc->frame_handoff = c->frame_handoff;
         lc->refine_stage_mode = c->refine_stage_mode;
     }
     for (int l = 0; l < L; ++l) lane_ctx(l)->refine_stage_separate = L > 1;
diff --git a/rs-aware-differential-sfm_amd/csrc/ransac_host.hip b/rs-aware-differential-sfm_amd/csrc/ransac_host.hip
--- a/rs-aware-differential-sfm_amd/csrc/ransac_host.hip
+++ b/rs-aware-differential-sfm_amd/csrc/ransac_host.hip
@@ -181,9 +181,12 @@
                                             nullptr, 0, 0, nullptr, R.tie_margin, lazy);
                     if (rc != RSDSFM_OK) return rc;
                     flags_via_pick = true;
+                    const bool direct = R.d_local_idx && R.spec_tail && R.tail_ahead;
                     rc = ransac_final_launch(c, R.d_q, R.d_u, R.d_a, R.d_ak, n, R.d_best, R.d_states, depth_mode, tol, R.d_rho, R.d_mask, R.d_bcounts,
-                                             R.d_boffs, out->inlier_idx, out->inliers, out->alpha, out->alpha_k, R.h_best, R.refine_flag_words);
-                    if (rc != RSDSFM_OK) return rc;
+                                             R.d_boffs, out->inlier_idx, out->inliers, out->alpha, out->alpha_k, R.h_best, R.refine_flag_words,
+                                             direct ? R.d_local_idx : nullptr, direct ? &R.handoff : nullptr);
+                    if (rc != RSDSFM_OK) return rc;
+                    R.direct_final = direct && R.handoff.local_idx;
                     R.final_done = true;
                     R.spec_final = true;
                     if (R.spec_tail && R.tail_ahead) {
@@ -271,6 +274,8 @@
                     rc = ransac_final_launch(c, R.d_q, R.d_u, R.d_a, R.d_ak, n, R.d_best, R.d_states, depth_mode, tol, R.d_rho, R.d_mask, R.d_bcounts,
                                              R.d_boffs, out->inlier_idx, out->inliers, out->alpha, out->alpha_k, R.h_best, R.refine_flag_words);
                     if (rc != RSDSFM_OK) return rc;
+                    R.direct_final = false;
+                    R.handoff = FrameHandoff();
                 }
                 if (R.spec_tail && !R.tail_enqueued) {
                     rc = (*R.spec_tail)(R.d_best);
@@ -371,9 +376,11 @@
 int ransac_begin(Ctx* c, const double* d_q, const double* d_u, const double* d_a, const double* d_ak, int64_t n, int use_alpha_k, int T,
                  double tol, const int32_t* h_samples, uint64_t seed, int depth_mode, int k_sign_mode, rsdsfm_ransac_out* out,
                  const RansacSpecTail* spec_tail, bool* spec_tail_held, RansacRun* run, const Minimal9Direct* direct,
-                 const std::function<int()>* after_minimal9, const DenseFlatten* dense, bool tail_ahead, bool count_only, int* refine_flag_words) {
+                 const std::function<int()>* after_minimal9, const DenseFlatten* dense, bool tail_ahead, bool count_only, int* refine_flag_words,
+                 uint32_t* local_idx) {
     RansacRun& R = *run;
     R = RansacRun();
+    R.d_local_idx = local_idx;
     R.tail_ahead = tail_ahead;
     R.core_math = c->ransac_math_mode == 0 && c->ransac_standard_math == 0;
     R.analytic = depth_mode == RSDSFM_DEPTH_CERES_LM && T > 0 && c->lm_arithmetic == 0 && c->lma_hold == 0;
diff --git a/rs-aware-differential-sfm_amd/csrc/ransac_kernels.hip b/rs-aware-differential-sfm_amd/csrc/ransac_kernels.hip
--- a/rs-aware-differential-sfm_amd/csrc/ransac_kernels.hip
+++ b/rs-aware-differential-sfm_amd/csrc/ransac_kernels.hip
@@ -705,10 +705,13 @@
                                                           const RansacBest* __restrict__ best,
                                                           const LmState* __restrict__ states, int depth_mode, double tol,
                                                           double* __restrict__ rho_out, uint8_t* __restrict__ mask_out,
-                                                          int64_t* __restrict__ block_counts) {
+                                                          int64_t* __restrict__ block_counts, uint32_t* __restrict__ local_idx = nullptr,
+                                                          int* __restrict__ zero_words = nullptr) {
     __shared__ LmPlanLds plan;
     __shared__ int s_cnt[kRB / 64];
+    __shared__ int s_win[2][kRB / 64];
     const int tid = threadIdx.x, lane = tid & 63, wv = tid >> 6;
+    if (zero_words && blockIdx.x == 0 && tid < (int)(kRefineStateBlockTail / sizeof(int))) zero_words[tid] = 0;
     if (best->undecided) return;
     const int bt = best->best_trial;
     Pose pose;
@@ -728,18 +731,50 @@
     const int64_t i0 = (int64_t)blockIdx.x * chunk;
     const int64_t i1 = (i0 + chunk < n) ? i0 + chunk : n;
     int count = 0;
-    for (int64_t i = i0 + tid; i < i1; i += kRB) {
-        double2 qq = q[i], uu = u[i];
-        const double al = alpha[i], ak = alpha_k[i];
-        bool in = false;
-        double rho = 0.0;
-        if (bt >= 0) {
-            rho = hyp_rho(qq.x, qq.y, uu.x, uu.y, al, ak, pose, two_over, depth_mode, plan);
-            in = point_error(qq.x, qq.y, uu.x, uu.y, al, ak, pose, two_over, rho) < tol;
-        }
-        rho_out[i] = rho;
-        mask_out[i] = in ? 1 : 0;
-        count += in ? 1 : 0;
+    if (local_idx) {
+        int base = 0, par = 0;
+        for (int64_t start = i0; start < i1; start += kRB, par ^= 1) {
+            const int64_t i = start + tid;
+            bool in = false;
+            if (i < i1) {
+                double2 qq = q[i], uu = u[i];
+                const double al = alpha[i], ak = alpha_k[i];
+                double rho = 0.0;
+                if (bt >= 0) {
+                    rho = hyp_rho(qq.x, qq.y, uu.x, uu.y, al, ak, pose, two_over, depth_mode, plan);
+                    in = point_error(qq.x, qq.y, uu.x, uu.y, al, ak, pose, two_over, rho) < tol;
+                }
+                rho_out[i] = rho;
+                mask_out[i] = in ? 1 : 0;
+                count += in ? 1 : 0;
+            }
+            const unsigned long long bal = __ballot(in);
+            if (lane == 0) s_win[par][wv] = __popcll(bal);
+            __syncthreads();
+            int woff = 0, total = 0;
+#pragma unroll
+            for (int w2 = 0; w2 < kRB / 64; ++w2) {
+                const int c = s_win[par][w2];
+                if (w2 < wv) woff += c;
+                total += c;
+            }
+            if (in) local_idx[i0 + base + woff + __popcll(bal & ((1ull << lane) - 1ull))] = (uint32_t)i;
+            base += total;
+        }
+    } else {
+        for (int64_t i = i0 + tid; i < i1; i += kRB) {
+            double2 qq = q[i], uu = u[i];
+            const double al = alpha[i], ak = alpha_k[i];
+            bool in = false;
+            double rho = 0.0;
+            if (bt >= 0) {
+                rho = hyp_rho(qq.x, qq.y, uu.x, uu.y, al, ak, pose, two_over, depth_mode, plan);
+                in = point_error(qq.x, qq.y, uu.x, uu.y, al, ak, pose, two_over, rho) < tol;
+            }
+            rho_out[i] = rho;
+            mask_out[i] = in ? 1 : 0;
+            count += in ? 1 : 0;
+        }
     }
     for (int off = 32; off >= 1; off >>= 1) count += __shfl_xor(count, off, 64);
     if (lane == 0) s_cnt[wv] = count;
@@ -1019,19 +1054,30 @@
 int ransac_final_launch(Ctx* c, const double* q, const double* u, const double* a, const double* ak, int64_t n,
                         RansacBest* best, const LmState* states, int depth_mode, double tol, double* rho, uint8_t* mask,
                         int64_t* block_counts, int64_t* block_offsets, int64_t* inlier_idx, double* inliers,
-                        double* out_alpha, double* out_alpha_k, RansacBest* best_host, int* zero_words) {
+                        double* out_alpha, double* out_alpha_k, RansacBest* best_host, int* zero_words, uint32_t* local_idx,
+                        FrameHandoff* handoff) {
     int64_t blocks = (n + kRB - 1) / kRB;
     if (blocks < 1) blocks = 1;
-    const int64_t cap = 2048;
+    const int64_t cap = kRfHandoffBlocks;
     int64_t chunk = kRB;
     if (blocks > cap) {
         chunk = ((blocks + cap - 1) / cap) * kRB;
         blocks = (n + chunk - 1) / chunk;
     }
+    const bool direct = local_idx && handoff && n <= (int64_t)INT32_MAX;
+    if (handoff) *handoff = FrameHandoff();
     hipLaunchKernelGGL(ransac_final_kernel, dim3((int)blocks), dim3(kRB), 0, c->stream, reinterpret_cast<const double2*>(q),
                        reinterpret_cast<const double2*>(u), a, ak, n, chunk, best, states, depth_mode, tol, rho, mask,
-                       block_counts);
-    RSDSFM_HIP_CHECK(c, hipGetLastError());
+                       block_counts, direct ? local_idx : nullptr, direct ? zero_words : nullptr);
+    RSDSFM_HIP_CHECK(c, hipGetLastError());
+    if (direct) {
+        FrameHandoff& H = *handoff;
+        H.local_idx = local_idx, H.block_counts = block_counts, H.nblocks = (int)blocks, H.chunk = chunk, H.n = n;
+        H.q = q, H.alpha = a, H.alpha_k = ak, H.rho = rho, H.mask = mask;
+        H.best = best, H.best_host = best_host;
+        H.inlier_idx = inlier_idx, H.inliers = inliers, H.out_alpha = out_alpha, H.out_alpha_k = out_alpha_k;
+        return RSDSFM_OK;
+    }
     if (inlier_idx || inliers || out_alpha || out_alpha_k) {
         hipLaunchKernelGGL(ransac_scatter_kernel, dim3((int)blocks), dim3(kRB), 0, c->stream, reinterpret_cast<const double2*>(q),
                            a, ak, n, chunk, rho, mask, block_counts, best, best_host, inlier_idx, inliers, out_alpha, out_alpha_k, zero_words);
@@ -1043,4 +1089,11 @@
     return RSDSFM_OK;
 }
 
-}
+int ransac_scatter_launch(Ctx* c, const FrameHandoff& H) {
+    hipLaunchKernelGGL(ransac_scatter_kernel, dim3(H.nblocks), dim3(kRB), 0, c->stream, reinterpret_cast<const double2*>(H.q), H.alpha, H.alpha_k, H.n,
+                       H.chunk, H.rho, H.mask, H.block_counts, H.best, H.best_host, H.inlier_idx, H.inliers, H.out_alpha, H.out_alpha_k, nullptr);
+    RSDSFM_HIP_CHECK(c, hipGetLastError());
+    return RSDSFM_OK;
+}
+
+}
diff --git a/rs-aware-differential-sfm_amd/csrc/refine_host.hip b/rs-aware-differential-sfm_amd/csrc/refine_host.hip
--- a/rs-aware-differential-sfm_amd/csrc/refine_host.hip
+++ b/rs-aware-differential-sfm_amd/csrc/refine_host.hip
@@ -9,7 +9,9 @@
 int refine_begin(Ctx* c, const double* d_flow, int64_t n_flow, int64_t m, const double* d_inl, const double* d_alpha,
                  const double* d_alpha_k, const int64_t* d_inlier_idx, const double v_in[3], const double w_in[3], double k_in,
                  int const_acceleration, int flow_index_mode, double* d_inl_out, const RefineTail* tail, const RansacBest* d_best,
-                 void* ws_base, RefineRun* run, RefineState* hs_prefetch, double* d_zpartials, bool exact, const FinishClaim* claim) {
+                 void* ws_base, RefineRun* run, RefineState* hs_prefetch, double* d_zpartials, bool exact, const FinishClaim* claim,
+                 const FrameHandoff* handoff) {
+    const bool direct = handoff && handoff->local_idx;
     if (m < 0 || n_flow < 0 || (!d_best && (!v_in || !w_in))) return fail(c, RSDSFM_ERR_INVALID, "bad arguments");
     if (flow_index_mode != RSDSFM_FLOW_COMPAT_RANK && flow_index_mode != RSDSFM_FLOW_GATHERED) return fail(c, RSDSFM_ERR_INVALID, "unknown flow_index_mode");
     if (flow_index_mode == RSDSFM_FLOW_GATHERED && m > 0 && !d_inlier_idx) return fail(c, RSDSFM_ERR_INVALID, "gathered mode needs inlier_idx");
@@ -62,6 +64,12 @@
     B.state_host = hs_prefetch;
     if (d_best && claim && claim->on && run->rf && !c->refine_stage_separate) {
         B.best_dev = d_best;
+        if (direct) {
+            B.handoff = *handoff;
+            B.fin_xy = B.uu, B.fin_stride = 4;
+        }
+    } else if (direct) {
+        return fail(c, RSDSFM_ERR_INVALID, "refinement: direct hand-off without the start state in the first pass");
     } else if (d_best) {
         rc = refine_state_from_best_launch(c, d_best, B, np);
         if (rc != RSDSFM_OK) return rc;
diff --git a/rs-aware-differential-sfm_amd/csrc/refine_kernels.hip b/rs-aware-differential-sfm_amd/csrc/refine_kernels.hip
--- a/rs-aware-differential-sfm_amd/csrc/refine_kernels.hip
+++ b/rs-aware-differential-sfm_amd/csrc/refine_kernels.hip
@@ -462,7 +462,8 @@
                                                                  double* __restrict__ inl_out, double* __restrict__ zpartials,
                                                                  RefineState* __restrict__ state_host, const int* __restrict__ bad_index,
                                                                  double fx, double fy, double cx, double cy, int rows, int ncols,
-                                                                 unsigned* __restrict__ owner, unsigned tag, int32_t* __restrict__ ys) {
+                                                                 unsigned* __restrict__ owner, unsigned tag, int32_t* __restrict__ ys,
+                                                                 int xy_stride) {
     __shared__ double s_red[kFB / 64];
     if (state_host && blockIdx.x == 0) {
         for (int i = threadIdx.x; i < (int)(sizeof(RefineState) / 8); i += kFB)
@@ -474,7 +475,7 @@
     const int64_t stride = (int64_t)gridDim.x * kFB;
     double acc = 0.0;
     for (int64_t i = (int64_t)blockIdx.x * kFB + threadIdx.x; i < m; i += stride) {
-        const double xn = inl[3 * i], yn = inl[3 * i + 1];
+        const double xn = inl[xy_stride * i], yn = inl[xy_stride * i + 1];
         inl_out[3 * i] = xn;
         inl_out[3 * i + 1] = yn;
         const double z = 1.0 / rho[i];
@@ -896,12 +897,13 @@
 int refine_finish_launch(Ctx* c, const RefineBuffers& B, double* inl_out) {
     if (!B.m_on_device && B.m == 0 && !B.zpartials && !B.state_host) return RSDSFM_OK;
     if (B.claim.on) {
-        hipLaunchKernelGGL(refine_finish_claim_kernel, dim3(refine_finish_grid(c, B)), dim3(kFB), 0, c->stream, B.m_on_device ? (int64_t)-1 : B.m, B.inl,
-                           B.rho_a, B.rho_b, B.state, inl_out, B.zpartials, B.state_host, B.bad_index, B.claim.fx, B.claim.fy, B.claim.cx, B.claim.cy,
-                           B.claim.rows, B.claim.cols, B.claim.owner, B.claim.tag, B.claim.ys);
+        hipLaunchKernelGGL(refine_finish_claim_kernel, dim3(refine_finish_grid(c, B)), dim3(kFB), 0, c->stream, B.m_on_device ? (int64_t)-1 : B.m,
+                           B.fin_xy ? B.fin_xy : B.inl, B.rho_a, B.rho_b, B.state, inl_out, B.zpartials, B.state_host, B.bad_index, B.claim.fx, B.claim.fy,
+                           B.claim.cx, B.claim.cy, B.claim.rows, B.claim.cols, B.claim.owner, B.claim.tag, B.claim.ys, B.fin_xy ? B.fin_stride : 3);
         RSDSFM_HIP_CHECK(c, hipGetLastError());
         return RSDSFM_OK;
     }
+    if (B.fin_xy) return fail(c, RSDSFM_ERR_INVALID, "refinement: the direct hand-off needs the claiming output pass");
     hipLaunchKernelGGL(refine_finish_kernel, dim3(refine_finish_grid(c, B)), dim3(kFB), 0, c->stream,
                        B.m_on_device ? (int64_t)-1 : B.m, B.inl, B.rho_a, B.rho_b, B.state, inl_out, B.zpartials, B.state_host, B.bad_index);
     RSDSFM_HIP_CHECK(c, hipGetLastError());
diff --git a/rs-aware-differential-sfm_amd/csrc/refine_rf_kernels.hip b/rs-aware-differential-sfm_amd/csrc/refine_rf_kernels.hip
--- a/rs-aware-differential-sfm_amd/csrc/refine_rf_kernels.hip
+++ b/rs-aware-differential-sfm_amd/csrc/refine_rf_kernels.hip
@@ -618,6 +618,19 @@
     const RansacBest* best;
     int grid_cap;
     unsigned long long* stamps;
+    const uint32_t* local_idx;
+    const int64_t* block_counts;
+    int nblocks;
+    int64_t chunk;
+    const double2* q_px;
+    const double* alpha_px;
+    const double* alpha_k_px;
+    const double* rho_px;
+    int64_t* inlier_idx_out;
+    double* alpha_out;
+    double* alpha_k_out;
+    RansacBest* best_pub;
+    RansacBest* best_host;
 };
 
 struct RfLoad {
@@ -642,9 +655,14 @@
 
 }
 
-template <int NP, bool FIRST, bool ZSUM>
+template <int NP, bool FIRST, bool ZSUM, bool DIRECT = false>
 __global__ __launch_bounds__(kFB) void refine_rf_pass_kernel(const RfPassArgs A) {
+    static_assert(FIRST || !DIRECT, "only the first pass gathers");
     using RR = RfRow<NP>;
+    __shared__ uint32_t s_off[DIRECT ? kRfHandoffBlocks + 1 : 1];
+    __shared__ uint32_t s_coarse[64];
+    static_assert(kRfHandoffBlocks == 64 * 32, "rounds of the search");
+    __shared__ uint32_t s_wtot[kFB / 64];
     __shared__ RfStageLds<NP> s_stage;
     __shared__ double s_red[kFB / 64][RR::NW];
     __shared__ RefineState s_state;
@@ -660,6 +678,54 @@
         for (int i = 0; i < 8; ++i) tk[i] = 0;
     }
     if (stamp) tk[0] = wall_clock64();
+    int64_t m_direct = 0;
+    if (DIRECT) {
+        const int tid = threadIdx.x, lane = tid & 63, wv = tid >> 6;
+        const int nb = A.nblocks;
+        if (!A.best->undecided) {
+            constexpr int kPer = (kRfHandoffBlocks + kFB - 1) / kFB;
+            const int per = (nb + kFB - 1) / kFB;
+            uint32_t cnt[kPer], sum = 0;
+#pragma unroll
+            for (int j = 0; j < kPer; ++j) {
+                const int b = tid * per + j;
+                cnt[j] = (j < per && b < nb) ? (uint32_t)A.block_counts[b] : 0u;
+                sum += cnt[j];
+            }
+            uint32_t inc = sum;
+#pragma unroll
+            for (int off = 1; off < 64; off <<= 1) {
+                const uint32_t t = __shfl_up(inc, off, 64);
+                if (lane >= off) inc += t;
+            }
+            if (lane == 63) s_wtot[wv] = inc;
+            __syncthreads();
+            uint32_t wbase = 0, total = 0;
+#pragma unroll
+            for (int w2 = 0; w2 < kFB / 64; ++w2) {
+                const uint32_t v = s_wtot[w2];
+                if (w2 < wv) wbase += v;
+                total += v;
+            }
+            uint32_t run = wbase + inc - sum;
+#pragma unroll
+            for (int j = 0; j < kPer; ++j) {
+                const int b = tid * per + j;
+                if (j < per && b < nb) {
+                    s_off[b] = run;
+                    run += cnt[j];
+                }
+            }
+            if (tid == 0) s_off[nb] = total;
+            m_direct = (int64_t)total;
+            __syncthreads();
+            if (tid < 64) s_coarse[tid] = tid * 32 < nb ? s_off[tid * 32] : 0xFFFFFFFFu;
+            if (blockIdx.x == 0 && tid == 0) {
+                A.best_pub->num_inliers_scan = m_direct;
+                if (A.best_host) A.best_host->num_inliers_scan = m_direct;
+            }
+        }
+    }
     if (FIRST && A.best) {
         if (threadIdx.x < sizeof(RefineState) / 8) reinterpret_cast<unsigned long long*>(&s_state)[threadIdx.x] = 0ull;
         __syncthreads();
@@ -674,7 +740,7 @@
             z.termination = -1;
             z.radius = kInitialRadius;
             z.need_schur = 1;
-            const int64_t mb = A.best->undecided ? 0 : A.best->num_inliers_scan;
+            const int64_t mb = A.best->undecided ? 0 : (DIRECT ? m_direct : A.best->num_inliers_scan);
             z.m = mb;
             int64_t b = (mb + kFB - 1) / kFB;
             if (b < 1) b = 1;
@@ -733,16 +799,7 @@
     if (FIRST) {
         RfPoint Pq = rf_point(st->p);
         const RfPoint P = rf_point_uniform(Pq);
-        for (int64_t i = i0; i < m; i += stride) {
-            int64_t fi = (A.flow_index_mode == RSDSFM_FLOW_GATHERED) ? A.inlier_idx[i] : i;
-            if (fi < 0 || fi >= A.n_flow) {
-                *A.bad_index = 1;
-                fi = 0;
-            }
-            const double2 f = A.flow[fi];
-            const double x = A.inl[3 * i], y = A.inl[3 * i + 1];
-            const double rho = 1.0 / A.inl[3 * i + 2];
-            const double al = A.alpha[i], ak = A.alpha_k[i];
+        auto body = [&](int64_t i, double x, double y, double rho, double al, double ak, const double2 f) {
             A.xyuv_out[i] = make_double4(x, y, f.x, f.y);
             const double ab = NP == 6 ? P.c1 * __builtin_fma(P.k, ak, al) : al;
             if (NP == 6) A.beta[i] = ab;
@@ -761,6 +818,84 @@
             const double ihm = flagged ? 0.0 : rcp_core(flagged ? 1.0 : o.h);
             rf_schur_accumulate<NP>(o, ihm, acc);
             if (flagged) rf_list_append(A.list_count, A.list_entries, x, y, f.x, f.y, ab, ak, rho, i);
+        };
+        if (DIRECT) {
+            const int lane = threadIdx.x & 63;
+            auto rank_pixel = [&](int64_t iw) -> int64_t {
+                if (iw >= m) return 0;
+                const uint32_t r0 = (uint32_t)iw, r = r0 + (uint32_t)lane;
+                const int c = __popcll(__ballot(s_coarse[lane] <= r0)) - 1;
+                const int t = c * 32 + lane;
+                const int b_lo = c * 32 + __popcll(__ballot(lane < 32 && t <= A.nblocks && s_off[t] <= r0)) - 1;
+                if (r >= (uint32_t)m) return 0;
+                int b = b_lo;
+                while (s_off[b + 1] <= r) ++b;
+                return (int64_t)A.local_idx[(int64_t)b * A.chunk + (r - s_off[b])];
+            };
+            struct Rec {
+                double2 q, f;
+                double rho, al, ak;
+                int64_t p;
+            };
+            auto load = [&](int64_t i, int64_t p) {
+                Rec r;
+                r.q = r.f = make_double2(0.0, 0.0), r.rho = r.al = r.ak = 0.0, r.p = p;
+                if (i < m) {
+                    int64_t fi = (A.flow_index_mode == RSDSFM_FLOW_GATHERED) ? p : i;
+                    if (fi < 0 || fi >= A.n_flow) {
+                        *A.bad_index = 1;
+                        fi = 0;
+                    }
+                    r.f = A.flow[fi];
+                    r.q = A.q_px[p];
+                    r.rho = A.rho_px[p];
+                    r.al = A.alpha_px[p], r.ak = A.alpha_k_px[p];
+                }
+                return r;
+            };
+            auto turn = [&](const Rec& r, int64_t i) {
+                const double z = 1.0 / r.rho;
+                const double rho = 1.0 / z;
+                A.inlier_idx_out[i] = r.p;
+                if (NP == 7) A.alpha_out[i] = r.al, A.alpha_k_out[i] = r.ak;
+                body(i, r.q.x, r.q.y, rho, r.al, r.ak, r.f);
+            };
+            const int64_t iw0 = i0 - lane;
+            if (NP == 6) {
+                Rec r0 = load(i0, rank_pixel(iw0));
+                Rec r1 = load(i0 + stride, rank_pixel(iw0 + stride));
+                int64_t p2 = rank_pixel(iw0 + 2 * stride);
+                for (int64_t iw = iw0; iw < m; iw += stride) {
+                    const int64_t i = iw + lane;
+                    const Rec r2 = load(i + 2 * stride, p2);
+                    p2 = rank_pixel(iw + 3 * stride);
+                    if (i < m) turn(r0, i);
+                    r0 = r1;
+                    r1 = r2;
+                }
+            } else {
+                int64_t p0 = rank_pixel(iw0), p1 = rank_pixel(iw0 + stride);
+                for (int64_t iw = iw0; iw < m; iw += stride) {
+                    const int64_t i = iw + lane;
+                    const Rec r = load(i, p0);
+                    p0 = p1;
+                    p1 = rank_pixel(iw + 2 * stride);
+                    if (i < m) turn(r, i);
+                }
+            }
+        } else {
+            for (int64_t i = i0; i < m; i += stride) {
+                int64_t fi = (A.flow_index_mode == RSDSFM_FLOW_GATHERED) ? A.inlier_idx[i] : i;
+                if (fi < 0 || fi >= A.n_flow) {
+                    *A.bad_index = 1;
+                    fi = 0;
+                }
+                const double2 f = A.flow[fi];
+                const double x = A.inl[3 * i], y = A.inl[3 * i + 1];
+                const double rho = 1.0 / A.inl[3 * i + 2];
+                const double al = A.alpha[i], ak = A.alpha_k[i];
+                body(i, x, y, rho, al, ak, f);
+            }
         }
     } else {
         RfPoint Pq = rf_point(st->p), Pcq = rf_point(st->pc);
@@ -1016,7 +1151,9 @@
 }
 template <int NP, bool ZSUM>
 void rf_pass_launch_t(Ctx* c, const RfPassArgs& A, bool first, int grid) {
-    if (first)
+    if (first && A.local_idx)
+        hipLaunchKernelGGL((refine_rf_pass_kernel<NP, true, ZSUM, true>), dim3(grid), dim3(kFB), 0, c->stream, A);
+    else if (first)
         hipLaunchKernelGGL((refine_rf_pass_kernel<NP, true, ZSUM>), dim3(grid), dim3(kFB), 0, c->stream, A);
     else
         hipLaunchKernelGGL((refine_rf_pass_kernel<NP, false, ZSUM>), dim3(grid), dim3(kFB), 0, c->stream, A);
@@ -1066,6 +1203,14 @@
     A.beat = rf_beat(c);
     A.slot = g;
     const bool first = g == 0;
+    if (first && B.handoff.local_idx) {
+        const FrameHandoff& H = B.handoff;
+        if (!A.best || H.nblocks > kRfHandoffBlocks || H.n > (int64_t)INT32_MAX) return fail(c, RSDSFM_ERR_INVALID, "refinement: direct hand-off without its preconditions");
+        A.local_idx = H.local_idx, A.block_counts = H.block_counts, A.nblocks = H.nblocks, A.chunk = H.chunk;
+        A.q_px = reinterpret_cast<const double2*>(H.q), A.alpha_px = H.alpha, A.alpha_k_px = H.alpha_k, A.rho_px = H.rho;
+        A.inlier_idx_out = H.inlier_idx, A.alpha_out = H.out_alpha, A.alpha_k_out = H.out_alpha_k;
+        A.best_pub = H.best, A.best_host = H.best_host;
+    }
     if (np == 7) {
         if (B.want_zsum) rf_pass_launch_t<7, true>(c, A, first, grid); else rf_pass_launch_t<7, false>(c, A, first, grid);
     } else {
diff --git a/rs-aware-differential-sfm_amd/csrc/rsdsfm_internal.hpp b/rs-aware-differential-sfm_amd/csrc/rsdsfm_internal.hpp
--- a/rs-aware-differential-sfm_amd/csrc/rsdsfm_internal.hpp
+++ b/rs-aware-differential-sfm_amd/csrc/rsdsfm_internal.hpp
@@ -72,6 +72,18 @@
     int32_t shared_best;
     int32_t _pad_shared;
     int32_t lazy_pending;
+};
+constexpr int kRfHandoffBlocks = 2048;
+struct FrameHandoff {
+    const uint32_t* local_idx = nullptr;
+    const int64_t* block_counts = nullptr;
+    int nblocks = 0;
+    int64_t chunk = 0, n = 0;
+    const double *q = nullptr, *alpha = nullptr, *alpha_k = nullptr, *rho = nullptr;
+    const uint8_t* mask = nullptr;
+    RansacBest *best = nullptr, *best_host = nullptr;
+    int64_t* inlier_idx = nullptr;
+    double *inliers = nullptr, *out_alpha = nullptr, *out_alpha_k = nullptr;
 };
 struct PickLazy {
     int* scored = nullptr;
@@ -159,6 +171,7 @@
     hipEvent_t ev_fork = nullptr, ev_join = nullptr, ev_seq = nullptr;
     int frame_side_flatten = 3;
     int frame_tail = 0;
+    int frame_handoff = 0;
     unsigned long long* d_flat_counters = nullptr;
     int seq_lanes = 0;
     int refine_stage_mode = 0;
@@ -351,7 +364,9 @@
 int ransac_final_launch(Ctx* c, const double* q, const double* u, const double* a, const double* ak, int64_t n,
                         RansacBest* best, const LmState* states, int depth_mode, double tol, double* rho, uint8_t* mask,
                         int64_t* block_counts, int64_t* block_offsets, int64_t* inlier_idx, double* inliers,
-                        double* out_alpha, double* out_alpha_k, RansacBest* best_host = nullptr, int* zero_words = nullptr);
+                        double* out_alpha, double* out_alpha_k, RansacBest* best_host = nullptr, int* zero_words = nullptr,
+                        uint32_t* local_idx = nullptr, FrameHandoff* handoff = nullptr);
+int ransac_scatter_launch(Ctx* c, const FrameHandoff& H);
 int ransac_rows_doubles();
 int ransac_lm_rows_launch(Ctx* c, const double* q, const double* u, const double* a, const double* ak, int64_t n,
                           const double* hyp, int T, const LmState* states, double* partials, int round, double tol, double* rows,
@@ -428,6 +443,9 @@
     double* zpartials = nullptr;
     const RansacBest* best_dev = nullptr;
     FinishClaim claim;
+    FrameHandoff handoff;
+    const double* fin_xy = nullptr;
+    int fin_stride = 3;
     bool want_zsum = false;
 };
 size_t ransac_pinned_bytes(int T);
@@ -447,6 +465,9 @@
     bool analytic = false;
     bool lma_restarted = false;
     int* refine_flag_words = nullptr;
+    uint32_t* d_local_idx = nullptr;
+    FrameHandoff handoff;
+    bool direct_final = false;
     bool count_only = false;
     int lazy_rounds = 0;
     int shared_best = 0;
@@ -483,7 +504,7 @@
                  double tol, const int32_t* h_samples, uint64_t seed, int depth_mode, int k_sign_mode, rsdsfm_ransac_out* out,
                  const RansacSpecTail* spec_tail, bool* spec_tail_held, RansacRun* run, const Minimal9Direct* direct,
                  const std::function<int()>* after_minimal9, const DenseFlatten* dense = nullptr, bool tail_ahead = true, bool count_only = false,
-                 int* refine_flag_words = nullptr);
+                 int* refine_flag_words = nullptr, uint32_t* local_idx = nullptr);
 int ransac_finish(Ctx* c, RansacRun* run);
 void ransac_commit_hints(Ctx* c, const RansacRun& run);
 int flatten_enqueue(Ctx* c, const double* d_img, int32_t rows, int32_t cols, double fx, double fy, double cx, double cy, double gamma,
@@ -508,7 +529,7 @@
                  const double* d_alpha_k, const int64_t* d_inlier_idx, const double v_in[3], const double w_in[3], double k_in,
                  int const_acceleration, int flow_index_mode, double* d_inl_out, const RefineTail* tail, const RansacBest* d_best,
                  void* ws_base, RefineRun* run, RefineState* hs_prefetch, double* d_zpartials, bool exact = false,
-                 const FinishClaim* claim = nullptr);
+                 const FinishClaim* claim = nullptr, const FrameHandoff* handoff = nullptr);
 constexpr int kRcRefineRestartExact = 1;
 int refine_device(Ctx* c, const double* d_flow, int64_t n_flow, int64_t m, const double* d_inl, const double* d_alpha,
                   const double* d_alpha_k, const int64_t* d_inlier_idx, const double v_in[3], const double w_in[3], double k_in,
```

Result: faster. 1785 (median of 6 runs) (+1.7%).
